# automl/RoBO

Hardware: AMD Instinct MI355X
Metric: EI evals/sec + GP-fit ms at N=4096,D=16; 1/2/4/8 MI355X vs host CPU (higher is better)
Workload: dtype f64

## Files before the change

include/robo_hip.h:

```cpp
#ifndef ROBO_HIP_H
#define ROBO_HIP_H

#include <stdint.h>

#ifdef __cplusplus
extern "C" {
#endif

typedef struct robo_ctx robo_ctx;
typedef struct robo_gp robo_gp;
typedef struct robo_cand robo_cand;

enum robo_status {
    ROBO_OK = 0,
    ROBO_NOT_POSITIVE_DEFINITE = 1,
    ROBO_NOT_FITTED = 2,
    ROBO_BAD_SHAPE = 3,
    ROBO_RUNTIME_ERROR = 4,
    ROBO_BAD_ARGUMENT = 5,
    ROBO_NUMERIC_ERROR = 6
};

enum robo_kernel_kind {
    ROBO_KERNEL_MATERN52_ARD = 0,
    ROBO_KERNEL_RBF_ARD = 1,
    ROBO_KERNEL_FABOLAS = 2
};

enum robo_acq_kind {
    ROBO_ACQ_EI = 0,
    ROBO_ACQ_LOG_EI = 1,
    ROBO_ACQ_PI = 2,
    ROBO_ACQ_LCB = 3
};

#define ROBO_FLAG_ZERO_SIGMA 1u
#define ROBO_FLAG_NEGATIVE_EI 2u
#define ROBO_FLAG_NAN 4u
#define ROBO_FLAG_NOT_FACTORED 8u
#define ROBO_FLAG_FROZEN 16u

int32_t robo_device_count(int32_t* out_n);
int32_t robo_ctx_create(int32_t device, void* hip_stream, robo_ctx** out);
int32_t robo_ctx_destroy(robo_ctx* ctx);
int32_t robo_ctx_live_count(int32_t* out_n);
int32_t robo_ctx_synchronize(robo_ctx* ctx);
int32_t robo_ctx_device_name(robo_ctx* ctx, char* buf, int32_t buf_len);
int32_t robo_ctx_event_record(robo_ctx* ctx, int32_t slot);
int32_t robo_ctx_event_elapsed_ms(robo_ctx* ctx, int32_t slot_begin, int32_t slot_end, float* out_ms);
int32_t robo_ctx_set_phase_events(robo_ctx* ctx, int32_t on);
int32_t robo_ctx_set_tuning(robo_ctx* ctx, const char* key, int64_t value);
const char* robo_last_error_string(void);
const char* robo_version_string(void);

int32_t robo_gp_create(robo_ctx* ctx, int32_t kernel_kind, int32_t n_max, int32_t dim, robo_gp** out);
int32_t robo_gp_destroy(robo_gp* gp);
int32_t robo_gp_set_data(robo_gp* gp, const double* X, const double* y, int32_t n);
int32_t robo_gp_set_output_transform(robo_gp* gp, double y_mean, double y_std);
int32_t robo_gp_set_precision(robo_gp* gp, int32_t fp32_gram);
int32_t robo_theta_size(int32_t kernel_kind, int32_t dim);
int32_t robo_gp_fit(robo_gp* gp, const double* theta, double mean_c, double* out_loglik, int32_t* out_fail_col);
int32_t robo_gp_grad_loglik(robo_gp* gp, const double* theta, double mean_c, double* out_loglik,
                            double* out_grad, int32_t* out_fail_col);

int32_t robo_gp_loglik_batch(robo_gp* gp, const double* thetas, int32_t S, double mean_c, double* out_loglik,
                             int32_t* out_status);

int32_t robo_gp_grad_loglik_batch(robo_gp* gp, const double* thetas, int32_t S, double mean_c, double* out_loglik,
                                  double* out_grad, int32_t* out_status);

int32_t robo_gp_optimize_hypers(robo_gp* gp, double mean_c, int32_t prior_kind, const double* prior_par,
                                const double* lower, const double* upper, const double* starts, int32_t n_starts,
                                int32_t n_iters, int32_t history, double step0, double c1, double gtol,
                                double* out_theta, double* out_value, int32_t* out_best, double* out_final,
                                double* out_values, int32_t* out_status, double* out_trace);

int32_t robo_gp_mcmc_run(robo_gp* gp, double mean_c, int32_t prior_kind, const double* prior_par, int32_t n_walkers,
                         int32_t n_steps, double a, const double* u_stretch, const int32_t* partner,
                         const double* u_accept, int32_t eval_start, double* pos, double* lnp, double* out_chain,
                         double* out_lnprob, int64_t* out_accepted);
int32_t robo_mcmc_draws(uint32_t* mt_key, int32_t* mt_pos, int32_t n_steps, int32_t half, double* u_stretch,
                        int32_t* partner, double* u_accept);
int32_t robo_gp_fit_batch(robo_gp* const* gps, int32_t S, const double* thetas, double mean_c, double* out_loglik,
                          int32_t* out_status);
int32_t robo_gp_get_factor(robo_gp* gp, double* out_L);
int32_t robo_gp_get_gram(robo_gp* gp, const double* theta, double* out_K);
int32_t robo_gp_factor_cond(robo_gp* gp, double* out);
int32_t robo_gp_prefetch_inverse(robo_gp* gp);

int32_t robo_cand_create(robo_ctx* ctx, const double* Xc, int64_t m, int32_t dim, robo_cand** out);
int32_t robo_cand_destroy(robo_cand* cand);
int32_t robo_cand_set_points(robo_cand* cand, const double* Xc, int64_t m);
int32_t robo_cand_create_uniform(robo_ctx* ctx, int64_t m, int32_t dim, uint64_t seed, robo_cand** out);
int32_t robo_cand_create_random(robo_ctx* ctx, int64_t m, int32_t dim, uint64_t seed, int64_t n_uniform,
                                const double* loc, const double* scale, robo_cand** out);
int32_t robo_cand_create_sobol(robo_ctx* ctx, int64_t m, int32_t dim, const uint64_t* sv, const uint64_t* shift,
                               int32_t bits, uint64_t first_index, robo_cand** out);
int32_t robo_cand_get_points(robo_cand* cand, double* out_Xc);
int32_t robo_cand_workspace_chunk(robo_cand* cand, int64_t* out_chunk);
int32_t robo_cand_last_solve_kernel(robo_cand* cand, char* buf, int32_t buf_len);
int32_t robo_cand_get_point(robo_cand* cand, int64_t index, double* out_x);

int32_t robo_gp_predict_cand(robo_gp* gp, robo_cand* cand, double* out_mean, double* out_var);
int32_t robo_gp_predict(robo_gp* gp, const double* Xc, int64_t m, double* out_mean, double* out_var);
int32_t robo_gp_predict_mixture_cand(robo_gp* const* gps, int32_t S, robo_cand* cand, double* out_mean,
                                     double* out_var);
int32_t robo_gp_predict_grad(robo_gp* gp, const double* Xc, int64_t m, double* out_mean, double* out_var,
                             double* out_dmean, double* out_dvar);
int32_t robo_gp_predict_cov(robo_gp* gp, const double* Xc, int64_t m, double* out_mean, double* out_cov);

int32_t robo_acq_eval_cand(robo_gp* gp, int32_t acq_kind, double par, double eta, robo_cand* cand, double* out_acq,
                           double* out_max, int64_t* out_argmax, uint32_t* out_flags);
int32_t robo_acq_eval(robo_gp* gp, int32_t acq_kind, double par, double eta, const double* Xc, int64_t m,
                      double* out_acq, double* out_max, int64_t* out_argmax, uint32_t* out_flags);
#define ROBO_SCREEN_NOT_ELIGIBLE 0
#define ROBO_SCREEN_SCREENED 1
#define ROBO_SCREEN_PROBE_USED 2
#define ROBO_SCREEN_FELL_BACK 3
int32_t robo_cand_last_screen(robo_cand* cand, int64_t* out_n_screened, int64_t* out_n_survivors, int32_t* out_outcome);
#define ROBO_SCREEN_FINISH_NONE 0
#define ROBO_SCREEN_FINISH_FULL 1
#define ROBO_SCREEN_FINISH_LEAN 2
int32_t robo_cand_last_screen_finish(robo_cand* cand, int32_t* out_finish, int32_t* out_fused_tail);
int32_t robo_cand_last_screen_first(robo_cand* cand, int32_t* out_stage, int64_t* out_kept);
int32_t robo_acq_screen_bounds(robo_gp* gp, int32_t acq_kind, double par, double eta, robo_cand* cand, double* out_upper,
                               double* out_lower);
int32_t robo_acq_eval_moments(robo_ctx* ctx, int32_t acq_kind, double par, double eta, const double* mean,
                              const double* var, int64_t m, double* out_acq, double* out_max, int64_t* out_argmax,
                              uint32_t* out_flags);
int32_t robo_acq_eval_marginal_cand(robo_gp* const* gps, int32_t S, int32_t acq_kind, double par, const double* etas,
                                    robo_cand* cand, double* out_acq, double* out_max, int64_t* out_argmax,
                                    uint32_t* out_flags);
int32_t robo_acq_eval_sum_cand(robo_gp* const* gps, int32_t S, int32_t acq_kind, double par, const double* etas,
                               robo_cand* cand, double* out_acq_sum, uint32_t* out_flags);

int32_t robo_acq_refine_cand(robo_gp* gp, int32_t acq_kind, double par, double eta, robo_cand* cand, int32_t n_starts,
                             int32_t n_steps, double step0, double* out_x, double* out_value, int64_t* out_start_index,
                             uint32_t* out_flags, int64_t* out_starts, double* out_trace);
int32_t robo_acq_refine_marginal_cand(robo_gp* const* gps, int32_t S, int32_t acq_kind, double par, const double* etas,
                                      robo_cand* cand, int32_t n_starts, int32_t n_steps, double step0, double* out_x,
                                      double* out_value, int64_t* out_start_index, uint32_t* out_flags,
                                      int64_t* out_starts, double* out_trace);

int32_t robo_rep_sample(robo_gp* gp, int32_t acq_kind, double par, double eta, const double* lower, const double* upper,
                        int32_t normalize, int32_t n_walkers, int32_t n_steps, double a, const double* u_stretch,
                        const int32_t* partner, const double* u_accept, double* pos, double* lnp, int32_t eval_start,
                        int64_t* out_accepted, uint32_t* out_flags, double* out_trace);
int32_t robo_rep_sample_batch(robo_gp* const* gps, int32_t S, int32_t acq_kind, double par, const double* etas,
                              const double* lower, const double* upper, int32_t normalize, int32_t n_walkers,
                              int32_t n_steps, double a, const double* u_stretch, const int32_t* partner,
                              const double* u_accept, double* pos, double* lnp, int32_t eval_start, int64_t* out_accepted,
                              uint32_t* out_flags, double* out_trace);

enum robo_fantasy_kind { ROBO_FANTASY_KRIGING_BELIEVER = 0, ROBO_FANTASY_CONSTANT_LIAR = 1 };
int32_t robo_acq_batch_cand(robo_gp* gp, int32_t acq_kind, double par, double eta, robo_cand* cand, int32_t q,
                            int32_t fantasy_kind, double liar, int64_t* out_idx, double* out_values, double* out_fantasy,
                            uint32_t* out_flags, int32_t* out_n_made, double* out_trace);
int32_t robo_acq_batch_marginal_cand(robo_gp* const* gps, int32_t S, int32_t acq_kind, double par, const double* etas,
                                     robo_cand* cand, int32_t q, int32_t fantasy_kind, double liar, int64_t* out_idx,
                                     double* out_values, double* out_fantasy, uint32_t* out_flags, int32_t* out_n_made,
                                     double* out_trace);

#define ROBO_QEI_MAX_Q 64
#define ROBO_QEI_MAX_K 1024
int32_t robo_qei_batch_cand(robo_gp* gp, double par, double eta, robo_cand* cand, int32_t q, const double* z, int32_t K,
                            int64_t* out_idx, double* out_gain, uint32_t* out_flags, int32_t* out_n_made, double* out_acq,
                            double* out_trace, double* out_coef, double* out_d, double* out_best);
int32_t robo_qei_batch_marginal_cand(robo_gp* const* gps, int32_t S, double par, const double* etas, robo_cand* cand,
                                     int32_t q, const double* z, int32_t K, int64_t* out_idx, double* out_gain,
                                     uint32_t* out_flags, int32_t* out_n_made, double* out_acq, double* out_trace,
                                     double* out_coef, double* out_d, double* out_best);

int32_t robo_mes_eval_cand(robo_gp* gp, double eta, robo_cand* cand, const double* u, int32_t K, int32_t clamp,
                           double* out_acq, double* out_max, int64_t* out_argmax, uint32_t* out_flags, double* out_ystar,
                           double* out_gumbel, double* out_trace);
int32_t robo_mes_eval_marginal_cand(robo_gp* const* gps, int32_t S, const double* etas, robo_cand* cand, const double* u,
                                    int32_t K, int32_t clamp, double* out_acq, double* out_max, int64_t* out_argmax,
                                    uint32_t* out_flags, double* out_ystar, double* out_gumbel, double* out_trace);
int32_t robo_mes_sample_min_moments(robo_ctx* ctx, const double* mean, const double* var, int64_t m, const double* u,
                                    int32_t K, int32_t clamp, double eta, double* out_ystar, double* out_gumbel);
int32_t robo_mes_eval_moments(robo_ctx* ctx, const double* mean, const double* var, int64_t m, const double* ystar,
                              int32_t K, double* out_acq, double* out_max, int64_t* out_argmax, uint32_t* out_flags);

int32_t robo_kg_eval_cand(robo_gp* gp, robo_cand* cand, robo_cand* rep, double sn2, int32_t include_self, double* out_kg,
                          double* out_max, int64_t* out_argmax, uint32_t* out_flags, double* out_disc_mean,
                          double* out_trace);
int32_t robo_kg_eval_marginal_cand(robo_gp* const* gps, int32_t S, robo_cand* cand, robo_cand* rep, const double* sn2s,
                                   int32_t include_self, double* out_kg, double* out_max, int64_t* out_argmax,
                                   uint32_t* out_flags, double* out_disc_mean, double* out_trace);
int32_t robo_kg_eval_moments(robo_ctx* ctx, int64_t m, int32_t nb, double sn2, int32_t include_self, const double* s,
                             const double* v, const double* mean, const double* disc_mean, double* out_kg,
                             double* out_max, int64_t* out_argmax, uint32_t* out_flags);

#define ROBO_EHVI_MAX_FRONT 4096
int32_t robo_ehvi_eval_cand(robo_gp* gp1, robo_gp* gp2, robo_cand* cand, const double* front, int32_t P, const double* ref,
                            double* out_ehvi, double* out_max, int64_t* out_argmax, uint32_t* out_flags,
                            double* out_trace);
int32_t robo_ehvi_eval_moments(robo_ctx* ctx, int64_t m, const double* mean1, const double* var1, const double* mean2,
                               const double* var2, const double* front, int32_t P, const double* ref, double* out_ehvi,
                               double* out_max, int64_t* out_argmax, uint32_t* out_flags);

#define ROBO_CEI_MAX_CONSTRAINTS 16
int32_t robo_cei_eval_cand(robo_gp* objective, robo_gp* const* constraints, int32_t C, const double* thresholds,
                           int32_t acq_kind, double par, double eta, int32_t has_eta, robo_cand* cand,
                           double* out_values , double* out_max, int64_t* out_argmax, uint32_t* out_flags,
                           double* out_trace );
int32_t robo_cei_refine_cand(robo_gp* objective, robo_gp* const* constraints, int32_t C, const double* thresholds,
                             int32_t acq_kind, double par, double eta, int32_t has_eta, robo_cand* cand,
                             int32_t n_starts, int32_t n_steps, double step0,
                             double* out_x, double* out_value, int64_t* out_start_index, uint32_t* out_flags,
                             int64_t* out_starts , double* out_trace );
int32_t robo_cei_eval_moments(robo_ctx* ctx, int64_t m, int32_t C, const double* mean0, const double* var0,
                              const double* means, const double* vars, const double* thresholds, int32_t acq_kind,
                              double par, double eta, int32_t has_eta, double* out_values, double* out_max,
                              int64_t* out_argmax, uint32_t* out_flags);

#define ROBO_PATHS_MAX 64
#define ROBO_PATHS_MAX_FEATURES 4096
typedef struct robo_paths robo_paths;
int32_t robo_paths_create(robo_gp* gp, int32_t F, int32_t S, const double* omega, const double* phase,
                          const double* w, const double* eps, robo_paths** out);
int32_t robo_paths_eval_cand(robo_paths* p, robo_cand* cand, double* out_values ,
                             double* out_min , int64_t* out_argmin , uint32_t* out_flags);
int32_t robo_paths_destroy(robo_paths* p);

#define ROBO_PATHS_MAX_STARTS 1024
#define ROBO_PATHS_MAX_DESCENTS 65536
int32_t robo_paths_descend(robo_paths* p, int32_t P, const int32_t* path_of, const double* x0 ,
                           int32_t n_steps, double step0, double* out_x , double* out_value ,
                           double* out_grad , int32_t* out_code ,
                           uint32_t* out_flags, double* out_trace );
int32_t robo_paths_refine_cand(robo_paths* p, robo_cand* cand, int32_t n_starts, int32_t n_steps, double step0,
                               double* out_x , double* out_value ,
                               int64_t* out_start_index , uint32_t* out_flags,
                               int64_t* out_starts , double* out_trace );

int32_t robo_ig_eval_cand(robo_gp* gp, robo_cand* cand, robo_cand* rep, int32_t n_outcomes, double sn2,
                          const double* logP, const double* lmb, const double* W, const double* dlogPdMu,
                          const double* dlogPdSigma, const double* dlogPdMudMu, double* out_dh, double* out_max,
                          int64_t* out_argmax);
int32_t robo_ig_eval_per_cost_cand(robo_gp* gp, robo_cand* cand, robo_cand* rep, int32_t n_outcomes, double sn2,
                                   const double* logP, const double* lmb, const double* W, const double* dlogPdMu,
                                   const double* dlogPdSigma, const double* dlogPdMudMu, robo_gp* cost_gp,
                                   robo_cand* cost_cand, double overhead, double* out_values, double* out_max,
                                   int64_t* out_argmax);
int32_t robo_ig_eval_moments(robo_ctx* ctx, int64_t m, int32_t nb, int32_t n_outcomes, double sn2, const double* s,
                             const double* v, const double* logP, const double* lmb, const double* W,
                             const double* dlogPdMu, const double* dlogPdSigma, const double* dlogPdMudMu,
                             double* out_dh);
int32_t robo_gp_cross_cov(robo_gp* gp, robo_cand* cand, robo_cand* ref, double* out_cov);
int32_t robo_ep_joint_min(robo_ctx* ctx, int32_t S, int32_t nb, const double* mu, const double* sigma,
                          int32_t with_derivatives, double* logP, double* dlogPdMu, double* dlogPdSigma,
                          double* dlogPdMudMu, int32_t* out_sweeps, int32_t* out_status);

int32_t robo_pmin_mc(robo_ctx* ctx, int32_t S, int32_t nb, int32_t nf, const double* mu, const double* sigma,
                     const double* z, double* out_pmin, double* out_jitter, int32_t* out_status);
int32_t robo_igmc_eval_cand(robo_gp* gp, robo_cand* cand, robo_cand* rep, int32_t n_outcomes, int32_t nf, double sn2,
                            const double* Mb, const double* Vb, const double* logP, const double* lmb, const double* W,
                            const double* z, double* out_dh, double* out_max, int64_t* out_argmax, uint32_t* out_flags);
int32_t robo_igmc_eval_moments(robo_ctx* ctx, int64_t m, int32_t nb, int32_t n_outcomes, int32_t nf, double sn2,
                               const double* s, const double* v, const double* Mb, const double* Vb, const double* logP,
                               const double* lmb, const double* W, const double* z, double* out_dh,
                               int32_t* out_counts, double* out_jitter);

typedef struct robo_comm robo_comm;
#define ROBO_COMM_ID_BYTES 128
int32_t robo_comm_create_id(void* out_id);
int32_t robo_comm_init(robo_ctx* ctx, int32_t rank, int32_t world, const void* id, robo_comm** out);
int32_t robo_comm_destroy(robo_comm* comm);
int32_t robo_comm_info(robo_comm* comm, int32_t* out_rank, int32_t* out_world);
int32_t robo_comm_allgather(robo_comm* comm, const double* send, int64_t count, double* recv);
int32_t robo_acq_eval_cand_sharded(robo_comm* comm, robo_gp* gp, int32_t acq_kind, double par, double eta,
                                   robo_cand* cand, int64_t global_offset, double* out_acq, double* out_max,
                                   int64_t* out_argmax, int32_t* out_owner_rank, uint32_t* out_flags);
int32_t robo_ig_eval_per_cost_cand_sharded(robo_comm* comm, robo_gp* gp, robo_cand* cand, robo_cand* rep,
                                           int32_t n_outcomes, double sn2, const double* logP, const double* lmb,
                                           const double* W, const double* dlogPdMu, const double* dlogPdSigma,
                                           const double* dlogPdMudMu, robo_gp* cost_gp, robo_cand* cost_cand,
                                           double overhead, int64_t global_offset, double* out_values, double* out_max,
                                           int64_t* out_argmax, int32_t* out_owner_rank);
int32_t robo_acq_eval_marginal_cand_sharded(robo_comm* comm, robo_gp* const* gps, int32_t S_local, int32_t S_total,
                                            int32_t acq_kind, double par, const double* etas, robo_cand* cand,
                                            double* out_acq, double* out_max, int64_t* out_argmax,
                                            uint32_t* out_flags);

typedef struct robo_multi robo_multi;
int32_t robo_multi_create(robo_ctx* const* ctxs, int32_t n_ctx, robo_multi** out);
int32_t robo_multi_destroy(robo_multi* multi);
int32_t robo_multi_info(robo_multi* multi, int32_t* out_n, int32_t* out_devices, int32_t* out_threads);
int32_t robo_gp_set_data_multi(robo_multi* multi, robo_gp* const* gps, const double* X, const double* y, int32_t n);
int32_t robo_gp_fit_multi(robo_multi* multi, robo_gp* const* gps, const double* theta, double mean_c, double* out_loglik,
                          int32_t* out_fail_col);
int32_t robo_gp_loglik_batch_multi(robo_multi* multi, robo_gp* const* gps, const double* thetas, int32_t S, double mean_c,
                                   double* out_loglik, int32_t* out_status);
int32_t robo_gp_fit_batch_multi(robo_multi* multi, robo_gp* const* gps, const int32_t* S_dev, const double* thetas,
                                double mean_c, double* out_loglik, int32_t* out_status);
int32_t robo_acq_eval_cand_multi(robo_multi* multi, robo_gp* const* gps, int32_t acq_kind, double par, double eta,
                                 robo_cand* const* cands, const int64_t* global_offsets, double* out_acq, double* out_max,
                                 int64_t* out_argmax, int32_t* out_owner, uint32_t* out_flags);
int32_t robo_ig_eval_cand_multi(robo_multi* multi, robo_gp* const* gps, robo_cand* const* cands, robo_cand* const* reps,
                                int32_t n_outcomes, double sn2, const double* logP, const double* lmb, const double* W,
                                const double* dlogPdMu, const double* dlogPdSigma, const double* dlogPdMudMu,
                                const int64_t* global_offsets, double* out_dh, double* out_max, int64_t* out_argmax,
                                int32_t* out_owner);
int32_t robo_ig_eval_per_cost_cand_multi(robo_multi* multi, robo_gp* const* gps, robo_cand* const* cands,
                                         robo_cand* const* reps, int32_t n_outcomes, double sn2, const double* logP,
                                         const double* lmb, const double* W, const double* dlogPdMu,
                                         const double* dlogPdSigma, const double* dlogPdMudMu, robo_gp* const* cost_gps,
                                         robo_cand* const* cost_cands, double overhead, const int64_t* global_offsets,
                                         double* out_values, double* out_max, int64_t* out_argmax, int32_t* out_owner);
int32_t robo_acq_eval_marginal_cand_multi(robo_multi* multi, robo_gp* const* gps, const int32_t* S_dev, int32_t acq_kind,
                                          double par, const double* etas, robo_cand* const* cands, double* out_acq,
                                          double* out_max, int64_t* out_argmax, uint32_t* out_flags);
int32_t robo_gp_predict_mixture_cand_multi(robo_multi* multi, robo_gp* const* gps, const int32_t* S_dev,
                                           robo_cand* const* cands, double* out_mean, double* out_var);

#ifdef __cplusplus
}
#endif
#endif
```

robo_amd/_lib.py:

```python
import atexit
import ctypes as C
import os
import weakref

import numpy as np

_HERE = os.path.dirname(os.path.abspath(__file__))
DEFAULT_LIBRARY = os.path.join(_HERE, "librobo_hip.so")
DEFAULT_DIAG_LIBRARY = os.path.join(_HERE, "librobo_hip_diag.so")

OK, NOT_POSITIVE_DEFINITE, NOT_FITTED, BAD_SHAPE, RUNTIME_ERROR, BAD_ARGUMENT, NUMERIC_ERROR = range(7)
EP_MAX_NB = 64
EP_NAN_MESSAGE = ("an error occurs while running expectation propagation in entropy search. "
                  "Resulting variance contains NaN")
KERNEL_KINDS = {"matern52": 0, "rbf": 1, "fabolas": 2}
ACQ_KINDS = {"ei": 0, "log_ei": 1, "pi": 2, "lcb": 3}
FLAG_ZERO_SIGMA, FLAG_NEGATIVE_EI, FLAG_NAN, FLAG_NOT_FACTORED, FLAG_FROZEN = 1, 2, 4, 8, 16
SCREEN_NOT_ELIGIBLE, SCREEN_SCREENED, SCREEN_PROBE_USED, SCREEN_FELL_BACK = 0, 1, 2, 3
SCREEN_FINISH_NONE, SCREEN_FINISH_FULL, SCREEN_FINISH_LEAN = 0, 1, 2
FANTASY_KINDS = {"kriging_believer": 0, "constant_liar": 1}
MES_MAX_K = 128
KG_MAX_DISC = 64
EHVI_MAX_FRONT = 4096
CEI_MAX_CONSTRAINTS = 16
PATHS_MAX = 64
PATHS_MAX_FEATURES = 4096
PATHS_MAX_STARTS = 1024
PATHS_MAX_DESCENTS = 65536
REFINE_MAX_STARTS = 1024
MC_MAX_NB, MC_MAX_NP, MC_MAX_NF = 64, 512, 65535

SYMBOLS = [
    "robo_device_count", "robo_ctx_create", "robo_ctx_destroy", "robo_ctx_live_count", "robo_ctx_synchronize",
    "robo_ctx_device_name", "robo_ctx_event_record", "robo_ctx_event_elapsed_ms", "robo_ctx_set_phase_events",
    "robo_ctx_set_tuning",
    "robo_last_error_string", "robo_version_string",
    "robo_gp_create", "robo_gp_destroy", "robo_gp_set_data", "robo_gp_set_output_transform",
    "robo_gp_set_precision", "robo_theta_size",
    "robo_gp_fit", "robo_gp_loglik_batch", "robo_gp_mcmc_run", "robo_mcmc_draws", "robo_gp_fit_batch", "robo_gp_grad_loglik", "robo_gp_grad_loglik_batch",
    "robo_gp_optimize_hypers", "robo_gp_get_factor", "robo_gp_get_gram", "robo_gp_factor_cond", "robo_gp_prefetch_inverse",
    "robo_cand_create", "robo_cand_destroy", "robo_cand_set_points", "robo_cand_create_uniform", "robo_cand_get_points",
    "robo_cand_create_random", "robo_cand_create_sobol", "robo_cand_get_point", "robo_cand_workspace_chunk", "robo_cand_last_solve_kernel",
    "robo_gp_predict_cand", "robo_gp_predict", "robo_gp_predict_cov", "robo_gp_predict_grad", "robo_gp_predict_mixture_cand",
    "robo_acq_eval_cand", "robo_acq_eval", "robo_acq_eval_moments", "robo_acq_eval_marginal_cand", "robo_acq_eval_sum_cand",
    "robo_cand_last_screen", "robo_cand_last_screen_finish", "robo_cand_last_screen_first", "robo_acq_screen_bounds",
    "robo_acq_refine_cand", "robo_acq_refine_marginal_cand",
    "robo_rep_sample", "robo_rep_sample_batch",
    "robo_acq_batch_cand", "robo_acq_batch_marginal_cand", "robo_qei_batch_cand", "robo_qei_batch_marginal_cand",
    "robo_mes_eval_cand", "robo_mes_eval_marginal_cand", "robo_mes_sample_min_moments", "robo_mes_eval_moments",
    "robo_kg_eval_cand", "robo_kg_eval_marginal_cand", "robo_kg_eval_moments",
    "robo_ehvi_eval_cand", "robo_ehvi_eval_moments",
    "robo_cei_eval_cand", "robo_cei_eval_moments", "robo_cei_refine_cand",
    "robo_paths_create", "robo_paths_eval_cand", "robo_paths_destroy", "robo_paths_descend", "robo_paths_refine_cand",
    "robo_ig_eval_cand", "robo_ig_eval_per_cost_cand", "robo_ig_eval_moments", "robo_gp_cross_cov",
    "robo_ep_joint_min", "robo_pmin_mc", "robo_igmc_eval_cand", "robo_igmc_eval_moments",
    "robo_comm_create_id", "robo_comm_init", "robo_comm_destroy", "robo_comm_info", "robo_comm_allgather",
    "robo_acq_eval_cand_sharded", "robo_acq_eval_marginal_cand_sharded", "robo_ig_eval_per_cost_cand_sharded",
    "robo_multi_create", "robo_multi_destroy", "robo_multi_info", "robo_gp_set_data_multi", "robo_gp_fit_multi",
    "robo_gp_loglik_batch_multi", "robo_gp_fit_batch_multi", "robo_acq_eval_cand_multi",
    "robo_ig_eval_cand_multi", "robo_ig_eval_per_cost_cand_multi", "robo_acq_eval_marginal_cand_multi",
    "robo_gp_predict_mixture_cand_multi",
]
COMM_ID_BYTES = 128
DIAG_SYMBOLS = [
    "robo_selftest_mfma_layout", "robo_microbench_mfma_f64", "robo_microbench_mfma_f64_detail", "robo_microbench_gemm_f64",
    "robo_selftest_diag_timeline", "robo_diag_clock_sample_begin", "robo_diag_clock_sample_end",
    "robo_selftest_stretch_move", "robo_diag_cross_gram", "robo_diag_cov_rows",
]


class RoboHipUnavailable(RuntimeError):
    pass


class RoboHipError(RuntimeError):
    pass


class RoboBadShape(AssertionError):
    """ROBO_BAD_SHAPE from the library (the reference uses ``assert`` for shapes, base_model.py:68-70,76) -- its own type
    so that callers can tell the library's verdict from a Python-side assert"""


_lib = None
_lib_path = None
_diag = None
_dp = C.POINTER(C.c_double)


def _arr(a):
    return a.ctypes.data_as(_dp)


def _f64(a, shape=None):
    a = np.ascontiguousarray(a, dtype=np.float64)
    if shape is not None and a.shape != shape:
        raise AssertionError("expected shape %r, got %r" % (shape, a.shape))
    return a


def _handles(gps):
    return (C.c_void_p * max(len(gps), 1))(*[g._h for g in gps])


def _etas(eta, S):
    return _f64(np.broadcast_to(np.asarray(eta, dtype=np.float64), (S,)))


def _ensemble_head(gps, eta, marginal, *between):
    if not marginal:
        return (gps[0]._h,) + between + (float(eta),)
    return (_handles(gps), len(gps)) + between + (_arr(_etas(eta, len(gps))),)


class _Best(object):

    def __init__(self):
        self.max, self.argmax, self.flags = C.c_double(0), C.c_int64(0), C.c_uint32(0)
        self.refs = (C.byref(self.max), C.byref(self.argmax), C.byref(self.flags))

    def values(self):
        return self.max.value, self.argmax.value, self.flags.value


def use_library(path):
    global _lib, _lib_path, _default_ctx, _diag, _extra_ctx, _multis
    _close_multis()
    _lib = None
    _diag = None
    _lib_path = path
    _default_ctx = {}
    _extra_ctx = {}
    _multis = {}


def library_path():
    return _lib_path or DEFAULT_LIBRARY


def lib():
    global _lib
    if _lib is not None:
        return _lib
    path = library_path()
    if not os.path.exists(path):
        raise RoboHipUnavailable(
            "%s not found: build it with `python -m robo_amd.build` (hipcc, gfx950). "
            "robo_amd has no CPU fallback." % path)
    try:
        L = C.CDLL(path)
    except OSError as e:
        raise RoboHipUnavailable("cannot load %s: %s" % (path, e))
    vp, i32, i64, dbl = C.c_void_p, C.c_int32, C.c_int64, C.c_double
    pp = C.POINTER(vp)
    sig = {
        "robo_device_count": [C.POINTER(i32)],
        "robo_ctx_create": [i32, vp, pp],
        "robo_ctx_destroy": [vp],
        "robo_ctx_live_count": [C.POINTER(i32)],
        "robo_ctx_synchronize": [vp],
        "robo_ctx_device_name": [vp, C.c_char_p, i32],
        "robo_ctx_event_record": [vp, i32],
        "robo_ctx_event_elapsed_ms": [vp, i32, i32, C.POINTER(C.c_float)],
        "robo_ctx_set_phase_events": [vp, i32],
        "robo_ctx_set_tuning": [vp, C.c_char_p, i64],
        "robo_gp_create": [vp, i32, i32, i32, pp],
        "robo_gp_destroy": [vp],
        "robo_gp_set_data": [vp, _dp, _dp, i32],
        "robo_gp_set_output_transform": [vp, dbl, dbl],
        "robo_gp_set_precision": [vp, i32],
        "robo_theta_size": [i32, i32],
        "robo_gp_fit": [vp, _dp, dbl, _dp, C.POINTER(i32)],
        "robo_gp_loglik_batch": [vp, _dp, i32, dbl, _dp, C.POINTER(i32)],
        "robo_gp_fit_batch": [pp, i32, _dp, dbl, _dp, C.POINTER(i32)],
        "robo_mcmc_draws": [C.POINTER(C.c_uint32), C.POINTER(i32), i32, i32, _dp, C.POINTER(i32), _dp],
        "robo_gp_mcmc_run": [vp, dbl, i32, _dp, i32, i32, dbl, _dp, C.POINTER(i32), _dp, i32, _dp, _dp, _dp, _dp,
                             C.POINTER(i64)],
        "robo_gp_grad_loglik": [vp, _dp, dbl, _dp, _dp, C.POINTER(i32)],
        "robo_gp_grad_loglik_batch": [vp, _dp, i32, dbl, _dp, _dp, C.POINTER(i32)],
        "robo_gp_optimize_hypers": [vp, dbl, i32, _dp, _dp, _dp, _dp, i32, i32, i32, dbl, dbl, dbl, _dp, _dp,
                                    C.POINTER(i32), _dp, _dp, C.POINTER(i32), _dp],
        "robo_gp_get_factor": [vp, _dp],
        "robo_gp_get_gram": [vp, _dp, _dp],
        "robo_gp_factor_cond": [vp, _dp],
        "robo_gp_prefetch_inverse": [vp],
        "robo_cand_create": [vp, _dp, i64, i32, pp],
        "robo_cand_destroy": [vp],
        "robo_cand_set_points": [vp, _dp, i64],
        "robo_cand_create_uniform": [vp, i64, i32, C.c_uint64, pp],
        "robo_cand_get_points": [vp, _dp],
        "robo_cand_create_random": [vp, i64, i32, C.c_uint64, i64, _dp, _dp, pp],
        "robo_cand_create_sobol": [vp, i64, i32, C.POINTER(C.c_uint64), C.POINTER(C.c_uint64), i32, C.c_uint64, pp],
        "robo_cand_get_point": [vp, i64, _dp],
        "robo_cand_workspace_chunk": [vp, C.POINTER(i64)],
        "robo_cand_last_solve_kernel": [vp, C.c_char_p, i32],
        "robo_gp_predict_cand": [vp, vp, _dp, _dp],
        "robo_gp_predict": [vp, _dp, i64, _dp, _dp],
        "robo_gp_predict_cov": [vp, _dp, i64, _dp, _dp],
        "robo_gp_predict_grad": [vp, _dp, i64, _dp, _dp, _dp, _dp],
        "robo_gp_predict_mixture_cand": [pp, i32, vp, _dp, _dp],
        "robo_acq_eval_cand": [vp, i32, dbl, dbl, vp, _dp, _dp, C.POINTER(i64), C.POINTER(C.c_uint32)],
        "robo_acq_eval": [vp, i32, dbl, dbl, _dp, i64, _dp, _dp, C.POINTER(i64), C.POINTER(C.c_uint32)],
        "robo_cand_last_screen": [vp, C.POINTER(i64), C.POINTER(i64), C.POINTER(i32)],
        "robo_cand_last_screen_finish": [vp, C.POINTER(i32), C.POINTER(i32)],
        "robo_cand_last_screen_first": [vp, C.POINTER(i32), C.POINTER(i64)],
        "robo_acq_screen_bounds": [vp, i32, dbl, dbl, vp, _dp, _dp],
        "robo_acq_eval_moments": [vp, i32, dbl, dbl, _dp, _dp, i64, _dp, _dp, C.POINTER(i64), C.POINTER(C.c_uint32)],
        "robo_acq_eval_marginal_cand": [pp, i32, i32, dbl, _dp, vp, _dp, _dp, C.POINTER(i64),
                                        C.POINTER(C.c_uint32)],
        "robo_acq_eval_sum_cand": [pp, i32, i32, dbl, _dp, vp, _dp, C.POINTER(C.c_uint32)],
        "robo_acq_refine_cand": [vp, i32, dbl, dbl, vp, i32, i32, dbl, _dp, _dp, C.POINTER(i64), C.POINTER(C.c_uint32),
                                 C.POINTER(i64), _dp],
        "robo_acq_refine_marginal_cand": [pp, i32, i32, dbl, _dp, vp, i32, i32, dbl, _dp, _dp, C.POINTER(i64),
                                          C.POINTER(C.c_uint32), C.POINTER(i64), _dp],
        "robo_rep_sample": [vp, i32, dbl, dbl, _dp, _dp, i32, i32, i32, dbl, _dp, C.POINTER(i32), _dp, _dp, _dp, i32,
                            C.POINTER(i64), C.POINTER(C.c_uint32), _dp],
        "robo_rep_sample_batch": [pp, i32, i32, dbl, _dp, _dp, _dp, i32, i32, i32, dbl, _dp, C.POINTER(i32), _dp, _dp, _dp,
                                  i32, C.POINTER(i64), C.POINTER(C.c_uint32), _dp],
        "robo_acq_batch_cand": [vp, i32, dbl, dbl, vp, i32, i32, dbl, C.POINTER(i64), _dp, _dp, C.POINTER(C.c_uint32),
                                C.POINTER(i32), _dp],
        "robo_acq_batch_marginal_cand": [pp, i32, i32, dbl, _dp, vp, i32, i32, dbl, C.POINTER(i64), _dp, _dp,
                                         C.POINTER(C.c_uint32), C.POINTER(i32), _dp],
        "robo_qei_batch_cand": [vp, dbl, dbl, vp, i32, _dp, i32, C.POINTER(i64), _dp, C.POINTER(C.c_uint32), C.POINTER(i32),
                                _dp, _dp, _dp, _dp, _dp],
        "robo_qei_batch_marginal_cand": [pp, i32, dbl, _dp, vp, i32, _dp, i32, C.POINTER(i64), _dp, C.POINTER(C.c_uint32),
                                         C.POINTER(i32), _dp, _dp, _dp, _dp, _dp],
        "robo_mes_eval_cand": [vp, dbl, vp, _dp, i32, i32, _dp, _dp, C.POINTER(i64), C.POINTER(C.c_uint32), _dp, _dp, _dp],
        "robo_mes_eval_marginal_cand": [pp, i32, _dp, vp, _dp, i32, i32, _dp, _dp, C.POINTER(i64), C.POINTER(C.c_uint32),
                                        _dp, _dp, _dp],
        "robo_mes_sample_min_moments": [vp, _dp, _dp, i64, _dp, i32, i32, dbl, _dp, _dp],
        "robo_mes_eval_moments": [vp, _dp, _dp, i64, _dp, i32, _dp, _dp, C.POINTER(i64), C.POINTER(C.c_uint32)],
        "robo_kg_eval_cand": [vp, vp, vp, dbl, i32, _dp, _dp, C.POINTER(i64), C.POINTER(C.c_uint32), _dp, _dp],
        "robo_kg_eval_marginal_cand": [pp, i32, vp, vp, _dp, i32, _dp, _dp, C.POINTER(i64), C.POINTER(C.c_uint32), _dp, _dp],
        "robo_kg_eval_moments": [vp, i64, i32, dbl, i32, _dp, _dp, _dp, _dp, _dp, _dp, C.POINTER(i64),
                                 C.POINTER(C.c_uint32)],
        "robo_ehvi_eval_cand": [vp, vp, vp, _dp, i32, _dp, _dp, _dp, C.POINTER(i64), C.POINTER(C.c_uint32), _dp],
        "robo_ehvi_eval_moments": [vp, i64, _dp, _dp, _dp, _dp, _dp, i32, _dp, _dp, _dp, C.POINTER(i64),
                                   C.POINTER(C.c_uint32)],
        "robo_cei_eval_cand": [vp, pp, i32, _dp, i32, dbl, dbl, i32, vp, _dp, _dp, C.POINTER(i64), C.POINTER(C.c_uint32),
                               _dp],
        "robo_cei_eval_moments": [vp, i64, i32, _dp, _dp, _dp, _dp, _dp, i32, dbl, dbl, i32, _dp, _dp, C.POINTER(i64),
                                  C.POINTER(C.c_uint32)],
        "robo_cei_refine_cand": [vp, pp, i32, _dp, i32, dbl, dbl, i32, vp, i32, i32, dbl, _dp, _dp, C.POINTER(i64),
                                 C.POINTER(C.c_uint32), C.POINTER(i64), _dp],
        "robo_paths_create": [vp, i32, i32, _dp, _dp, _dp, _dp, pp],
        "robo_paths_eval_cand": [vp, vp, _dp, _dp, C.POINTER(i64), C.POINTER(C.c_uint32)],
        "robo_paths_destroy": [vp],
        "robo_paths_descend": [vp, i32, C.POINTER(i32), _dp, i32, dbl, _dp, _dp, _dp, C.POINTER(i32), C.POINTER(C.c_uint32),
                               _dp],
        "robo_paths_refine_cand": [vp, vp, i32, i32, dbl, _dp, _dp, C.POINTER(i64), C.POINTER(C.c_uint32), C.POINTER(i64),
                                   _dp],
        "robo_ig_eval_cand": [vp, vp, vp, i32, dbl, _dp, _dp, _dp, _dp, _dp, _dp, _dp, _dp, C.POINTER(i64)],
        "robo_ig_eval_per_cost_cand": [vp, vp, vp, i32, dbl, _dp, _dp, _dp, _dp, _dp, _dp, vp, vp, dbl, _dp, _dp,
                                       C.POINTER(i64)],
        "robo_ig_eval_per_cost_cand_sharded": [vp, vp, vp, vp, i32, dbl, _dp, _dp, _dp, _dp, _dp, _dp, vp, vp, dbl, i64,
                                               _dp, _dp, C.POINTER(i64), C.POINTER(i32)],
        "robo_ig_eval_moments": [vp, i64, i32, i32, dbl, _dp, _dp, _dp, _dp, _dp, _dp, _dp, _dp, _dp],
        "robo_gp_cross_cov": [vp, vp, vp, _dp],
        "robo_ep_joint_min": [vp, i32, i32, _dp, _dp, i32, _dp, _dp, _dp, _dp, C.POINTER(i32), C.POINTER(i32)],
        "robo_pmin_mc": [vp, i32, i32, i32, _dp, _dp, _dp, _dp, _dp, C.POINTER(i32)],
        "robo_igmc_eval_cand": [vp, vp, vp, i32, i32, dbl, _dp, _dp, _dp, _dp, _dp, _dp, _dp, _dp, C.POINTER(i64),
                                C.POINTER(C.c_uint32)],
        "robo_igmc_eval_moments": [vp, i64, i32, i32, i32, dbl, _dp, _dp, _dp, _dp, _dp, _dp, _dp, _dp, _dp,
                                   C.POINTER(i32), _dp],
        "robo_comm_create_id": [C.c_char_p],
        "robo_comm_init": [vp, i32, i32, C.c_char_p, pp],
        "robo_comm_destroy": [vp],
        "robo_comm_info": [vp, C.POINTER(i32), C.POINTER(i32)],
        "robo_comm_allgather": [vp, _dp, i64, _dp],
        "robo_acq_eval_cand_sharded": [vp, vp, i32, dbl, dbl, vp, i64, _dp, _dp, C.POINTER(i64), C.POINTER(i32),
                                       C.POINTER(C.c_uint32)],
        "robo_acq_eval_marginal_cand_sharded": [vp, pp, i32, i32, i32, dbl, _dp, vp, _dp, _dp, C.POINTER(i64),
                                                C.POINTER(C.c_uint32)],
        "robo_multi_create": [pp, i32, pp],
        "robo_multi_destroy": [vp],
        "robo_multi_info": [vp, C.POINTER(i32), C.POINTER(i32), C.POINTER(i32)],
        "robo_gp_set_data_multi": [vp, pp, _dp, _dp, i32],
        "robo_gp_fit_multi": [vp, pp, _dp, dbl, _dp, C.POINTER(i32)],
        "robo_gp_loglik_batch_multi": [vp, pp, _dp, i32, dbl, _dp, C.POINTER(i32)],
        "robo_gp_fit_batch_multi": [vp, pp, C.POINTER(i32), _dp, dbl, _dp, C.POINTER(i32)],
        "robo_acq_eval_cand_multi": [vp, pp, i32, dbl, dbl, pp, C.POINTER(i64), _dp, _dp, C.POINTER(i64), C.POINTER(i32),
                                     C.POINTER(C.c_uint32)],
        "robo_ig_eval_cand_multi": [vp, pp, pp, pp, i32, dbl, _dp, _dp, _dp, _dp, _dp, _dp, C.POINTER(i64), _dp, _dp,
                                    C.POINTER(i64), C.POINTER(i32)],
        "robo_ig_eval_per_cost_cand_multi": [vp, pp, pp, pp, i32, dbl, _dp, _dp, _dp, _dp, _dp, _dp, pp, pp, dbl,
                                             C.POINTER(i64), _dp, _dp, C.POINTER(i64), C.POINTER(i32)],
        "robo_acq_eval_marginal_cand_multi": [vp, pp, C.POINTER(i32), i32, dbl, _dp, pp, _dp, _dp, C.POINTER(i64),
                                              C.POINTER(C.c_uint32)],
        "robo_gp_predict_mixture_cand_multi": [vp, pp, C.POINTER(i32), pp, _dp, _dp],
    }
    for name, args in sig.items():
        if path != DEFAULT_LIBRARY and not hasattr(L, name):
            def missing(*_, _name=name, _path=path):
                raise RoboHipUnavailable("%s does not export %s" % (_path, _name))
            setattr(L, name, missing)
            continue
        fn = getattr(L, name)
        fn.argtypes = args
        fn.restype = i32
    L.robo_last_error_string.restype = C.c_char_p
    L.robo_last_error_string.argtypes = []
    L.robo_version_string.restype = C.c_char_p
    L.robo_version_string.argtypes = []
    n = i32(0)
    L.robo_device_count(C.byref(n))
    if n.value < 1:
        raise RoboHipUnavailable("librobo_hip loaded but no HIP device is visible (robo_amd has no CPU fallback)")
    _lib = L
    return L


def diag():
    global _diag
    if _diag is not None:
        return _diag
    lib()
    path = _lib_path or DEFAULT_DIAG_LIBRARY
    if not os.path.exists(path):
        raise RoboHipUnavailable("%s not found: build it with `python -m robo_amd.build`" % path)
    D = C.CDLL(path)
    vp, i32 = C.c_void_p, C.c_int32
    for name, args in {"robo_selftest_mfma_layout": [vp, _dp], "robo_microbench_mfma_f64": [vp, i32, _dp],
                       "robo_microbench_mfma_f64_detail": [vp, i32, _dp],
                       "robo_microbench_gemm_f64": [vp, i32, i32, i32, i32, _dp],
                       "robo_selftest_diag_timeline": [vp, _dp, _dp],
                       "robo_diag_clock_sample_begin": [vp, i32], "robo_diag_clock_sample_end": [vp, _dp],
                       "robo_selftest_stretch_move": [vp, _dp, _dp, _dp, C.c_double, i32, i32, _dp, _dp, _dp],
                       "robo_diag_cross_gram": [vp, _dp, _dp, i32, _dp],
                       "robo_diag_cov_rows": [vp, i32, i32, C.c_double, C.c_double, C.c_double, _dp, _dp, C.c_int64,
                                              _dp]}.items():
        fn = getattr(D, name)
        fn.argtypes = args
        fn.restype = i32
    _diag = D
    return D


def last_error():
    return lib().robo_last_error_string().decode("utf-8", "replace")


def check(status, msg=None):
    if status == OK:
        return
    msg = last_error() if msg is None else msg
    if status == NOT_POSITIVE_DEFINITE:
        raise np.linalg.LinAlgError(msg or "matrix is not positive definite")
    if status == NOT_FITTED:
        raise Exception('Model has to be trained first!')
    if status == BAD_SHAPE:
        raise RoboBadShape(msg)
    if status == BAD_ARGUMENT:
        raise ValueError(msg)
    if status == NUMERIC_ERROR:
        raise Exception(EP_NAN_MESSAGE)
    raise RoboHipError(msg)


def live_contexts():
    n = C.c_int32(0)
    lib().robo_ctx_live_count(C.byref(n))
    return n.value


def device_count():
    n = C.c_int32(0)
    lib().robo_device_count(C.byref(n))
    return n.value


def mcmc_draws(random_state, n_steps, half):
    name, key, pos, has_gauss, cached = random_state.get_state()
    if name != "MT19937":
        raise ValueError("legacy MT19937 RandomState expected")
    key = np.ascontiguousarray(key, dtype=np.uint32).copy()
    p = C.c_int32(int(pos))
    uz = np.empty((n_steps, 2, half))
    ua = np.empty((n_steps, 2, half))
    pa = np.empty((n_steps, 2, half), dtype=np.int32)
    check(lib().robo_mcmc_draws(key.ctypes.data_as(C.POINTER(C.c_uint32)), C.byref(p), int(n_steps), int(half), _arr(uz),
                                pa.ctypes.data_as(C.POINTER(C.c_int32)), _arr(ua)))
    random_state.set_state((name, key, int(p.value), has_gauss, cached))
    return uz, pa, ua


class Context(object):

    def __init__(self, device=0, stream=None):
        self._h = C.c_void_p()
        self._owner = lib()
        check(self._owner.robo_ctx_create(int(device), C.c_void_p(stream) if stream else None, C.byref(self._h)))
        self.device = int(device)

    def close(self):
        if getattr(self, "_h", None) is not None and self._h:
            self._owner.robo_ctx_destroy(self._h)
            self._h = None

    def __del__(self):
        try:
            self.close()
        except Exception:
            pass

    def synchronize(self):
        check(lib().robo_ctx_synchronize(self._h))

    @property
    def name(self):
        buf = C.create_string_buffer(256)
        check(lib().robo_ctx_device_name(self._h, buf, 256))
        return buf.value.decode()

    def record(self, slot):
        check(lib().robo_ctx_event_record(self._h, int(slot)))

    def elapsed_ms(self, a, b):
        ms = C.c_float(0)
        check(lib().robo_ctx_event_elapsed_ms(self._h, int(a), int(b), C.byref(ms)))
        return float(ms.value)

    def set_phase_events(self, on):
        check(lib().robo_ctx_set_phase_events(self._h, 1 if on else 0))

    def set_tuning(self, key, value=None):
        v = -(2 ** 63) if value is None else int(value)
        check(lib().robo_ctx_set_tuning(self._h, key.encode(), v))

    def selftest_mfma_layout(self):
        e = C.c_double(0)
        check(diag().robo_selftest_mfma_layout(self._h, C.byref(e)))
        return e.value

    def selftest_stretch_move(self, c, s, u, a=2.0, P=18):
        c, s, u = (np.ascontiguousarray(v, dtype=np.float64) for v in (c, s, u))
        assert c.shape == s.shape == u.shape and c.ndim == 1
        z, q, d = np.empty_like(c), np.empty_like(c), np.empty_like(c)
        check(diag().robo_selftest_stretch_move(self._h, _arr(c), _arr(s), _arr(u), float(a), int(P), c.size,
                                                _arr(z), _arr(q), _arr(d)))
        return z, q, d

    def cov_rows(self, kind, xi, xj, amp=1.0, blr_a=0.0, blr_b=0.0):
        xi, xj = _f64(xi), _f64(xj)
        assert xi.ndim == 2 and xi.shape == xj.shape
        out = np.empty(xi.shape[0])
        check(diag().robo_diag_cov_rows(self._h, KERNEL_KINDS[kind], xi.shape[1], float(amp), float(blr_a), float(blr_b),
                                        _arr(xi), _arr(xj), xi.shape[0], _arr(out)))
        return out

    def microbench_mfma_f64_detail(self, iters=2000):
        out = np.zeros(4)
        check(diag().robo_microbench_mfma_f64_detail(self._h, int(iters), _arr(out)))
        return {"tflops": out[0], "cycles_per_mfma_single_wave": out[1], "shader_mhz": out[2],
                "cycles_per_mfma_dependent_chain": out[3]}

    def microbench_gemm_f64(self, variant, wgs=512, k=4096, reps=5):
        out = np.zeros(2)
        check(diag().robo_microbench_gemm_f64(self._h, int(variant), int(wgs), int(k), int(reps), _arr(out)))
        return float(out[0]), float(out[1])

    def clock_sample_begin(self, window_us):
        check(diag().robo_diag_clock_sample_begin(self._h, int(window_us)))

    def clock_sample_end(self):
        out = np.zeros(3)
        check(diag().robo_diag_clock_sample_end(self._h, _arr(out)))
        return {"mean": float(out[0]), "min": float(out[1]), "max": float(out[2])}

    def microbench_mfma_f64(self, iters=2000):
        t = C.c_double(0)
        check(diag().robo_microbench_mfma_f64(self._h, int(iters), C.byref(t)))
        return t.value


_default_ctx = {}


def default_context(device=None):
    if device is None:
        device = int(os.environ.get("ROBO_DEVICE", os.environ.get("LOCAL_RANK", "0")))
        if device >= device_count():
            device = 0
    if device not in _default_ctx:
        _default_ctx[device] = Context(device)
    return _default_ctx[device]


_extra_ctx = {}
_multis = {}
_live_multis = weakref.WeakSet()


def _close_multis():
    for m in list(_live_multis):
        try:
            m.close()
        except Exception:
            pass
    _multis.clear()


atexit.register(_close_multis)


def resolve_devices(devices=None, n_gpus=None):
    if devices is None and n_gpus is not None and int(n_gpus) > 1:
        devices = list(range(int(n_gpus)))
    if devices is None:
        return None
    devices = [int(d) for d in devices]
    n = device_count()
    if any(d < 0 or d >= n for d in devices):
        raise ValueError("devices %r: this process sees %d HIP device(s)" % (devices, n))
    return devices if len(devices) > 1 else None


def contexts_for(devices):
    seen = {}
    out = []
    for d in devices:
        k = seen.get(d, 0)
        seen[d] = k + 1
        if k == 0:
            out.append(default_context(d))
        else:
            if (d, k) not in _extra_ctx:
                _extra_ctx[(d, k)] = Context(d)
            out.append(_extra_ctx[(d, k)])
    return out


def multi_for(devices):
    key = tuple(int(d) for d in devices)
    if key not in _multis:
        _multis[key] = Multi(contexts_for(key))
    return _multis[key]


def shard_range(n_items, slot, n_slots):
    base, rem = divmod(int(n_items), int(n_slots))
    begin = slot * base + min(slot, rem)
    return begin, begin + base + (1 if slot < rem else 0)


class Candidates(object):

    def __init__(self, ctx, Xc=None, m=None, dim=None, seed=None, n_uniform=None, loc=None, scale=None, sobol=None,
                 first=0):
        self.ctx = ctx
        self._h = C.c_void_p()
        self._owner = lib()
        if sobol is not None:
            if hasattr(sobol, "random"):
                if not all(hasattr(sobol, a) for a in ("_sv", "_shift", "bits")):
                    raise RoboHipError("this SciPy's qmc.Sobol does not expose its direction numbers (_sv, _shift, "
                                       "bits; SciPy 1.7-1.15 do): pass a (sv, shift, bits) triple instead")
                sv, shift, bits = sobol._sv, sobol._shift, int(sobol.bits)
            else:
                sv, shift, bits = sobol
            sv = np.ascontiguousarray(sv, dtype=np.uint64)
            shift = np.ascontiguousarray(shift, dtype=np.uint64)
            assert sv.ndim == 2 and sv.shape[1] == bits and shift.shape == (sv.shape[0],)
            self.m, self.dim = int(m), int(sv.shape[0])
            u64p = C.POINTER(C.c_uint64)
            check(lib().robo_cand_create_sobol(ctx._h, self.m, self.dim, sv.ctypes.data_as(u64p),
                                               shift.ctypes.data_as(u64p), bits, int(first), C.byref(self._h)))
        elif loc is not None:
            loc, scale = _f64(loc), _f64(scale)
            self.m, self.dim = int(m), int(loc.shape[0])
            assert scale.shape == loc.shape
            check(lib().robo_cand_create_random(ctx._h, self.m, self.dim, int(seed or 0),
                                                self.m if n_uniform is None else int(n_uniform), _arr(loc),
                                                _arr(scale), C.byref(self._h)))
        elif Xc is not None:
            Xc = _f64(Xc)
            assert Xc.ndim == 2
            self.m, self.dim = Xc.shape
            check(lib().robo_cand_create(ctx._h, _arr(Xc), self.m, self.dim, C.byref(self._h)))
        else:
            self.m, self.dim = int(m), int(dim)
            check(lib().robo_cand_create_uniform(ctx._h, self.m, self.dim, int(seed or 0), C.byref(self._h)))

    def set_points(self, Xc):
        Xc = _f64(Xc, (self.m, self.dim))
        check(lib().robo_cand_set_points(self._h, _arr(Xc), self.m))

    def point(self, index):
        out = np.empty(self.dim)
        check(lib().robo_cand_get_point(self._h, int(index), _arr(out)))
        return out

    def chunk(self):
        n = C.c_int64(0)
        check(lib().robo_cand_workspace_chunk(self._h, C.byref(n)))
        return int(n.value)

    def solve_kernel(self):
        buf = C.create_string_buffer(64)
        check(lib().robo_cand_last_solve_kernel(self._h, buf, 64))
        return buf.value.decode()

    def bounds_kernel(self):
        buf = C.create_string_buffer(128)
        check(lib().robo_cand_last_solve_kernel(self._h, buf, 128))
        return buf.raw.split(b"\0")[1].decode()

    def screen_finish(self):
        f = C.c_int32(0)
        check(lib().robo_cand_last_screen_finish(self._h, C.byref(f), None))
        return int(f.value)

    def screen_tail_fused(self):
        f, t = C.c_int32(0), C.c_int32(0)
        check(lib().robo_cand_last_screen_finish(self._h, C.byref(f), C.byref(t)))
        return bool(t.value)

    def screen_first(self):
        stage, kept = C.c_int32(0), C.c_int64(0)
        check(lib().robo_cand_last_screen_first(self._h, C.byref(stage), C.byref(kept)))
        return int(stage.value), int(kept.value)

    def last_screen(self):
        n, kept, outcome = C.c_int64(0), C.c_int64(0), C.c_int32(0)
        check(lib().robo_cand_last_screen(self._h, C.byref(n), C.byref(kept), C.byref(outcome)))
        return int(n.value), int(kept.value), int(outcome.value)

    def points(self):
        out = np.empty((self.m, self.dim))
        check(lib().robo_cand_get_points(self._h, _arr(out)))
        return out

    def close(self):
        if getattr(self, "_h", None) is not None and self._h:
            self._owner.robo_cand_destroy(self._h)
            self._h = None

    def __del__(self):
        try:
            self.close()
        except Exception:
            pass


def _full_theta(gp, theta):
    head = gp.fixed_head
    if not head:
        return theta
    theta = np.asarray(theta, dtype=np.float64)
    if theta.ndim == 1:
        return np.concatenate([head, theta])
    return np.hstack([np.tile(np.asarray(head, dtype=np.float64), (theta.shape[0], 1)), theta])


class DeviceGP(object):

    def __init__(self, ctx, kind, n_max, dim, fixed_head=()):
        self.ctx, self.kind, self.n_max, self.dim = ctx, kind, int(n_max), int(dim)
        self._h = C.c_void_p()
        self._owner = lib()
        check(self._owner.robo_gp_create(ctx._h, KERNEL_KINDS[kind], self.n_max, self.dim, C.byref(self._h)))
        self.n = 0
        self.n_theta = lib().robo_theta_size(KERNEL_KINDS[kind], self.dim)
        self.fixed_head = tuple(float(v) for v in fixed_head)

    def set_precision(self, fp32_gram):
        check(lib().robo_gp_set_precision(self._h, 1 if fp32_gram else 0))

    def close(self):
        if getattr(self, "_h", None) is not None and self._h:
            self._owner.robo_gp_destroy(self._h)
            self._h = None

    def __del__(self):
        try:
            self.close()
        except Exception:
            pass

    def set_data(self, X, y):
        X, y = _f64(X), _f64(y)
        assert X.ndim == 2 and y.ndim == 1 and X.shape[0] == y.shape[0] and X.shape[1] == self.dim
        check(lib().robo_gp_set_data(self._h, _arr(X), _arr(y), X.shape[0]))
        self.n = X.shape[0]

    def set_output_transform(self, y_mean, y_std):
        check(lib().robo_gp_set_output_transform(self._h, float(y_mean), float(y_std)))

    def fit(self, theta, mean_c):
        theta = _f64(_full_theta(self, theta), (self.n_theta,))
        ll, col = C.c_double(0), C.c_int32(0)
        check(lib().robo_gp_fit(self._h, _arr(theta), float(mean_c), C.byref(ll), C.byref(col)))
        return ll.value

    def grad_loglik(self, theta, mean_c):
        theta = _f64(_full_theta(self, theta), (self.n_theta,))
        ll = C.c_double()
        col = C.c_int32()
        grad = np.empty(self.n_theta)
        check(lib().robo_gp_grad_loglik(self._h, _arr(theta), float(mean_c), C.byref(ll), _arr(grad), C.byref(col)))
        return ll.value, grad[len(self.fixed_head):]

    def loglik_batch(self, thetas, mean_c):
        thetas = _f64(_full_theta(self, np.atleast_2d(thetas)))
        assert thetas.ndim == 2 and thetas.shape[1] == self.n_theta
        S = thetas.shape[0]
        ll = np.empty(S)
        st = np.empty(S, dtype=np.int32)
        check(lib().robo_gp_loglik_batch(self._h, _arr(thetas), S, float(mean_c), _arr(ll),
                                         st.ctypes.data_as(C.POINTER(C.c_int32))))
        return ll, st

    def grad_loglik_batch(self, thetas, mean_c):
        thetas = _f64(_full_theta(self, np.atleast_2d(thetas)))
        assert thetas.ndim == 2 and thetas.shape[1] == self.n_theta
        S = thetas.shape[0]
        ll = np.empty(S)
        grad = np.empty((S, self.n_theta))
        st = np.empty(S, dtype=np.int32)
        check(lib().robo_gp_grad_loglik_batch(self._h, _arr(thetas), S, float(mean_c), _arr(ll), _arr(grad),
                                              st.ctypes.data_as(C.POINTER(C.c_int32))))
        return ll, grad[:, len(self.fixed_head):], st

    def optimize_hypers(self, mean_c, prior, lower, upper, starts, n_iters=60, history=8, step0=0.5, c1=1e-4, gtol=1e-5,
                        diagnostics=False):
        assert not self.fixed_head, "the device optimiser moves every library hyper-parameter: use the host optimiser"
        P = self.n_theta
        starts = _f64(np.atleast_2d(starts))
        K = starts.shape[0]
        assert starts.shape == (K, P)
        lower, upper = _f64(np.broadcast_to(lower, (P,))), _f64(np.broadcast_to(upper, (P,)))
        if prior is None:
            kind, par = 0, np.zeros(9)
        else:
            kind = int(prior[0])
            par = np.zeros(9)
            given = _f64(prior[1]).reshape(-1)
            assert given.size == (9 if kind == 2 else 5)
            par[:given.size] = given
        n_iters = int(n_iters)
        theta, value, best = np.empty(P), C.c_double(), C.c_int32()
        final, values, status = np.empty((K, P)), np.empty(K), np.empty(K, dtype=np.int32)
        trace = np.empty((max(n_iters, 0) + 1, K, 2 * P + 3)) if diagnostics else None
        check(lib().robo_gp_optimize_hypers(self._h, float(mean_c), kind, _arr(par), _arr(lower), _arr(upper), _arr(starts),
                                            K, n_iters, int(history), float(step0), float(c1), float(gtol), _arr(theta),
                                            C.byref(value), C.byref(best), _arr(final), _arr(values),
                                            status.ctypes.data_as(C.POINTER(C.c_int32)),
                                            _arr(trace) if diagnostics else None))
        return HyperOptResult(theta, value.value, best.value, final, values, status, trace)

    def mcmc_run(self, mean_c, prior, pos, lnp, n_steps, u_stretch, partner, u_accept, a=2.0):
        pos = np.array(pos, dtype=np.float64, order="C")
        k = pos.shape[0]
        assert not self.fixed_head, "the device chain moves every library hyper-parameter: use the host sampler"
        assert pos.shape == (k, self.n_theta)
        eval_start = lnp is None
        lnp = np.zeros(k) if eval_start else np.array(lnp, dtype=np.float64)
        n_steps = int(n_steps)
        uz = np.ascontiguousarray(u_stretch, dtype=np.float64).reshape(-1)
        ua = np.ascontiguousarray(u_accept, dtype=np.float64).reshape(-1)
        pa = np.ascontiguousarray(partner, dtype=np.int32).reshape(-1)
        assert uz.size == ua.size == pa.size == n_steps * k
        chain = np.empty((k, n_steps, self.n_theta))
        lnps = np.empty((k, n_steps))
        acc = np.zeros(k, dtype=np.int64)
        if prior is None:
            kind, par = 0, np.zeros(9)
        else:
            kind = int(prior[0])
            par = np.zeros(9)
            given = _f64(prior[1]).reshape(-1)
            assert given.size == (9 if kind == 2 else 5)
            par[:given.size] = given
        check(lib().robo_gp_mcmc_run(self._h, float(mean_c), kind, _arr(par), k, n_steps, float(a), _arr(uz),
                                     pa.ctypes.data_as(C.POINTER(C.c_int32)), _arr(ua), int(eval_start), _arr(pos),
                                     _arr(lnp), _arr(chain), _arr(lnps), acc.ctypes.data_as(C.POINTER(C.c_int64))))
        return pos, lnp, chain, lnps, acc

    def factor(self):
        out = np.empty((self.n, self.n))
        check(lib().robo_gp_get_factor(self._h, _arr(out)))
        return out

    def prefetch_inverse(self):
        check(lib().robo_gp_prefetch_inverse(self._h))

    def factor_cond(self):
        out = np.zeros(3)
        check(lib().robo_gp_factor_cond(self._h, _arr(out)))
        return float(out[0]), float(out[1]), float(out[2])

    def gram(self, theta):
        theta = _f64(_full_theta(self, theta), (self.n_theta,))
        out = np.empty((self.n, self.n))
        check(lib().robo_gp_get_gram(self._h, _arr(theta), _arr(out)))
        return out

    def cross_gram(self, theta, Xc):
        theta = _f64(_full_theta(self, theta), (self.n_theta,))
        Xc = _f64(Xc)
        assert Xc.ndim == 2 and Xc.shape[1] == self.dim
        out = np.empty((Xc.shape[0], self.n))
        check(diag().robo_diag_cross_gram(self._h, _arr(theta), _arr(Xc), Xc.shape[0], _arr(out)))
        return out

    def diag_timeline(self, theta):
        theta = _f64(theta, (self.n_theta,))
        out = np.zeros(38)
        check(diag().robo_selftest_diag_timeline(self._h, _arr(theta), _arr(out)))
        return out

    def predict(self, Xc):
        if isinstance(Xc, Candidates):
            mean, var = np.empty(Xc.m), np.empty(Xc.m)
            check(lib().robo_gp_predict_cand(self._h, Xc._h, _arr(mean), _arr(var)))
            return mean, var
        Xc = _f64(Xc)
        assert Xc.ndim == 2 and Xc.shape[1] == self.dim
        mean, var = np.empty(Xc.shape[0]), np.empty(Xc.shape[0])
        check(lib().robo_gp_predict(self._h, _arr(Xc), Xc.shape[0], _arr(mean), _arr(var)))
        return mean, var

    def predict_cov(self, Xc):
        Xc = _f64(Xc)
        assert Xc.ndim == 2 and Xc.shape[1] == self.dim
        m = Xc.shape[0]
        mean, cov = np.empty(m), np.empty((m, m))
        check(lib().robo_gp_predict_cov(self._h, _arr(Xc), m, _arr(mean), _arr(cov)))
        return mean, cov

    def predict_grad(self, Xc):
        Xc = _f64(Xc)
        assert Xc.ndim == 2 and Xc.shape[1] == self.dim
        m = Xc.shape[0]
        mean, var, dm, dv = np.empty(m), np.empty(m), np.empty((m, self.dim)), np.empty((m, self.dim))
        check(lib().robo_gp_predict_grad(self._h, _arr(Xc), m, _arr(mean), _arr(var), _arr(dm), _arr(dv)))
        return mean, var, dm, dv

    def acq(self, kind, par, eta, Xc, want_values=True):
        best = _Best()
        if isinstance(Xc, Candidates):
            m = Xc.m
            out = np.empty(m) if want_values else None
            check(lib().robo_acq_eval_cand(self._h, ACQ_KINDS[kind], float(par), float(eta), Xc._h,
                                           _arr(out) if want_values else None, *best.refs))
        else:
            Xc = _f64(Xc)
            assert Xc.ndim == 2 and Xc.shape[1] == self.dim
            m = Xc.shape[0]
            out = np.empty(m) if want_values else None
            check(lib().robo_acq_eval(self._h, ACQ_KINDS[kind], float(par), float(eta), _arr(Xc), m,
                                      _arr(out) if want_values else None, *best.refs))
        return (out,) + best.values()

    def screen_bounds(self, kind, par, eta, cand):
        up, lo = np.empty(cand.m), np.empty(cand.m)
        check(lib().robo_acq_screen_bounds(self._h, ACQ_KINDS[kind], float(par), float(eta), cand._h, _arr(up), _arr(lo)))
        return up, lo

    def refine(self, kind, par, eta, cand, n_starts=256, n_steps=50, step0=0.05, diagnostics=False):
        return acq_refine([self], kind, par, eta, cand, n_starts, n_steps, step0, diagnostics, marginal=False)


    def select_batch(self, kind, par, eta, cand, q, fantasy="kriging_believer", liar=0.0, diagnostics=False):
        return acq_batch([self], kind, par, eta, cand, q, fantasy, liar, diagnostics, marginal=False)

    def select_batch_joint(self, par, eta, cand, q, z, diagnostics=False):
        return qei_batch([self], par, eta, cand, q, z, diagnostics, marginal=False)


    def mes(self, eta, cand, u, clamp=True, want_values=True, diagnostics=False):
        return mes_marginal([self], eta, cand, u, clamp, want_values, diagnostics, marginal=False)


    def kg(self, cand, rep, sn2, include_self=True, want_values=True, diagnostics=False):
        return kg_marginal([self], cand, rep, sn2, include_self, want_values, diagnostics, marginal=False)


    def ehvi(self, other, cand, front, ref, want_values=True, diagnostics=False):
        front, ref = _ehvi_front(front, ref)
        P = front.shape[0]
        out = np.empty(cand.m) if want_values else None
        trace = np.empty((cand.m, 4)) if (diagnostics and P <= EHVI_MAX_FRONT) else None
        best = _Best()
        check(lib().robo_ehvi_eval_cand(self._h, other._h, cand._h, _arr(front), P, _arr(ref),
                                        _arr(out) if want_values else None, *best.refs,
                                        _arr(trace) if trace is not None else None))
        return EHVIResult(out, *best.values(), trace)

    def cei(self, constraint_gps, cand, thresholds, kind, par, eta, want_values=True, diagnostics=False):
        head = self._cei_head(constraint_gps, thresholds, kind, par, eta)
        Cn = head[2]
        out = np.empty(cand.m) if want_values else None
        trace = np.empty((cand.m, 2 * (Cn + 1) + 2)) if (diagnostics and Cn <= CEI_MAX_CONSTRAINTS) else None
        best = _Best()
        check(lib().robo_cei_eval_cand(*head, cand._h, _arr(out) if want_values else None, *best.refs,
                                       _arr(trace) if trace is not None else None))
        return CEIResult(out, *best.values(), trace)

    def _cei_head(self, constraint_gps, thresholds, kind, par, eta):
        constraint_gps = list(constraint_gps)
        Cn = len(constraint_gps)
        return (self._h, _handles(constraint_gps), Cn, _arr(_cei_thresholds(thresholds, Cn)), _cei_kind(kind), float(par),
                0.0 if eta is None else float(eta), int(eta is not None))

    def cei_refine(self, constraint_gps, cand, thresholds, kind, par, eta, n_starts=256, n_steps=50, step0=0.05,
                   diagnostics=False):
        return _refine_call(lib().robo_cei_refine_cand, self._cei_head(constraint_gps, thresholds, kind, par, eta), cand,
                            n_starts, n_steps, step0, diagnostics)

    def sample_paths(self, omega, phase, w, eps):
        return PosteriorPaths(self, omega, phase, w, eps)


class HyperOptResult(object):

    def __init__(self, theta, value, best, final, values, status, trace=None):
        self.theta, self.value, self.best = theta, value, best
        self.final, self.values, self.status, self.trace = final, values, status, trace


class MESResult(object):

    def __init__(self, values, max, argmax, flags, ystar, gumbel=None, trace=None):
        self.values, self.max, self.argmax, self.flags = values, float(max), int(argmax), int(flags)
# ... 741 lines not shown
```

robo_amd/csrc/api_ctx.hip:

```cpp
#include <atomic>
#include <cctype>
#include <cstdarg>
#include <cstdlib>
#include <mutex>

#include "api_internal.h"

namespace robo {

static thread_local char g_err[1024] = "";

void set_error(const char* fmt, ...) {
    va_list ap;
    va_start(ap, fmt);
    vsnprintf(g_err, sizeof(g_err), fmt, ap);
    va_end(ap);
}

struct TuneKey {
    const char* name;
    long long Tuning::*ll;
    int Tuning::*i;
    long long dflt;
};
static const TuneKey TUNE_KEYS[] = {
    {"ws_bytes", &Tuning::ws_bytes, nullptr, (long long)6 << 30},
    {"trsm_small_max", &Tuning::trsm_small_max, nullptr, 16384},
    {"trsm_small_narrow", nullptr, &Tuning::trsm_small_narrow, -1},
    {"trsm_small_deep", nullptr, &Tuning::trsm_small_deep, -1},
    {"trsm_rows", nullptr, &Tuning::trsm_rows, 1},
    {"trsm_pair", nullptr, &Tuning::trsm_pair, 0},
    {"predict_stepwise", nullptr, &Tuning::predict_stepwise, 0},
    {"winv_max", &Tuning::winv_max, nullptr, 32768},
    {"winv_min_blocks", nullptr, &Tuning::winv_min_blocks, 6},
    {"winv_cond_max", &Tuning::winv_cond_max, nullptr, 100000},
    {"winv_rows", nullptr, &Tuning::winv_rows, -1},
    {"winv_kc_shift", nullptr, &Tuning::winv_kc_shift, -1},
    {"winv_gemv", nullptr, &Tuning::winv_gemv, -1},
    {"potrf_fused", nullptr, &Tuning::potrf_fused, 1},
    {"potrf_fused_panels", nullptr, &Tuning::potrf_fused_panels, -1},
    {"potrf_tm4_min", nullptr, &Tuning::potrf_tm4_min, 96},
    {"potrf_max_wg", nullptr, &Tuning::potrf_max_wg, 0},
    {"potrf_group", nullptr, &Tuning::potrf_group, 0},
    {"potrf_tail_split", nullptr, &Tuning::potrf_tail_split, 1},
    {"potrf_follow", nullptr, &Tuning::potrf_follow, 1},
    {"potrf_follow_from", nullptr, &Tuning::potrf_follow_from, -2},
    {"potrf_pub_early", nullptr, &Tuning::potrf_pub_early, 6},
    {"potrf_follow_rows", nullptr, &Tuning::potrf_follow_rows, -1},
    {"potrf_poll_sleep", nullptr, &Tuning::potrf_poll_sleep, 1},
    {"potrf_batch_roll", nullptr, &Tuning::potrf_batch_roll, 0},
    {"potrf_batch_follow", nullptr, &Tuning::potrf_batch_follow, -1},
    {"potrf_batch_tm4_min", nullptr, &Tuning::potrf_batch_tm4_min, 96},
    {"potrf_thin_last", nullptr, &Tuning::potrf_thin_last, 1},
    {"potrf_split", nullptr, &Tuning::potrf_split, 3},
    {"potrf_gram_split", nullptr, &Tuning::potrf_gram_split, 0},
    {"potrf_split_min", nullptr, &Tuning::potrf_split_min, 12},
    {"potrf_lead", nullptr, &Tuning::potrf_lead, -1},
    {"mcmc_block_step", nullptr, &Tuning::mcmc_block_step, 2},
    {"mcmc_fused_tail", nullptr, &Tuning::mcmc_fused_tail, 1},
    {"acq_screen", nullptr, &Tuning::acq_screen, 1},
    {"acq_screen_min", &Tuning::acq_screen_min, nullptr, -1},
    {"acq_screen_keep_max", nullptr, &Tuning::acq_screen_keep_max, 25},
    {"acq_screen_dot", nullptr, &Tuning::acq_screen_dot, -1},
    {"acq_screen_lean", nullptr, &Tuning::acq_screen_lean, -1},
    {"acq_screen_single", nullptr, &Tuning::acq_screen_single, -1},
    {"acq_screen_fused_tail", nullptr, &Tuning::acq_screen_fused_tail, 1},
    {"trsm_chain", nullptr, &Tuning::trsm_chain, -1},
    {"trsm_chain_max_wg", nullptr, &Tuning::trsm_chain_max_wg, 4},
    {"trsm_chain_spin_limit", &Tuning::trsm_chain_spin_limit, nullptr, -1},
};

static void tune_set(Tuning* t, const TuneKey& k, long long v) {
    if (k.ll) t->*(k.ll) = v;
    else t->*(k.i) = (int)v;
}

void tuning_from_env(Tuning* t) {
    for (const TuneKey& k : TUNE_KEYS) {
        char env[64] = "ROBO_";
        size_t o = strlen(env);
        for (const char* p = k.name; *p && o + 1 < sizeof(env); ++p) env[o++] = (char)toupper((unsigned char)*p);
        env[o] = 0;
        const char* e = getenv(env);
        tune_set(t, k, (e && *e) ? (long long)atof(e) : k.dflt);
    }
    if (t->ws_bytes < 1) t->ws_bytes = (long long)6 << 30;
}

static std::mutex g_ctx_life;
static std::atomic<int> g_ctx_live{0};

static void ctx_free(robo_ctx* c) {
    hipSetDevice(c->device);
    hipStreamSynchronize(c->stream);
    for (int i = 0; i < ROBO_EVENT_SLOTS; ++i) hipEventDestroy(c->events[i]);
    if (c->aux_ready) {
        hipEventDestroy(c->ev_fork);
        for (int i = 0; i < ROBO_AUX_STREAMS; ++i) {
            hipStreamSynchronize(c->aux[i]);
            hipStreamDestroy(c->aux[i]);
            hipEventDestroy(c->ev_join[i]);
        }
    }
    hipFree(c->d_scalars);
    hipFree(c->d_fail);
    hipFree(c->d_prog);
    hipHostFree(c->h_pinned);
    if (c->h_chain) hipHostFree(c->h_chain);
    ep_release(c);
    mc_release(c);
    if (c->own_stream) hipStreamDestroy(c->stream);
    delete c;
    --g_ctx_live;
}

void ctx_retain(robo_ctx* c) {
    std::lock_guard<std::mutex> lock(g_ctx_life);
    ++c->users;
}

void ctx_release(robo_ctx* c) {
    bool last;
    {
        std::lock_guard<std::mutex> lock(g_ctx_life);
        last = --c->users == 0 && c->closing;
    }
    if (last) ctx_free(c);
}

int ctx_aux_streams(robo_ctx* c) {
    if (c->aux_ready) return ROBO_OK;
    ROBO_HIP_CHECK(hipSetDevice(c->device));
    ROBO_HIP_CHECK(hipEventCreateWithFlags(&c->ev_fork, hipEventDisableTiming));
    for (int i = 0; i < ROBO_AUX_STREAMS; ++i) {
        ROBO_HIP_CHECK(hipStreamCreateWithFlags(&c->aux[i], hipStreamNonBlocking));
        ROBO_HIP_CHECK(hipEventCreateWithFlags(&c->ev_join[i], hipEventDisableTiming));
    }
    c->aux_ready = true;
    return ROBO_OK;
}

}

using namespace robo;

extern "C" {

const char* robo_last_error_string(void) { return g_err; }
const char* robo_version_string(void) { return "robo_hip 0.1 (gfx950, fp64 MFMA)"; }

int32_t robo_device_count(int32_t* out_n) {
    int n = 0;
    if (hipGetDeviceCount(&n) != hipSuccess) n = 0;
    *out_n = n;
    return ROBO_OK;
}

int32_t robo_ctx_create(int32_t device, void* hip_stream, robo_ctx** out) {
    if (!out) return ROBO_BAD_ARGUMENT;
    ROBO_HIP_CHECK(hipSetDevice(device));
    robo_ctx* c = new robo_ctx();
    memset(c, 0, sizeof(*c));
    c->device = device;
    if (hip_stream) {
        c->stream = (hipStream_t)hip_stream;
        c->own_stream = false;
    } else {
        ROBO_HIP_CHECK(hipStreamCreateWithFlags(&c->stream, hipStreamNonBlocking));
        c->own_stream = true;
    }
    for (int i = 0; i < ROBO_EVENT_SLOTS; ++i) ROBO_HIP_CHECK(hipEventCreate(&c->events[i]));
    {
        const char* e = getenv("ROBO_PHASE_EVENTS");
        c->phase_events = e && atoi(e) != 0;
    }
    tuning_from_env(&c->tune);
    hipDeviceProp_t prop;
    ROBO_HIP_CHECK(hipGetDeviceProperties(&prop, device));
    snprintf(c->name, sizeof(c->name), "%s (%s)", prop.name, prop.gcnArchName);
    c->num_cu = prop.multiProcessorCount;
    ROBO_TRY(dev_alloc(&c->d_scalars, 8));
    ROBO_TRY(dev_alloc(&c->d_fail, 4));
    ROBO_TRY(dev_alloc(&c->d_prog, 2 * PROG_STRIDE));
    ROBO_HIP_CHECK(hipHostMalloc((void**)&c->h_pinned, (MAX_DIM + 64) * sizeof(double), 0));
    ++g_ctx_live;
    *out = c;
    return ROBO_OK;
}

int32_t robo_ctx_destroy(robo_ctx* c) {
    if (!c) return ROBO_OK;
    bool now;
    {
        std::lock_guard<std::mutex> lock(g_ctx_life);
        c->closing = true;
        now = c->users == 0;
    }
    if (now) ctx_free(c);
    return ROBO_OK;
}

int32_t robo_ctx_live_count(int32_t* out_n) {
    if (!out_n) return ROBO_BAD_ARGUMENT;
    *out_n = g_ctx_live.load();
    return ROBO_OK;
}

int32_t robo_ctx_synchronize(robo_ctx* c) {
    if (!c) return ROBO_BAD_ARGUMENT;
    ROBO_HIP_CHECK(hipSetDevice(c->device));
    ROBO_HIP_CHECK(hipStreamSynchronize(c->stream));
    return ROBO_OK;
}

int32_t robo_ctx_device_name(robo_ctx* c, char* buf, int32_t len) {
    if (!buf || len <= 0) return ROBO_BAD_ARGUMENT;
    snprintf(buf, (size_t)len, "%s", c->name);
    return ROBO_OK;
}

int32_t robo_ctx_event_record(robo_ctx* c, int32_t slot) {
    if (slot < 0 || slot >= ROBO_EVENT_SLOTS) return ROBO_BAD_ARGUMENT;
    ROBO_HIP_CHECK(hipSetDevice(c->device));
    ROBO_HIP_CHECK(hipEventRecord(c->events[slot], c->stream));
    return ROBO_OK;
}

int32_t robo_ctx_set_phase_events(robo_ctx* c, int32_t on) {
    if (!c) return ROBO_BAD_ARGUMENT;
    c->phase_events = on != 0;
    return ROBO_OK;
}

int32_t robo_ctx_set_tuning(robo_ctx* c, const char* key, int64_t value) {
    if (!c || !key) return ROBO_BAD_ARGUMENT;
    if (strcmp(key, "env") == 0) {
        tuning_from_env(&c->tune);
        return ROBO_OK;
    }
    for (const TuneKey& k : TUNE_KEYS)
        if (strcmp(key, k.name) == 0) {
            tune_set(&c->tune, k, value == INT64_MIN ? k.dflt : (long long)value);
            if (c->tune.ws_bytes < 1) c->tune.ws_bytes = (long long)6 << 30;
            if (strcmp(key, "trsm_chain") == 0) c->chain_off = false;
            return ROBO_OK;
        }
    set_error("robo_ctx_set_tuning: unknown key '%s'", key);
    return ROBO_BAD_ARGUMENT;
}

int32_t robo_ctx_event_elapsed_ms(robo_ctx* c, int32_t a, int32_t b, float* out_ms) {
    if (a < 0 || a >= ROBO_EVENT_SLOTS || b < 0 || b >= ROBO_EVENT_SLOTS || !out_ms) return ROBO_BAD_ARGUMENT;
    ROBO_HIP_CHECK(hipEventSynchronize(c->events[b]));
    ROBO_HIP_CHECK(hipEventElapsedTime(out_ms, c->events[a], c->events[b]));
    return ROBO_OK;
}

}
```

robo_amd/csrc/common.h:

```cpp
#pragma once
#include <hip/hip_runtime.h>

#include <cstdint>
#include <cstdio>
#include <cstring>

#include "../../include/robo_hip.h"

namespace robo {

constexpr int NB = 128;
constexpr int WG = 256;
constexpr double JITTER = 1.25e-12;
constexpr int MAX_DIM = 256;
constexpr int PROG_STRIDE = 512;

typedef double v4d __attribute__((vector_size(32)));

__device__ __forceinline__ v4d mfma_f64(double a, double b, v4d c) {
    return __builtin_amdgcn_mfma_f64_16x16x4f64(a, b, c, 0, 0, 0);
}

__device__ __forceinline__ double rn_add(double a, double b) {
#pragma clang fp contract(off)
    return a + b;
}
__device__ __forceinline__ double rn_sub(double a, double b) {
#pragma clang fp contract(off)
    return a - b;
}
__device__ __forceinline__ double rn_mul(double a, double b) {
#pragma clang fp contract(off)
    return a * b;
}
__device__ __forceinline__ double rn_div(double a, double b) {
#pragma clang fp contract(off)
    return a / b;
}

__device__ __forceinline__ void st_agent(double* p, double v) { __hip_atomic_store(p, v, __ATOMIC_RELAXED, __HIP_MEMORY_SCOPE_AGENT); }
__device__ __forceinline__ double ld_agent(const double* p) {
    return __hip_atomic_load(const_cast<double*>(p), __ATOMIC_RELAXED, __HIP_MEMORY_SCOPE_AGENT);
}
__device__ __forceinline__ void st_agent_u32(unsigned* p, unsigned v) { __hip_atomic_store(p, v, __ATOMIC_RELAXED, __HIP_MEMORY_SCOPE_AGENT); }
__device__ __forceinline__ unsigned ld_agent_u32(const unsigned* p) {
    return __hip_atomic_load(const_cast<unsigned*>(p), __ATOMIC_RELAXED, __HIP_MEMORY_SCOPE_AGENT);
}
__device__ __forceinline__ void add_agent_u32(unsigned* p, unsigned v) {
    __hip_atomic_fetch_add(p, v, __ATOMIC_RELAXED, __HIP_MEMORY_SCOPE_AGENT);
}
__device__ __forceinline__ void st_agent2(double* p, double2 v) {
#ifdef __AMDGCN__
    typedef double v2d __attribute__((ext_vector_type(2)));
    const v2d x = {v.x, v.y};
    asm volatile("global_store_dwordx4 %0, %1, off sc1\n\ts_nop 1" : : "v"(p), "v"(x) : "memory");
#else
    p[0] = v.x;
    p[1] = v.y;
#endif
}
__device__ __forceinline__ void ld_agent2x4(const double* p, double2& a, double2& b, double2& c, double2& d) {
#ifdef __AMDGCN__
    typedef double v2d __attribute__((ext_vector_type(2)));
    v2d x0, x1, x2, x3;
    asm volatile(
        "global_load_dwordx4 %0, %4, off sc1\n\t"
        "global_load_dwordx4 %1, %4, off offset:16 sc1\n\t"
        "global_load_dwordx4 %2, %4, off offset:32 sc1\n\t"
        "global_load_dwordx4 %3, %4, off offset:48 sc1\n\t"
        "s_waitcnt vmcnt(0)"
        : "=&v"(x0), "=&v"(x1), "=&v"(x2), "=&v"(x3)
        : "v"(p)
        : "memory");
    a = make_double2(x0.x, x0.y);
    b = make_double2(x1.x, x1.y);
    c = make_double2(x2.x, x2.y);
    d = make_double2(x3.x, x3.y);
#else
    a = make_double2(p[0], p[1]);
    b = make_double2(p[2], p[3]);
    c = make_double2(p[4], p[5]);
    d = make_double2(p[6], p[7]);
#endif
}
__device__ __forceinline__ void drain_vmem() { __builtin_amdgcn_s_waitcnt(0x0F70); }
constexpr long long FOLLOW_SENTINEL = 0x7FF8DEAD00C0FFEELL;
constexpr unsigned PROG_SPIN_LIMIT = 1u << 24;

struct CovParams {
    int kind;
    int dim;
    double amp, blr_a, blr_b;
};

struct FitSample {
    CovParams cov;
    double noise;
    double mean_c;
    int direct;
};

constexpr double GRAM_DIRECT_BOUND = 1e-12;
__host__ __device__ inline int gram_needs_direct(int kind, const double* ism, const double* x2max, int D) {
#pragma clang fp contract(off)
    if (kind == ROBO_KERNEL_FABOLAS) return 0;
    double s = 0.0;
    for (int d = 0; d < D; ++d) {
        const double m2 = ism[d] * ism[d];
        const double t = m2 * x2max[d];
        s = s + t;
    }
    const double c = (double)(D + 3) * 4.44089209850062616e-16;
    const double b = c * s;
    return b > GRAM_DIRECT_BOUND ? 1 : 0;
}

struct ThetaArgs {
    FitSample sp;
    double ism[MAX_DIM];
};

void set_error(const char* fmt, ...);

#define ROBO_HIP_CHECK(expr)                                                                       \
    do {                                                                                           \
        hipError_t _e = (expr);                                                                    \
        if (_e != hipSuccess) {                                                                    \
            robo::set_error("%s failed: %s (%s:%d)", #expr, hipGetErrorString(_e), __FILE__, __LINE__); \
            return ROBO_RUNTIME_ERROR;                                                             \
        }                                                                                          \
    } while (0)

#define ROBO_LAUNCH_CHECK()                                                                        \
    do {                                                                                           \
        hipError_t _e = hipGetLastError();                                                         \
        if (_e != hipSuccess) {                                                                    \
            robo::set_error("kernel launch failed: %s (%s:%d)", hipGetErrorString(_e), __FILE__, __LINE__); \
            return ROBO_RUNTIME_ERROR;                                                             \
        }                                                                                          \
    } while (0)

#define ROBO_TRY(expr)                \
    do {                              \
        int _s = (expr);              \
        if (_s != ROBO_OK) return _s; \
    } while (0)

static inline int round_up(int x, int m) { return (x + m - 1) / m * m; }
static inline int64_t round_up64(int64_t x, int64_t m) { return (x + m - 1) / m * m; }

}

namespace robo {
struct Tuning {
    long long ws_bytes;
    long long trsm_small_max;
    int trsm_small_narrow;
    int trsm_small_deep;
    int trsm_rows;
    int trsm_pair;
    int predict_stepwise;
    long long winv_max;
    int winv_min_blocks;
    int winv_gemv;
    int winv_kc_shift;
    int winv_rows;
    long long winv_cond_max;
    int potrf_fused;
    int potrf_fused_panels;
    int potrf_tm4_min, potrf_max_wg, potrf_group;
    int potrf_batch_tm4_min;
    int potrf_thin_last;
    int potrf_split;
    int potrf_gram_split;
    int potrf_split_min;
    int potrf_lead;
    int potrf_tail_split;
    int potrf_follow;
    int potrf_follow_from;
    int potrf_pub_early;
    int potrf_follow_rows;
    int potrf_poll_sleep;
    int potrf_batch_roll;
    int potrf_batch_follow;
    int mcmc_fused_tail;
    int mcmc_block_step;
    int acq_screen;
    long long acq_screen_min;
    int acq_screen_keep_max;
    int acq_screen_dot;
    int acq_screen_lean;
    int acq_screen_single;
    int acq_screen_fused_tail;
    int trsm_chain;
    int trsm_chain_max_wg;
    long long trsm_chain_spin_limit;
};
void tuning_from_env(Tuning* t);
}
struct robo_ctx;
namespace robo {
struct EpWork;
void ep_release(robo_ctx* ctx);
struct McWork;
void mc_release(robo_ctx* ctx);
int ctx_aux_streams(robo_ctx* ctx);
void ctx_retain(robo_ctx* ctx);
void ctx_release(robo_ctx* ctx);
}

struct robo_cand;
namespace robo {
struct RefineSel {
    unsigned long long hi;
    unsigned lo;
    unsigned remaining;
    unsigned keff;
    unsigned count;
};
struct RefineState {
    int K, D;
    double *x, *f, *g, *alpha;
    double *aused;
    double *y, *ys;
    double *fy, *gy;
    int *frozen, *bad;
    long long* start;
    double* sel_val;
    long long* sel_idx;
    unsigned* hist;
    unsigned* flags;
    RefineSel* sel;
    double* out;
    double* trace;
};
struct RefineWork {
    int K, D;
    ::robo_cand* ws;
    char* d_block;
    double* d_trace;
    size_t trace_cap;
    RefineState st;
};
int refine_alloc(robo_ctx* ctx, int K, int D, RefineWork** out);
void refine_free(RefineWork* w);

constexpr int BATCH_MAX_Q = 1024;
struct BatchState {
    int S, q, qcap;
    long long m, m_pad;
    double *mu_lat, *var_lat;
    double* mean_t;
    double *w, *v, *beta;
    double* chist;
    double* dhist;
    double* scal;
    double* eta;
    double *val, *fant;
    long long* idx;
    unsigned* flg;
    int *n_made, *stop;
    double* trace;
};
struct BatchWork {
    int64_t m;
    int S, n_pad, q;
    char* d_block;
    double* d_trace;
    size_t trace_cap;
    char* h_report;
    size_t rep_off, rep_bytes, off_fant, off_idx, off_flg, off_int;
    BatchState st;
};
int batch_alloc(robo_ctx* ctx, int64_t m, int64_t m_pad, int S, int n_pad, int q, BatchWork** out);
void batch_free(BatchWork* w);

constexpr int QEI_MAX_Q = 64, QEI_MAX_K = 1024;
struct QeiState {
    int K;
    double* z;
    double* b;
    double* acq;
    double* coef;
    double* best;
};
struct QeiWork {
    int64_t m;
    int S, n_pad, q, K;
    BatchWork* base;
    char* d_block;
    double* d_diag;
    size_t diag_cap;
    QeiState qs;
};

struct MesState {
    long long m;
    int K, nblk;
    double *ystar, *gumbel;
    double* status;
    double* u;
    double* brk;
    double *bpart, *fpart;
    int* done;
};
struct MesWork {
    int64_t m;
    int S, K;
    double* d_block;
    double* d_trace;
    size_t trace_cap;
    double* h_stage;
    size_t rep_doubles;
    MesState st;
};
int mes_alloc(int64_t m, int S, int K, MesWork** out);
void mes_free(MesWork* w);

struct RepChain {
    const double* ism;
    double* Xcs;
    const double *mean, *var;
    double eta;
};
struct RepState {
    int S, k, D, T, normalize;
    long long m_pad;
    double a;
    double *pos, *lnp;
    double *q, *z;
    int* outside;
    long long* nacc;
    unsigned* flags;
    const double *uz, *ua;
    const int* partner;
    const double *lower, *upper;
    const RepChain* chain;
    double* trace;
};
struct RepWork {
    size_t bytes;
    char* d_block;
    double* d_trace;
    size_t trace_cap;
};
void rep_free(RepWork* w);

constexpr int HYPER_MAX_STARTS = 64, HYPER_MAX_HISTORY = 16;
struct HyperState {
    int K, P, D, kind, n, hist, n_iters, prior_kind;
    double mean_c, step0, c1, gtol;
    double prior_par[9];
    const double *lower, *upper;
    double *x, *f, *g, *alpha;
    double *z, *aused;
    double *sh, *yh;
    int *npairs, *state, *pending;
    int* err;
    double* out;
    double* trace;
    FitSample* d_sp;
    double* d_ism;
    const double* d_x2max;
    const double *d_out, *d_grad;
    const int* d_fail;
};
struct HyperWork {
    int g_cap, g_npad, g_P;
    double *d_V, *d_A, *d_alpha, *d_part, *d_out;
    int K, P, hist;
    char* d_block;
    double* d_trace;
    size_t trace_cap;
};
void hyper_free(HyperWork* w);
int launch_rep_propose(robo_ctx* ctx, const RepState& st, int start, int h, int it);
int launch_rep_accept(robo_ctx* ctx, const RepState& st, int acq_kind, double par, int start, int h, int it);
}

constexpr int ROBO_AUX_STREAMS = 3;
enum RoboEventSlot {
    EV_GRAM_KERNEL = 19,
    EV_FIT_BEGIN = 20,
    EV_FIT_GRAM_END = 21,
    EV_FIT_POTRF_END = 22,
    EV_FIT_END = 23,
    EV_PREDICT_BEGIN = 24,
    EV_PREDICT_GRAM_END = 25,
    EV_PREDICT_SOLVE_END = 26,
    EV_PREDICT_END = 27,
    EV_GRAD_BEGIN = 28,
    EV_GRAD_END = 29,
    EV_FOLD_BEGIN = 30,
    EV_FOLD_END = 31,
    EV_CEI_BEGIN = 32,
    EV_CEI_END = 33,
    EV_LAST = EV_CEI_END
};
constexpr int ROBO_EVENT_SLOTS = EV_LAST + 1;
constexpr int ROBO_CHAIN_SLOTS = 16;
struct robo_ctx {
    int device;
    hipStream_t stream;
    bool own_stream;
    hipStream_t aux[ROBO_AUX_STREAMS];
    hipEvent_t ev_fork, ev_join[ROBO_AUX_STREAMS];
    bool aux_ready;
    int users;
    bool closing;
    hipEvent_t events[ROBO_EVENT_SLOTS];
    bool phase_events;
    char name[256];
    int num_cu;
    robo::Tuning tune;
    double* d_scalars;
    int* d_fail;
    unsigned* d_prog;
    double* h_pinned;
    robo::EpWork* ep;
    robo::McWork* mc;
    unsigned* h_chain;
    int chain_pending;
    bool chain_off;
};

namespace robo {
constexpr int WP_FRAGS = 144;
constexpr int WP_BLOCK = WP_FRAGS * 64;
__host__ __device__ constexpr int wp_offset(int cb) { return 4 * (36 - (cb + 1) * (cb + 2) / 2); }
}

struct robo_gp {
    robo_ctx* ctx;
    int kind, dim, n_max;
    int n;
    int n_pad;
    int n_pad_max;
    bool has_data, fitted;
    unsigned long long fit_gen;
    struct robo_cand* host_cand;
    bool fp32_gram;
    robo::CovParams cov;
    double amp, noise, mean_c;
    double y_mean, y_std;
    double loglik;
    double* d_X;
    double* d_Xs;
    double* d_y;
    double* d_K;
    double* d_Linv;
    double* d_LinvP;
    double* d_theta;
    robo::FitSample* d_sp;
    double x2max[robo::MAX_DIM];
    double* d_x2max;
    int b_cap, b_npad;
    double *d_bK, *d_bLinv, *d_bXs, *d_bism, *d_bout, *h_bstage;
    robo::FitSample* d_bsp;
    int* d_bfail;
    unsigned* d_bprog;
    double *d_llpart, *d_bllpart;
    char* d_bkeep;
    double *d_gV, *d_gA, *d_galpha, *d_gpart, *d_gout;
    char* d_mcmc;
    size_t mcmc_bytes;
    double* d_Winv;
    unsigned long long winv_gen;
    int* d_wunits[3];
    int* d_wprefix[3];
    int winv_units[3], winv_kc[3];
    int winv_nbk;
    double diag_min, diag_max;
    double winv_cond;
    double* d_wnorm;
    double* h_wnorm;
    unsigned long long winv_launched;
    robo::RefineWork* refine;
    robo::BatchWork* batch;
    robo::QeiWork* qei;
    robo::MesWork* mes;
    robo::RepWork* rep;
    robo::HyperWork* hyper;
    double* d_alpha;
    double dot_extent;
    double dot_alpha_sum;
    unsigned long long alpha_gen;
    unsigned long long screen_gen;
    int screen_skip, screen_backoff;
    int single_skip, single_backoff;
};

struct robo_cand {
    robo_ctx* ctx;
    int dim;
    int64_t m;
    int64_t m_pad;
    double* d_Xc;
    double* d_Xcs;
    double* d_V;
    int64_t chunk;
    const char* solve_kernel;
    int ldv;
    size_t v_bytes;
    const robo_gp* solved_gp;
    unsigned long long solved_gen;
    double* d_q;
    double* d_mu;
    double* d_mean;
    double* d_var;
    double* d_acq;
    double* d_acq_sum;
    double *d_S, *d_F, *d_Q, *d_G, *d_igc;
    size_t f_cap, q_cap, g_cap;
    double* d_kg;
    size_t kg_cap;
    double* h_igkey;
    size_t igkey_len;
    double* d_mu_all;
    double* d_var_all;
    int s_cap;
    double *d_Ks, *d_P, *d_qpart;
    size_t ks_bytes, p_bytes, qpart_bytes;
    double* d_part_val;
    long long* d_part_idx;
    unsigned* d_flags;
    int n_part;
    double *d_scr_up, *d_scr_lo;
    int* d_scr_cnt;
    long long* d_scr_map;
    struct robo_cand* scr_sub;
    robo::RefineWork* scr_probe;
    int64_t scr_cap;
    int64_t scr_n, scr_kept;
    int scr_outcome;
    const char* scr_bounds_kernel;
    int scr_finish;
    int scr_first_stage;
    int64_t scr_first_kept;
    bool scr_tail_fused;
    char* d_chain;
    size_t chain_bytes;
    bool defer_post;
    bool best_reported;
    size_t chain_cleared;
};

namespace robo {
inline bool phase_events_on(const robo_ctx* c, const robo_cand* k) { return c->phase_events || (k && k->m_pad > 16384); }
inline int record_phase(robo_ctx* c, int slot) {
    ROBO_HIP_CHECK(hipEventRecord(c->events[slot], c->stream));
    return ROBO_OK;
}
}

namespace robo {
int launch_scale_inputs(robo_ctx* ctx, const double* d_in, double* d_out, const double* d_inv_sqrt_metric,
                        int64_t rows_real, int64_t rows_pad, int dim, int S = 1, size_t out_stride = 0,
                        size_t ism_stride = 0, unsigned long long* d_word = nullptr, unsigned long long word_value = 0);
struct FitBuffers {
    double* K; size_t k_stride;
    double* Linv; size_t linv_stride;
    const double* Xs; size_t xs_stride;
    const FitSample* sp;
    int* fail;
    unsigned* prog;
    double* out;
    double* ll_part;
    double* LinvP;
    double* host_out;
    bool want_inverse;
    bool skip_tail;
    bool gram_mixed = true;
    int S;
};
int launch_scale_inputs_theta(robo_ctx* ctx, const double* d_in, double* d_out, const ThetaArgs& ta, int64_t rows_real,
                              int64_t rows_pad, int dim, double* d_ism_out, FitSample* d_sp_out);
struct KeepDst {
    double *K, *Linv, *LinvP, *Xs, *theta;
    double *X, *y;
    FitSample* sp;
    int ok;
};
int launch_batch_keep(robo_gp* g0, const KeepDst* d_dst, int ns);
int launch_gram(robo_gp* gp, const FitBuffers& fb, hipStream_t stream = nullptr, int s0 = 0, int ns = -1);
struct McmcState {
    int k, P, D, kind, n, n_steps, ns_eval, prior_kind;
    double a, mean_c;
    double prior_par[9];
    double *d_pos, *d_lnp, *d_q, *d_z, *d_prior;
    long long* d_nacc;
    int *d_it, *d_err;
    const double *d_uz, *d_ua;
    const int* d_partner;
    double *d_chain, *d_lnprob;
    FitSample* d_sp;
    double* d_ism;
    const double* d_x2max;
    const double* d_out;
    const int* d_fail;
};
int launch_mcmc_propose_scale(robo_ctx* ctx, const McmcState& st, int start, int first, int h, int it, const double* d_X,
                              double* d_Xs, int64_t rows_real, int64_t rows_pad, size_t xs_stride);
int launch_mcmc_accept(robo_ctx* ctx, const McmcState& st, int start, int first, int h, int it);
int launch_mcmc_tail(robo_ctx* ctx, const McmcState& st, int start, int first, int h, int it, const double* d_K, size_t k_stride,
                     int ld, int nbf, const int* d_fail);
int launch_mcmc_block_step(robo_gp* gp, const McmcState& st, int start, int first, int h, int it);
int launch_potrf(robo_gp* gp, const FitBuffers& fb, bool with_gram = false);
int launch_diag_timeline(robo_gp* gp, long long* d_stamps);
int launch_cross_gram(robo_gp* gp, robo_cand* cand, int64_t c0, int64_t cn, double* d_out = nullptr);
int winv_ensure(robo_gp* gp);
int winv_launch(robo_gp* gp);
int launch_per_cost(robo_ctx* ctx, double* d_dh, const double* d_log_cost, double overhead, int64_t m);
int launch_predict_winv(robo_gp* gp, robo_cand* cand, int64_t c0, int64_t cn, bool store_v);
int winv_rows_buffer(robo_gp* gp, robo_cand* cand, int64_t rows, double** out);
int launch_winv_rows(robo_gp* gp, robo_cand* cand, int64_t rows);
int launch_trsm(robo_gp* gp, robo_cand* cand, int64_t c0, int64_t cn);
int launch_predict_fused(robo_gp* gp, robo_cand* cand, int64_t c0, int64_t cn);
bool chain_wanted(const robo_gp* gp, int64_t cn);
int launch_predict_chain(robo_gp* gp, robo_cand* cand, int64_t c0, int64_t cn);
int chain_state_ensure(const robo_gp* gp, robo_cand* cand, int64_t cn, size_t* state_bytes_out);
bool chain_timed_out(robo_ctx* ctx);
int launch_pack_linv(robo_gp* gp);
int launch_grad_loglik(robo_gp* gp, double* d_V, double* d_A, double* d_alpha, double* d_part, double* d_out,
                       double* h_out);
int launch_triinv(robo_gp* gp, double* d_W, double* d_V);
struct GradBatch {
    const double* K; size_t k_stride;
    const double* Linv; size_t linv_stride;
    const double* Xs; size_t xs_stride;
    const FitSample* sp;
    double *V, *A;
    double *alpha, *part, *out;
    int S;
};
int launch_grad_loglik_batch(robo_gp* gp, const GradBatch& gb);
int launch_hyper_propose(robo_ctx* ctx, const HyperState& st, int t, const double* d_X, double* d_Xs, int64_t rows_real,
                         int64_t rows_pad, size_t xs_stride);
int launch_hyper_accept(robo_ctx* ctx, const HyperState& st, int t);
int launch_hyper_result(robo_ctx* ctx, const HyperState& st);
int launch_post(robo_gp* gp, robo_cand* cand, int64_t c0, int64_t cn);
int launch_cross_grad(robo_gp* gp, const double* d_Xcs, double* d_V, int64_t c_first, int64_t c_count, int64_t rows_pad);
int launch_predgrad_post(robo_gp* gp, const double* d_V, const double* d_q, const double* d_mu, const double* d_Xcs,
                         int64_t c_first, int64_t c_count, double* d_mean, double* d_var, double* d_dmean,
                         double* d_dvar);
int launch_refine_select(robo_ctx* ctx, const RefineState& st, const double* d_vals, int64_t m, const double* d_Xc,
                         double step0);
int launch_refine_eval(robo_gp* gp, const RefineState& st, const robo_cand* ws, int acq_kind, double par, double eta, int s,
                       int S, int t, int T);
int launch_refine_result(robo_ctx* ctx, const RefineState& st, unsigned* d_cand_flags, bool sweep_only);
int refine_ensure(robo_gp* g, int K, int D, RefineWork** out);
struct CeiRefineStep {
    bool objective, first, last;
    double thr;
    int C, kind, has_eta;
    double par, eta;
};
int launch_cei_refine_eval(robo_gp* gp, const RefineState& st, const robo_cand* ws, const CeiRefineStep& step, int t, int T);
int launch_batch_reset(robo_ctx* ctx, const BatchState& st);
int launch_batch_init(robo_gp* gp, const BatchState& st, const robo_cand* cand, int s, double eta);
int launch_batch_record(robo_ctx* ctx, const BatchState& st, const robo_cand* cand, int j, bool take_flags);
int launch_batch_condition(robo_gp* gp, const BatchState& st, const robo_cand* cand, int s, int j, int acq_kind, double par,
                           int fantasy_kind, double liar);
int launch_acq(robo_ctx* ctx, robo_cand* cand, int acq_kind, double par, double eta, bool accumulate, bool first);
int launch_argmax(robo_cand* cand, const double* d_vals, double scale);
int launch_report_best(robo_cand* cand, double* h_pinned);
int launch_acq_tail(robo_gp* gp, robo_cand* s, int acq_kind, double par, double eta, const long long* d_map, robo_cand* k,
                    double* h_report);
int launch_fwd_rows(robo_gp* gp, double* d_w, double* d_v, const int* d_stop);
int launch_bwd_rows(robo_gp* gp, double* d_v, double* d_beta, const int* d_stop = nullptr);
int launch_cov(robo_gp* gp, robo_cand* cand, double* d_cov);
int launch_mixture(robo_cand* cand, int S);
int launch_cross_cov(robo_gp* gp, robo_cand* cand, robo_cand* rep, int64_t c0, int64_t cn, double* d_S, bool clip = true);
int launch_kg(robo_ctx* ctx, const double* d_S, const double* d_var, const double* d_mean, const double* d_disc, int64_t m,
              int nb, double sn2, int include_self, bool first, double* d_acq_sum, unsigned* d_flags, double* d_trace);
int launch_ehvi(robo_ctx* ctx, const double* d_mean1, const double* d_var1, const double* d_mean2, const double* d_var2,
                const double* d_front, int P, double r1, double r2, int64_t m, double* d_out, unsigned* d_flags,
                double* d_trace);
struct CeiThresholds {
    double t[ROBO_CEI_MAX_CONSTRAINTS];
};
int launch_cei(robo_ctx* ctx, const double* d_mean0, const double* d_var0, const double* d_means, const double* d_vars,
               int64_t stride, int C, const CeiThresholds& th, int kind, double par, double eta, int has_eta, int64_t m,
               double* d_out, unsigned* d_flags, double* d_trace);
int launch_ig_dh(robo_ctx* ctx, const double* d_S, const double* d_var, double* d_F, double* d_Q, const double* d_G,
                 const double* d_consts, int64_t c0, int64_t cn, int64_t m, int nb, int npts, int kf, double sn2,
                 double H, double* d_out);
int mc_eval_gains(robo_ctx* c, int64_t m, int nb, int np, int nf, double sn2, const double* d_s, int lds,
                  const double* d_v, const double* Mb, const double* Vb, const double* logP, const double* lmb,
                  const double* W, const double* z, double* d_gain, int* d_counts, double* d_jit, unsigned* d_flags);
int launch_random_candidates(robo_ctx* ctx, double* d_out, int64_t m_pad, int dim, uint64_t seed, int64_t n_uniform,
                             const double* d_loc, const double* d_scale);
int launch_uniform(robo_ctx* ctx, double* d_out, int64_t m, int64_t m_pad, int dim, uint64_t seed);
int launch_sobol(robo_ctx* ctx, double* d_out, int64_t m, int64_t m_pad, int dim, const unsigned long long* d_sv,
                 const unsigned long long* d_shift, int bits, uint64_t first);
int launch_mfma_selftest(robo_ctx* ctx, double* out_err);
int launch_cov_rows_probe(robo_ctx* ctx, const CovParams& cp, const double* h_xi, const double* h_xj, long long n,
                          double* h_out);
int launch_stretch_probe(robo_ctx* ctx, const double* h_c, const double* h_s, const double* h_u, double a, int P, int n,
                         double* h_z, double* h_q, double* h_d);
int launch_gemm_microbench(robo_ctx* ctx, int variant, int wgs, int K, int reps, double* out_tflops);
int launch_clock_sampler(robo_ctx* ctx, int window_us);
int collect_clock_sampler(double* out3);
int launch_mfma_microbench(robo_ctx* ctx, int iters, double* out_tflops, double* out_cycles_per_mfma,
                           double* out_shader_mhz, double* out_chain);
}
```

robo_amd/csrc/diag/selftest.hip:

```cpp
#include "../common.h"
#include "../kern_math.h"
#include "../mcmc_dev.h"

namespace robo {

__global__ __launch_bounds__(64) void mfma_layout_kernel(const double* __restrict__ A, const double* __restrict__ B,
                                                         double* __restrict__ C) {
    const int l = threadIdx.x;
    v4d acc = {0.0, 0.0, 0.0, 0.0};
    acc = mfma_f64(A[(l & 15) * 4 + (l >> 4)], B[(l >> 4) * 16 + (l & 15)], acc);
#pragma unroll
    for (int r = 0; r < 4; ++r) C[((l >> 4) + 4 * r) * 16 + (l & 15)] = acc[r];
}

__global__ __launch_bounds__(256) void mfma_bench_kernel(double* __restrict__ sink, int iters, double seed,
                                                         long long* __restrict__ clocks) {
    const int l = threadIdx.x & 63;
    const long long t0 = clock64(), w0 = wall_clock64();
    const double a = seed + 1e-3 * l, b = seed - 1e-3 * l;
    v4d c0 = {0, 0, 0, 0}, c1 = {1, 1, 1, 1}, c2 = {2, 2, 2, 2}, c3 = {3, 3, 3, 3};
    v4d c4 = {0, 0, 0, 0}, c5 = {1, 1, 1, 1}, c6 = {2, 2, 2, 2}, c7 = {3, 3, 3, 3};
    for (int i = 0; i < iters; ++i) {
        c0 = mfma_f64(a, b, c0);
        c1 = mfma_f64(a, b, c1);
        c2 = mfma_f64(a, b, c2);
        c3 = mfma_f64(a, b, c3);
        c4 = mfma_f64(a, b, c4);
        c5 = mfma_f64(a, b, c5);
        c6 = mfma_f64(a, b, c6);
        c7 = mfma_f64(a, b, c7);
    }
    const v4d s = c0 + c1 + c2 + c3 + c4 + c5 + c6 + c7;
    if (s[0] + s[1] + s[2] + s[3] == 12345.678) sink[threadIdx.x] = s[0];
    const long long t1 = clock64(), w1 = wall_clock64();
    if (clocks && blockIdx.x == 0 && threadIdx.x == 0) {
        clocks[0] = t1 - t0;
        clocks[1] = w1 - w0;
    }
}

__global__ __launch_bounds__(64) void mfma_chain_kernel(double* __restrict__ sink, int iters, double seed,
                                                        long long* __restrict__ clocks) {
    const int l = threadIdx.x & 63;
    const double a = seed + 1e-3 * l, b = seed - 1e-3 * l;
    v4d c0 = {0, 0, 0, 0};
    const long long t0 = clock64();
    for (int i = 0; i < iters; ++i) {
        c0 = mfma_f64(a, b, c0);
        c0 = mfma_f64(a, b, c0);
        c0 = mfma_f64(a, b, c0);
        c0 = mfma_f64(a, b, c0);
    }
    if (c0[0] + c0[1] == 12345.678) sink[threadIdx.x] = c0[0];
    const long long t1 = clock64();
    if (threadIdx.x == 0) clocks[0] = t1 - t0;
}

__global__ __launch_bounds__(256) void stretch_q_probe_kernel(const double* __restrict__ c, const double* __restrict__ s,
                                                              const double* __restrict__ z, double* __restrict__ q, int n) {
    const int i = blockIdx.x * 256 + threadIdx.x;
    if (i < n) q[i] = mcmc_stretch_q(c[i], s[i], z[i]);
}
__global__ __launch_bounds__(256) void stretch_z_probe_kernel(const double* __restrict__ u, double a, double* __restrict__ z,
                                                              int n) {
    const int i = blockIdx.x * 256 + threadIdx.x;
    if (i < n) z[i] = mcmc_stretch_z(a, u[i]);
}
__global__ __launch_bounds__(256) void lnpdiff_probe_kernel(const double* __restrict__ lz, const double* __restrict__ lpn,
                                                            const double* __restrict__ lpo, int P, double* __restrict__ out,
                                                            int n) {
    const int i = blockIdx.x * 256 + threadIdx.x;
    if (i < n) out[i] = mcmc_lnpdiff(P, lz[i], lpn[i], lpo[i]);
}

int launch_stretch_probe(robo_ctx* ctx, const double* h_c, const double* h_s, const double* h_u, double a, int P, int n,
                         double* h_z, double* h_q, double* h_d) {
    double* d = nullptr;
    const size_t bytes = (size_t)n * sizeof(double);
    ROBO_HIP_CHECK(hipMalloc(&d, 6 * bytes));
    double *dc = d, *ds = d + n, *du = d + 2 * (size_t)n, *dz = d + 3 * (size_t)n, *dq = d + 4 * (size_t)n, *dd = d + 5 * (size_t)n;
    ROBO_HIP_CHECK(hipMemcpyAsync(dc, h_c, bytes, hipMemcpyHostToDevice, ctx->stream));
    ROBO_HIP_CHECK(hipMemcpyAsync(ds, h_s, bytes, hipMemcpyHostToDevice, ctx->stream));
    ROBO_HIP_CHECK(hipMemcpyAsync(du, h_u, bytes, hipMemcpyHostToDevice, ctx->stream));
    const int blocks = (n + 255) / 256;
    hipLaunchKernelGGL(stretch_z_probe_kernel, dim3(blocks), dim3(256), 0, ctx->stream, (const double*)du, a, dz, n);
    hipLaunchKernelGGL(stretch_q_probe_kernel, dim3(blocks), dim3(256), 0, ctx->stream, (const double*)dc, (const double*)ds,
                       (const double*)dz, dq, n);
    hipLaunchKernelGGL(lnpdiff_probe_kernel, dim3(blocks), dim3(256), 0, ctx->stream, (const double*)du, (const double*)dc,
                       (const double*)ds, P, dd, n);
    ROBO_LAUNCH_CHECK();
    ROBO_HIP_CHECK(hipMemcpyAsync(h_z, dz, bytes, hipMemcpyDeviceToHost, ctx->stream));
    ROBO_HIP_CHECK(hipMemcpyAsync(h_q, dq, bytes, hipMemcpyDeviceToHost, ctx->stream));
    ROBO_HIP_CHECK(hipMemcpyAsync(h_d, dd, bytes, hipMemcpyDeviceToHost, ctx->stream));
    ROBO_HIP_CHECK(hipStreamSynchronize(ctx->stream));
    ROBO_HIP_CHECK(hipFree(d));
    return ROBO_OK;
}

__global__ __launch_bounds__(256) void cov_rows_probe_kernel(CovParams cp, const double* __restrict__ xi,
                                                             const double* __restrict__ xj, double* __restrict__ out,
                                                             long long n) {
    const long long p = (long long)blockIdx.x * blockDim.x + threadIdx.x;
    if (p < n) out[p] = cov_rows(cp, xi + p * cp.dim, xj + p * cp.dim);
}

int launch_cov_rows_probe(robo_ctx* ctx, const CovParams& cp, const double* h_xi, const double* h_xj, long long n,
                          double* h_out) {
    const size_t rows = (size_t)n * cp.dim * sizeof(double), bytes = 2 * rows + (size_t)n * sizeof(double);
    double* d = nullptr;
    ROBO_HIP_CHECK(hipMalloc((void**)&d, bytes));
    double *dxi = d, *dxj = d + (size_t)n * cp.dim, *dout = dxj + (size_t)n * cp.dim;
    const int st = [&]() -> int {
        ROBO_HIP_CHECK(hipMemcpyAsync(dxi, h_xi, rows, hipMemcpyHostToDevice, ctx->stream));
        ROBO_HIP_CHECK(hipMemcpyAsync(dxj, h_xj, rows, hipMemcpyHostToDevice, ctx->stream));
        hipLaunchKernelGGL(cov_rows_probe_kernel, dim3((unsigned)((n + 255) / 256)), dim3(256), 0, ctx->stream, cp,
                           (const double*)dxi, (const double*)dxj, dout, n);
        ROBO_LAUNCH_CHECK();
        ROBO_HIP_CHECK(hipMemcpyAsync(h_out, dout, (size_t)n * sizeof(double), hipMemcpyDeviceToHost, ctx->stream));
        ROBO_HIP_CHECK(hipStreamSynchronize(ctx->stream));
        return ROBO_OK;
    }();
    hipFree(d);
    return st;
}

int launch_mfma_selftest(robo_ctx* ctx, double* out_err) {
    double hA[64], hB[64], hC[256];
    for (int i = 0; i < 64; ++i) {
        hA[i] = 0.25 * i + 1.0 + 0.01 * (i % 7);
        hB[i] = 3.0 - 0.125 * i + 0.02 * (i % 5);
    }
    double* d = nullptr;
    ROBO_HIP_CHECK(hipMalloc(&d, (64 + 64 + 256) * sizeof(double)));
    ROBO_HIP_CHECK(hipMemcpyAsync(d, hA, sizeof(hA), hipMemcpyHostToDevice, ctx->stream));
    ROBO_HIP_CHECK(hipMemcpyAsync(d + 64, hB, sizeof(hB), hipMemcpyHostToDevice, ctx->stream));
    hipLaunchKernelGGL(mfma_layout_kernel, dim3(1), dim3(64), 0, ctx->stream, (const double*)d,
                       (const double*)(d + 64), d + 128);
    ROBO_HIP_CHECK(hipMemcpyAsync(hC, d + 128, sizeof(hC), hipMemcpyDeviceToHost, ctx->stream));
    ROBO_HIP_CHECK(hipStreamSynchronize(ctx->stream));
    ROBO_HIP_CHECK(hipFree(d));
    double err = 0.0;
    for (int i = 0; i < 16; ++i)
        for (int j = 0; j < 16; ++j) {
            double s = 0.0;
            for (int k = 0; k < 4; ++k) s += hA[i * 4 + k] * hB[k * 16 + j];
            const double e = s - hC[i * 16 + j];
            if ((e < 0 ? -e : e) > err) err = e < 0 ? -e : e;
        }
    *out_err = err;
    return ROBO_OK;
}

int launch_mfma_microbench(robo_ctx* ctx, int iters, double* out_tflops, double* out_cycles_per_mfma,
                           double* out_shader_mhz, double* out_chain) {
    const int blocks = 4096;
    double* sink = nullptr;
    ROBO_HIP_CHECK(hipMalloc(&sink, (256 + 4) * sizeof(double)));
    long long* clocks = reinterpret_cast<long long*>(sink + 256);
    hipEvent_t e0, e1;
    ROBO_HIP_CHECK(hipEventCreate(&e0));
    ROBO_HIP_CHECK(hipEventCreate(&e1));
    hipLaunchKernelGGL(mfma_bench_kernel, dim3(blocks), dim3(256), 0, ctx->stream, sink, iters / 4 + 1, 0.5,
                       (long long*)nullptr);
    ROBO_HIP_CHECK(hipEventRecord(e0, ctx->stream));
    hipLaunchKernelGGL(mfma_bench_kernel, dim3(blocks), dim3(256), 0, ctx->stream, sink, iters, 0.5, clocks);
    ROBO_HIP_CHECK(hipEventRecord(e1, ctx->stream));
    ROBO_HIP_CHECK(hipEventSynchronize(e1));
    float ms = 0.f;
    ROBO_HIP_CHECK(hipEventElapsedTime(&ms, e0, e1));
    ROBO_HIP_CHECK(hipEventDestroy(e0));
    ROBO_HIP_CHECK(hipEventDestroy(e1));
    long long hclk[2] = {0, 0};
    ROBO_HIP_CHECK(hipMemcpy(hclk, clocks, sizeof(hclk), hipMemcpyDeviceToHost));
    if (out_shader_mhz) *out_shader_mhz = hclk[1] > 0 ? (double)hclk[0] / ((double)hclk[1] / 100.0) : 0.0;
    hipLaunchKernelGGL(mfma_bench_kernel, dim3(1), dim3(64), 0, ctx->stream, sink, iters, 0.5, clocks);
    ROBO_HIP_CHECK(hipStreamSynchronize(ctx->stream));
    ROBO_HIP_CHECK(hipMemcpy(hclk, clocks, sizeof(hclk), hipMemcpyDeviceToHost));
    if (out_cycles_per_mfma) *out_cycles_per_mfma = (double)hclk[0] / ((double)iters * 8.0);
    hipLaunchKernelGGL(mfma_chain_kernel, dim3(1), dim3(64), 0, ctx->stream, sink, iters, 0.5, clocks);
    ROBO_HIP_CHECK(hipStreamSynchronize(ctx->stream));
    ROBO_HIP_CHECK(hipMemcpy(hclk, clocks, sizeof(hclk), hipMemcpyDeviceToHost));
    ROBO_HIP_CHECK(hipFree(sink));
    if (out_chain) *out_chain = (double)hclk[0] / ((double)iters * 4.0);
    const double flops = (double)blocks * 4.0 * (double)iters * 8.0 * 2048.0;
    *out_tflops = flops / ((double)ms * 1e-3) / 1e12;
    return ROBO_OK;
}

}
```

robo_amd/csrc/screen.hip:

```cpp
#include <cmath>

#include "api_internal.h"
#include "kern_math.h"

namespace robo {

constexpr double SCREEN_DELTA_REL = 1e-11;
constexpr double SCREEN_RHO = 1e-5;
constexpr double SCREEN_DIAG_RATIO_MAX = 1e4;
constexpr int SCREEN_PROBE = NB;
constexpr int SCREEN_DOT_MAX_D = 32;
constexpr double SCREEN_DOT_SAFETY = 4.0;
constexpr double SCREEN_DOT_BOUND = GRAM_DIRECT_BOUND;

constexpr int SC_CAND = 64;
constexpr int SC_ROWS = 32;
constexpr int SC_LD = NB + 2;

__global__ __launch_bounds__(256) void screen_alpha_norm_kernel(const double* __restrict__ alpha, const double* __restrict__ Xs,
                                                                CovParams cp, int n, double* __restrict__ out) {
    __shared__ double sh[256];
    double a = 0.0;
    for (int j = threadIdx.x; j < n; j += 256)
        a += fabs(alpha[j]) * sqrt(fabs(cov_self(cp, Xs[(size_t)j * cp.dim + cp.dim - 1])));
    sh[threadIdx.x] = a;
    __syncthreads();
    for (int o = 128; o > 0; o >>= 1) {
        if ((int)threadIdx.x < o) sh[threadIdx.x] += sh[threadIdx.x + o];
        __syncthreads();
    }
    if (threadIdx.x == 0) out[0] = sh[0];
}

__device__ __forceinline__ double screen_widen(double x, double sign, double abs_term) {
    return isfinite(x) ? x + sign * SCREEN_RHO * (fabs(x) + abs_term) : x;
}

__device__ __forceinline__ void screen_bounds(int kind, double par, double eta, double m, double delta, double v_prior,
                                              double& up, double& lo) {
    const double eps = 2.220446049250313e-16;
    double v_hi = v_prior < eps ? eps : v_prior;
    v_hi = v_hi * (1.0 + SCREEN_RHO);
    const double v_lo = eps;
    const double m_lo = m - delta, m_hi = m + delta;
    if (kind == ROBO_ACQ_EI) {
        up = acq_ei(m_lo, v_hi, eta, par);
        lo = acq_ei(m_hi, v_lo, eta, par);
        if (up < 0.0 && up > -2.2250738585072014e-308) up = 0.0;
        if (lo < 0.0 && lo > -2.2250738585072014e-308) lo = 0.0;
        up = screen_widen(up, 1.0, 0.0);
        lo = screen_widen(lo, -1.0, 0.0);
    } else if (kind == ROBO_ACQ_LOG_EI) {
        up = screen_widen(acq_log_ei(m_lo, v_hi, eta, par), 1.0, 1.0);
        lo = screen_widen(acq_log_ei(m_hi, v_lo, eta, par), -1.0, 1.0);
    } else if (kind == ROBO_ACQ_PI) {
        up = (eta - m_lo - par >= 0.0) ? 1.0 : screen_widen(acq_pi(m_lo, v_hi, eta, par), 1.0, 0.0);
        lo = screen_widen(acq_pi(m_hi, (eta - m_hi - par >= 0.0) ? v_hi : v_lo, eta, par), -1.0, 0.0);
    } else {
        up = acq_lcb(m_lo, v_hi, par);
        lo = acq_lcb(m_hi, v_lo, par);
    }
}

__device__ __forceinline__ unsigned long long screen_key(double x) {
    const unsigned long long u = (unsigned long long)__double_as_longlong(x);
    return (u >> 63) ? ~u : (u | 0x8000000000000000ull);
}
__device__ __forceinline__ double screen_unkey(unsigned long long k) {
    return __longlong_as_double((long long)((k >> 63) ? (k & 0x7FFFFFFFFFFFFFFFull) : ~k));
}
constexpr unsigned long long SCREEN_KEY_NONE = 0x000FFFFFFFFFFFFFull;

__device__ __forceinline__ double screen_block_max(double x, double* sh) {
    for (int o = 32; o > 0; o >>= 1) {
        const double y = __shfl_xor(x, o);
        x = y > x ? y : x;
    }
    if ((threadIdx.x & 63) == 0) sh[threadIdx.x >> 6] = x;
    __syncthreads();
    double r = sh[0];
    for (int w = 1; w < 4; ++w) r = sh[w] > r ? sh[w] : r;
    return r;
}

template <int KIND, bool SMALLD>
__global__ __launch_bounds__(256) void screen_bounds_kernel(const double* __restrict__ Xcs, const double* __restrict__ Xs,
                                                            const double* __restrict__ alpha,
                                                            const double* __restrict__ alpha_norm, CovParams cp, int n,
                                                            long long m, double mean_c, double y_mean, double y_std,
                                                            int acq_kind, double par, double eta, double* __restrict__ up,
                                                            double* __restrict__ lo, unsigned long long* __restrict__ bkey) {
    __shared__ double sX[16 * SC_LD];
    __shared__ double sA[NB];
    __shared__ double sP[4][SC_CAND];
    const int tid = threadIdx.x, lane = tid & 63, wave = tid >> 6, D = cp.dim;
    const long long i = (long long)blockIdx.x * SC_CAND + lane;
    const bool live = i < m;
    const long long ii = live ? i : 0;
    double xc[16];
    if (SMALLD) {
#pragma unroll
        for (int d = 0; d < 16; ++d) xc[d] = d < D ? Xcs[ii * D + d] : 0.0;
    }
    const int nbk = (n + NB - 1) / NB;
    double dot = 0.0;
    for (int tile = 0; tile < nbk; ++tile) {
        double acc[SC_ROWS], uu[SC_ROWS];
#pragma unroll
        for (int r = 0; r < SC_ROWS; ++r) cov_init<double, KIND>(cp, acc[r], uu[r]);
        for (int d0 = 0; d0 < D; d0 += 16) {
            __syncthreads();
#pragma unroll
            for (int e = 0; e < 8; ++e) {
                const int idx = tid + e * 256, row = idx >> 4, d = idx & 15;
                const int rg = tile * NB + row;
                sX[d * SC_LD + row] = (d0 + d < D && rg < n) ? Xs[(size_t)rg * D + d0 + d] : 0.0;
            }
            if (d0 == 0 && tid < NB) sA[tid] = tile * NB + tid < n ? alpha[tile * NB + tid] : 0.0;
            __syncthreads();
            const int dn = D - d0 < 16 ? D - d0 : 16;
            const double* sx = sX + wave * SC_ROWS;
            if (SMALLD) {
#pragma unroll
                for (int d = 0; d < 16; ++d) {
                    if (d < dn) {
#pragma unroll
                        for (int r = 0; r < SC_ROWS; ++r)
                            cov_step<double, KIND>(cp, d, xc[d], sx[d * SC_LD + r], acc[r], uu[r]);
                    }
                }
            } else {
                for (int d = 0; d < dn; ++d) {
                    const double xi = Xcs[ii * D + d0 + d];
#pragma unroll
                    for (int r = 0; r < SC_ROWS; ++r)
                        cov_step<double, KIND>(cp, d0 + d, xi, sx[d * SC_LD + r], acc[r], uu[r]);
                }
            }
        }
#pragma unroll
        for (int r = 0; r < SC_ROWS; ++r) {
            const double kv = cov_finish<double, KIND>(cp, acc[r], uu[r]);
            if (tile * NB + wave * SC_ROWS + r < n) dot = fma(kv, sA[wave * SC_ROWS + r], dot);
        }
    }
    sP[wave][lane] = dot;
    __syncthreads();
    if (wave != 0) return;
    double lmax = -__builtin_huge_val();
    if (live) {
        const double mu = (sP[0][lane] + sP[1][lane]) + (sP[2][lane] + sP[3][lane]);
        const double kself = cov_self(cp, Xcs[i * D + D - 1]);
        double mt = mu + mean_c;
        mt = mt * y_std + y_mean;
        const double v_prior = kself * (y_std * y_std);
        const double delta = SCREEN_DELTA_REL * (fabs(y_mean) + fabs(y_std) * (fabs(mean_c) + sqrt(fabs(kself)) * alpha_norm[0]));
        double u, l;
        screen_bounds(acq_kind, par, eta, mt, delta, v_prior, u, l);
        up[i] = u;
        lo[i] = l;
        if (!isnan(l)) lmax = l;
    }
    for (int o = 32; o > 0; o >>= 1) {
        const double y = __shfl_xor(lmax, o);
        lmax = y > lmax ? y : lmax;
    }
    if (lane == 0) atomicMax(bkey, screen_key(lmax));
}

template <int N>
__device__ __forceinline__ double screen_block_reduce(double x, double* sh, int op) {
    __syncthreads();
    sh[threadIdx.x] = x;
    __syncthreads();
    for (int o = N / 2; o > 0; o >>= 1) {
        if ((int)threadIdx.x < o) {
            const double y = sh[threadIdx.x + o];
            sh[threadIdx.x] = op == 0 ? sh[threadIdx.x] + y : (y > sh[threadIdx.x] ? y : sh[threadIdx.x]);
        }
        __syncthreads();
    }
    return sh[0];
}

constexpr int SD_CTR = 4;
__global__ __launch_bounds__(256) void screen_dot_prep_kernel(const double* __restrict__ alpha, const double* __restrict__ Xs,
                                                              int D, int n, double* __restrict__ st) {
    __shared__ double sh[256];
    __shared__ double sc[SCREEN_DOT_MAX_D];
    const double inf = __builtin_huge_val();
    double ext = 0.0;
    for (int d = 0; d < D; ++d) {
        double hi = -inf, nlo = -inf;
        for (int j = threadIdx.x; j < n; j += 256) {
            const double x = Xs[(size_t)j * D + d];
            hi = x > hi ? x : hi;
            nlo = -x > nlo ? -x : nlo;
        }
        hi = screen_block_reduce<256>(hi, sh, 1);
        nlo = screen_block_reduce<256>(nlo, sh, 1);
        const double c = 0.5 * (hi - nlo), h = hi - c, l = c + nlo;
        ext += fmax(h * h, l * l);
        if (threadIdx.x == 0) sc[d] = c;
    }
    __syncthreads();
    double a = 0.0, r = 0.0;
    for (int j = threadIdx.x; j < n; j += 256) {
        a += fabs(alpha[j]);
        double s = 0.0;
        for (int d = 0; d < D; ++d) {
            const double b = Xs[(size_t)j * D + d] - sc[d];
            s = fma(b, b, s);
        }
        r = s > r ? s : r;
    }
    a = screen_block_reduce<256>(a, sh, 0);
    r = screen_block_reduce<256>(r, sh, 1);
    if (threadIdx.x == 0) {
        st[1] = a;
        st[2] = r;
        st[3] = ext;
    }
    if ((int)threadIdx.x < D) st[SD_CTR + threadIdx.x] = sc[threadIdx.x];
}

__global__ __launch_bounds__(256) void screen_dot_pack_kernel(const double* __restrict__ alpha, const double* __restrict__ Xs,
                                                              const double* __restrict__ st, double amp, int D, int ks, int n,
                                                              double* __restrict__ rows, double* __restrict__ apack) {
    const int tile = blockIdx.x * 4 + (threadIdx.x >> 6), l = threadIdx.x & 63, g = l >> 4;
    const int row = tile * 16 + (l & 15);
    const bool real = row < n;
    double nb = 0.0;
    if (real)
        for (int d = 0; d < D; ++d) {
            const double b = Xs[(size_t)row * D + d] - st[SD_CTR + d];
            nb = fma(b, b, nb);
        }
    for (int kk = 0; kk < ks; ++kk) {
        const int k = 4 * kk + g;
        double v = 0.0;
        if (real && k < D) v = -2.0 * (Xs[(size_t)row * D + k] - st[SD_CTR + k]);
        rows[((size_t)tile * ks + kk) * 64 + l] = v;
    }
    if (l < 16) {
        const int slot = (tile >> 3) * 2 * NB + (tile & 7) * 16 + (l & 3) * 4 + (l >> 2);
        apack[slot] = real ? amp * alpha[row] : 0.0;
        apack[slot + NB] = nb;
    }
}

constexpr double SD_R2_MIN = 1e-290;
template <int KIND>
__device__ __forceinline__ void screen_dot_finish(const v4d acc, double nc, const double* __restrict__ al, double (&dot)[4]) {
    double x[4], q[4];
#pragma unroll
    for (int r = 0; r < 4; ++r) {
        if (KIND == ROBO_KERNEL_MATERN52_ARD) {
            const double t = fmax(fma(5.0, acc[r], nc), 5.0 * SD_R2_MIN);
            double y = __builtin_amdgcn_rsq(t);
            const double e = fma(-t * y, y, 1.0);
            y = fma(y * e, fma(e, 0.375, 0.5), y);
            const double s0 = t * y;
            const double s = fma(fma(-s0, s0, t), 0.5 * y, s0);
            x[r] = -s;
            q[r] = fma(t, 1.0 / 3.0, 1.0 + s);
        } else {
            x[r] = fmin(fma(-0.5, acc[r], nc), -0.5 * SD_R2_MIN);
            q[r] = 1.0;
        }
    }
    double nn[4], rr[4], p[4];
#pragma unroll
    for (int r = 0; r < 4; ++r) {
        nn[r] = rint(x[r] * 1.4426950408889634074);
        rr[r] = fma(nn[r], -6.93147180369123816490e-01, x[r]);
        rr[r] = fma(nn[r], -1.90821492927058770002e-10, rr[r]);
        p[r] = 2.08767569878680989792e-09;
    }
#define ROBO_SD_HORNER(C)                                     \
    _Pragma("unroll") for (int r = 0; r < 4; ++r) p[r] = fma(p[r], rr[r], C)
    ROBO_SD_HORNER(2.50521083854417187751e-08);
    ROBO_SD_HORNER(2.75573192239858906526e-07);
    ROBO_SD_HORNER(2.75573192239858906526e-06);
    ROBO_SD_HORNER(2.48015873015873015873e-05);
    ROBO_SD_HORNER(1.98412698412698412698e-04);
    ROBO_SD_HORNER(1.38888888888888888889e-03);
    ROBO_SD_HORNER(8.33333333333333333333e-03);
    ROBO_SD_HORNER(4.16666666666666666667e-02);
    ROBO_SD_HORNER(1.66666666666666666667e-01);
    ROBO_SD_HORNER(0.5);
    ROBO_SD_HORNER(1.0);
    ROBO_SD_HORNER(1.0);
#undef ROBO_SD_HORNER
#pragma unroll
    for (int r = 0; r < 4; ++r) {
        double kv = ldexp(p[r], (int)nn[r]);
        if (KIND == ROBO_KERNEL_MATERN52_ARD) kv *= q[r];
        dot[r] = fma(kv, al[r], dot[r]);
    }
}

constexpr double SD_LEAN_EPS = 8e-13;
constexpr double SCREEN_LEAN_SAFETY = 1e4;
constexpr double SCREEN_LEAN_MAX = 1e-2;
template <int KIND>
__device__ __forceinline__ void screen_dot_finish_lean(const v4d acc, double nc, const double* __restrict__ al, double (&dot)[4]) {
    double x[4], q[4];
#pragma unroll
    for (int r = 0; r < 4; ++r) {
        if (KIND == ROBO_KERNEL_MATERN52_ARD) {
            const double t = fmax(fma(5.0, acc[r], nc), 5.0 * SD_R2_MIN);
            double y = __builtin_amdgcn_rsq(t);
            const double e = fma(-t * y, y, 1.0);
            y = fma(y * e, fma(e, 0.375, 0.5), y);
            const double s = t * y;
            x[r] = -s;
            q[r] = fma(t, 1.0 / 3.0, 1.0 + s);
        } else {
            x[r] = fmin(fma(-0.5, acc[r], nc), -0.5 * SD_R2_MIN);
            q[r] = 1.0;
        }
    }
    double nn[4], rr[4], p[4];
#pragma unroll
    for (int r = 0; r < 4; ++r) {
        nn[r] = rint(x[r] * 1.4426950408889634074);
        rr[r] = fma(nn[r], -6.93147180559945286e-01, x[r]);
        p[r] = 2.47270673012491639e-05;
    }
#define ROBO_SD_HORNER(C)                                     \
    _Pragma("unroll") for (int r = 0; r < 4; ++r) p[r] = fma(p[r], rr[r], C)
    ROBO_SD_HORNER(1.99155698002864343e-04);
    ROBO_SD_HORNER(1.38891798039418699e-03);
    ROBO_SD_HORNER(8.33326676781509339e-03);
    ROBO_SD_HORNER(4.16666642053601585e-02);
    ROBO_SD_HORNER(1.66666668867537560e-01);
    ROBO_SD_HORNER(5.00000000062317818e-01);
    ROBO_SD_HORNER(9.99999999980468957e-01);
    ROBO_SD_HORNER(9.99999999999759970e-01);
#undef ROBO_SD_HORNER
#pragma unroll
    for (int r = 0; r < 4; ++r) {
        double kv = ldexp(p[r], (int)nn[r]);
        if (KIND == ROBO_KERNEL_MATERN52_ARD) kv *= q[r];
        dot[r] = fma(kv, al[r], dot[r]);
    }
}

constexpr double SD_SINGLE_EPS = 6.3e-7;
constexpr double SCREEN_SINGLE_SAFETY = 1.5;
constexpr double SCREEN_SINGLE_MAX = 0.5;
template <int KIND>
__device__ __forceinline__ void screen_dot_finish_single(const v4d acc, double nc, const double* __restrict__ al, double (&dot)[4]) {
#pragma unroll
    for (int r = 0; r < 4; ++r) {
        float kv;
        if (KIND == ROBO_KERNEL_MATERN52_ARD) {
            const float t = (float)fmax(fma(5.0, acc[r], nc), 5.0 * SD_R2_MIN);
            const float s = hw_sqrt_f32(t);
            const float q = fmaf(t, 0.333333333f, 1.0f + s);
            kv = q * hw_exp2_f32(s * -1.44269504f);
        } else {
            const float x = (float)fmin(fma(-0.5, acc[r], nc), -0.5 * SD_R2_MIN);
            kv = hw_exp2_f32(x * 1.44269504f);
        }
        dot[r] = fma((double)kv, al[r], dot[r]);
    }
}

enum ScreenFinish { SD_FULL = 0, SD_LEAN = 1, SD_SINGLE = 2 };

constexpr int SD_CAND = 64;
constexpr int SD_STAGE = NB;

template <int KIND, int KS, ScreenFinish FINISH>
__global__ __launch_bounds__(256) void screen_bounds_dot_kernel(const double* __restrict__ Xcs, const double* __restrict__ Xs,
                                                                const double* __restrict__ alpha,
                                                                const double* __restrict__ alpha_norm, CovParams cp, int n,
                                                                long long m, double mean_c, double y_mean, double y_std,
                                                                int acq_kind, double par, double eta, double* __restrict__ up,
                                                                double* __restrict__ lo, unsigned long long* __restrict__ bkey) {
    __shared__ double sMx[4];
    constexpr int TILES = SD_STAGE / 16, STAGE_DOUBLES = TILES * KS * 64, PER = STAGE_DOUBLES / 256;
    __shared__ double sA[STAGE_DOUBLES];
    __shared__ __attribute__((aligned(32))) double sAN[2 * SD_STAGE];
    const double *sAl = sAN, *sNj = sAN + SD_STAGE;
    const int tid = threadIdx.x, lane = tid & 63, wave = tid >> 6, g = lane >> 4, D = cp.dim;
    const long long i = (long long)blockIdx.x * SD_CAND + wave * 16 + (lane & 15);
    const bool live = i < m;
    const long long ii = live ? i : 0;
    double b[KS], nc = 0.0;
#pragma unroll
    for (int kk = 0; kk < KS; ++kk) {
        const int k = 4 * kk + g;
        b[kk] = k < D ? Xcs[ii * D + k] - alpha_norm[SD_CTR + k] : 0.0;
        nc = fma(b[kk], b[kk], nc);
    }
    nc += __shfl_xor(nc, 16);
    nc += __shfl_xor(nc, 32);
    const double ncf = KIND == ROBO_KERNEL_MATERN52_ARD ? 5.0 * nc : -0.5 * nc;
    const int nst = (n + SD_STAGE - 1) / SD_STAGE;
    double pa[PER];
#pragma unroll
    for (int e = 0; e < PER; ++e) pa[e] = Xs[e * 256 + tid];
    double pan = alpha[tid];
    double dot[4] = {0.0, 0.0, 0.0, 0.0};
    for (int s = 0; s < nst; ++s) {
        __syncthreads();
#pragma unroll
        for (int e = 0; e < PER; ++e) sA[e * 256 + tid] = pa[e];
        sAN[tid] = pan;
        __syncthreads();
        if (s + 1 < nst) {
            const double* nx = Xs + (size_t)(s + 1) * STAGE_DOUBLES;
#pragma unroll
            for (int e = 0; e < PER; ++e) pa[e] = nx[e * 256 + tid];
            pan = alpha[(s + 1) * 2 * SD_STAGE + tid];
        }
        const double* nj = sNj + g * 4;
        v4d acc = v4d{nj[0], nj[1], nj[2], nj[3]};
#pragma unroll
        for (int kk = 0; kk < KS; ++kk) acc = mfma_f64(sA[kk * 64 + lane], b[kk], acc);
#pragma unroll
        for (int t = 0; t < TILES; ++t) {
            v4d nxt = acc;
            if (t + 1 < TILES) {
                nj += 16;
                nxt = v4d{nj[0], nj[1], nj[2], nj[3]};
#pragma unroll
                for (int kk = 0; kk < KS; ++kk) nxt = mfma_f64(sA[((t + 1) * KS + kk) * 64 + lane], b[kk], nxt);
            }
            if (FINISH == SD_SINGLE) screen_dot_finish_single<KIND>(acc, ncf, sAl + t * 16 + g * 4, dot);
            else if (FINISH == SD_LEAN) screen_dot_finish_lean<KIND>(acc, ncf, sAl + t * 16 + g * 4, dot);
            else screen_dot_finish<KIND>(acc, ncf, sAl + t * 16 + g * 4, dot);
            acc = nxt;
        }
    }
    double mu = (dot[0] + dot[1]) + (dot[2] + dot[3]);
    mu += __shfl_xor(mu, 16);
    mu += __shfl_xor(mu, 32);
    double lmax = -__builtin_huge_val();
    if (g == 0 && live) {
        const double kself = cp.amp;
        double mt = mu + mean_c;
        mt = mt * y_std + y_mean;
        const double v_prior = kself * (y_std * y_std);
        const double ck = KIND == ROBO_KERNEL_MATERN52_ARD ? 5.0 / 6.0 : 0.5;
        const double r2_err = (double)(4 * KS + 6) * 4.44089209850062616e-16 * (nc + alpha_norm[2]);
        double delta = SCREEN_DELTA_REL * (fabs(y_mean) + fabs(y_std) * (fabs(mean_c) + sqrt(fabs(kself)) * alpha_norm[0])) +
                       SCREEN_DOT_SAFETY * fabs(y_std) * fabs(cp.amp) * ck * r2_err * alpha_norm[1];
        if (FINISH != SD_FULL) delta += SCREEN_LEAN_SAFETY * SD_LEAN_EPS * fabs(y_std) * fabs(cp.amp) * alpha_norm[1];
        if (FINISH == SD_SINGLE) delta += SCREEN_SINGLE_SAFETY * SD_SINGLE_EPS * fabs(y_std) * fabs(cp.amp) * alpha_norm[1];
        double u, l;
        screen_bounds(acq_kind, par, eta, mt, delta, v_prior, u, l);
        up[i] = u;
        lo[i] = l;
        if (!isnan(l)) lmax = l;
    }
    lmax = screen_block_max(lmax, sMx);
    if (tid == 0) atomicMax(bkey, screen_key(lmax));
}

__device__ __forceinline__ bool screen_survives(const double* __restrict__ up, long long c, long long m, double b) {
    return c < m && !(up[c] < b);
}

__device__ __forceinline__ void screen_scan(int* cnt, int n_part, double b, double* __restrict__ host) {
    __shared__ int s[256];
    __shared__ int carry;
    const int t = threadIdx.x;
    if (t == 0) carry = 0;
    __syncthreads();
    for (int base = 0; base < n_part; base += 256) {
        const int x = base + t < n_part ? cnt[base + t] : 0;
        s[t] = x;
        __syncthreads();
        for (int o = 1; o < 256; o <<= 1) {
            const int y = t >= o ? s[t - o] : 0;
            __syncthreads();
            s[t] += y;
            __syncthreads();
        }
        const int c0 = carry;
        if (base + t < n_part) cnt[base + t] = c0 + s[t] - x;
        __syncthreads();
        if (t == 255) carry = c0 + s[255];
        __syncthreads();
    }
    if (t == 0) {
        cnt[n_part] = carry;
        host[0] = (double)carry;
        host[1] = b;
    }
}

__global__ __launch_bounds__(256) void screen_count_scan_kernel(const double* __restrict__ up, long long m,
                                                                const unsigned long long* __restrict__ bkey, int* cnt,
                                                                int n_part, double* __restrict__ host) {
    __shared__ int sw[4];
    __shared__ int last;
    const double b = screen_unkey(*bkey);
    const long long c = (long long)blockIdx.x * 256 + threadIdx.x;
    const unsigned long long mask = __ballot(screen_survives(up, c, m, b) ? 1 : 0);
    if ((threadIdx.x & 63) == 0) sw[threadIdx.x >> 6] = __builtin_popcountll(mask);
    __syncthreads();
    if (threadIdx.x == 0) {
        cnt[blockIdx.x] = (sw[0] + sw[1]) + (sw[2] + sw[3]);
        __threadfence();
        last = atomicAdd(cnt + n_part + 1, 1) == n_part - 1;
    }
    __syncthreads();
    if (!last) return;
    __threadfence();
    screen_scan(cnt, n_part, b, host);
    if (threadIdx.x == 0) cnt[n_part + 1] = 0;
}

__global__ __launch_bounds__(256) void screen_gather_kernel(const double* __restrict__ up, long long m,
                                                            const unsigned long long* __restrict__ bkey,
                                                            const int* __restrict__ cnt, const double* __restrict__ Xcs, int dim,
                                                            long long rows, long long cap, double* __restrict__ sub_Xcs,
                                                            long long* __restrict__ map, unsigned* __restrict__ clear,
                                                            long long clear_words) {
    __shared__ int sw[4];
    __shared__ long long first;
    for (long long e = (long long)blockIdx.x * 256 + threadIdx.x; e < clear_words; e += (long long)gridDim.x * 256) clear[e] = 0u;
    const int lane = threadIdx.x & 63, wave = threadIdx.x >> 6;
    const long long c = (long long)blockIdx.x * 256 + threadIdx.x;
    const bool keep = screen_survives(up, c, m, screen_unkey(*bkey));
    const unsigned long long mask = __ballot(keep ? 1 : 0);
    if (lane == 0) sw[wave] = __builtin_popcountll(mask);
    if (threadIdx.x == 0) first = -1;
    __syncthreads();
    if (keep) {
        int before = __builtin_popcountll(mask & ((1ull << lane) - 1ull));
        for (int w = 0; w < wave; ++w) before += sw[w];
        const long long dst = (long long)cnt[blockIdx.x] + before;
        if (dst < cap) {
            map[dst] = c;
            for (int d = 0; d < dim; ++d) sub_Xcs[dst * dim + d] = Xcs[c * dim + d];
            if (dst == 0) first = c;
        }
    }
    __syncthreads();
    const long long c0 = first;
    if (c0 < 0) return;
    const long long total = (cap - rows) * dim;
    for (long long e = threadIdx.x; e < total; e += 256) sub_Xcs[rows * dim + e] = Xcs[c0 * dim + e % dim];
}

__global__ void screen_map_best_kernel(const double* __restrict__ sub_val, const long long* __restrict__ sub_idx,
                                       unsigned* __restrict__ sub_flags, const long long* __restrict__ map,
                                       double* __restrict__ best_val, long long* __restrict__ best_idx,
                                       unsigned* __restrict__ flags) {
    if (threadIdx.x != 0 || blockIdx.x != 0) return;
    *best_val = *sub_val;
    *best_idx = *sub_idx < 0 ? *sub_idx : map[*sub_idx];
    *flags |= *sub_flags;
    *sub_flags = 0u;
}

__global__ void screen_probe_bound_kernel(const double* __restrict__ vals, const RefineSel* __restrict__ sel, int kind,
                                          unsigned long long* __restrict__ bkey, unsigned* __restrict__ probe_flags) {
    if (threadIdx.x != 0 || blockIdx.x != 0) return;
    double best = -__builtin_huge_val();
    const int keff = (int)sel->keff;
    for (int i = 0; i < keff; ++i)
        if (vals[i] > best) best = vals[i];
    if (kind != ROBO_ACQ_LCB) best = screen_widen(best, -1.0, kind == ROBO_ACQ_LOG_EI ? 1.0 : 0.0);
    if (best > screen_unkey(*bkey)) *bkey = screen_key(best);
    *probe_flags = 0u;
}

static bool screen_kind_ok(int kind, double par, double eta) {
    if (!std::isfinite(par)) return false;
    if (kind == ROBO_ACQ_LCB) return par >= 0.0;
    return (kind == ROBO_ACQ_EI || kind == ROBO_ACQ_LOG_EI || kind == ROBO_ACQ_PI) && std::isfinite(eta);
}

static int screen_dot_ks(const robo_gp* g) {
    if ((g->kind != ROBO_KERNEL_MATERN52_ARD && g->kind != ROBO_KERNEL_RBF_ARD) || g->dim > SCREEN_DOT_MAX_D) return 0;
    return g->dim <= 4 ? 1 : g->dim <= 8 ? 2 : g->dim <= 16 ? 4 : 8;
}

static int alpha_ensure(robo_gp* g) {
    const size_t np = (size_t)g->n_pad_max;
    const int ks = screen_dot_ks(g);
    const size_t dot_doubles = ks ? SD_CTR + SCREEN_DOT_MAX_D + 2 * np + np * 4 * (size_t)ks : 0;
    if (!g->d_alpha) ROBO_TRY(dev_alloc(&g->d_alpha, 2 * np + 8 + dot_doubles));
    if (g->alpha_gen == g->fit_gen) return ROBO_OK;
    robo_ctx* c = g->ctx;
    hipStream_t st = c->stream;
    double* v = g->d_alpha;
    double* a = g->d_alpha + np;
    ROBO_HIP_CHECK(hipMemcpyAsync(v, g->d_K + (size_t)g->n * g->n_pad, (size_t)g->n * sizeof(double), hipMemcpyDeviceToDevice, st));
    ROBO_TRY(launch_bwd_rows(g, v, a));
    double* stats = g->d_alpha + 2 * np;
    hipLaunchKernelGGL(screen_alpha_norm_kernel, dim3(1), dim3(256), 0, st, (const double*)a, (const double*)g->d_Xs, g->cov,
                       g->n, stats);
    g->dot_extent = g->dot_alpha_sum = 0.0;
    if (ks) {
        double* apack = stats + SD_CTR + SCREEN_DOT_MAX_D;
        const int nst = (g->n + SD_STAGE - 1) / SD_STAGE;
        hipLaunchKernelGGL(screen_dot_prep_kernel, dim3(1), dim3(256), 0, st, (const double*)a, (const double*)g->d_Xs, g->dim,
                           g->n, stats);
        hipLaunchKernelGGL(screen_dot_pack_kernel, dim3((unsigned)(nst * SD_STAGE / 64)), dim3(256), 0, st, (const double*)a,
                           (const double*)g->d_Xs, (const double*)stats, g->cov.amp, g->dim, ks, g->n, apack + 2 * np, apack);
        ROBO_LAUNCH_CHECK();
        double* hp = c->h_pinned + MAX_DIM + 16;
        ROBO_HIP_CHECK(hipMemcpyAsync(hp, stats + 1, 3 * sizeof(double), hipMemcpyDeviceToHost, st));
        ROBO_HIP_CHECK(hipStreamSynchronize(st));
        g->dot_alpha_sum = hp[0];
        g->dot_extent = hp[2];
    }
    ROBO_LAUNCH_CHECK();
    g->alpha_gen = g->fit_gen;
    return ROBO_OK;
}

static bool screen_dot_wanted(const robo_gp* g) {
    const int t = g->ctx->tune.acq_screen_dot;
    if (t == 0 || !screen_dot_ks(g)) return false;
    if (t > 0) return true;
    const double worst = (double)(g->dim + 3) * 4.44089209850062616e-16 * g->dot_extent;
    return worst <= SCREEN_DOT_BOUND;
}

static bool screen_lean_wanted(const robo_gp* g) {
    const int t = g->ctx->tune.acq_screen_lean;
    if (t == 0) return false;
    if (t > 0) return true;
    const double term = SCREEN_LEAN_SAFETY * SD_LEAN_EPS * std::sqrt(std::fabs(g->cov.amp)) * g->dot_alpha_sum;
    return term <= SCREEN_LEAN_MAX;
}

static bool screen_single_wanted(const robo_gp* g) {
    const int t = g->ctx->tune.acq_screen_single;
    if (t == 0 || !screen_dot_wanted(g) || !screen_lean_wanted(g)) return false;
    if (t > 0) return true;
    const double term = SCREEN_SINGLE_SAFETY * SD_SINGLE_EPS * std::sqrt(std::fabs(g->cov.amp)) * g->dot_alpha_sum;
    return term <= SCREEN_SINGLE_MAX;
}

static int screen_buffers(robo_cand* k) {
    const size_t mp = (size_t)k->m_pad;
    if (!k->d_scr_up) ROBO_TRY(dev_alloc(&k->d_scr_up, mp));
    if (!k->d_scr_lo) ROBO_TRY(dev_alloc(&k->d_scr_lo, mp + 2));
    if (!k->d_scr_cnt) {
        ROBO_TRY(dev_alloc(&k->d_scr_cnt, (size_t)k->n_part + 2));
        ROBO_HIP_CHECK(hipMemsetAsync(k->d_scr_cnt, 0, ((size_t)k->n_part + 2) * sizeof(int), k->ctx->stream));
    }
    return ROBO_OK;
}

static int launch_screen_bounds(robo_gp* g, robo_cand* k, int kind, double par, double eta, bool single = false) {
    robo_ctx* c = g->ctx;
    ROBO_TRY(alpha_ensure(g));
    ROBO_TRY(screen_buffers(k));
    unsigned long long* bkey = reinterpret_cast<unsigned long long*>(k->d_scr_lo + k->m_pad);
    ROBO_TRY(launch_scale_inputs(c, k->d_Xc, k->d_Xcs, g->d_theta, k->m, k->m_pad, g->dim, 1, 0, 0, bkey, SCREEN_KEY_NONE));
    const dim3 grid((unsigned)((k->m + SC_CAND - 1) / SC_CAND));
    const double* alpha = g->d_alpha + (size_t)g->n_pad_max;
    const double* anorm = g->d_alpha + 2 * (size_t)g->n_pad_max;
    if (screen_dot_wanted(g)) {
        const double* apack = anorm + SD_CTR + SCREEN_DOT_MAX_D;
        const double* rows = apack + 2 * (size_t)g->n_pad_max;
        const dim3 dgrid((unsigned)((k->m + SD_CAND - 1) / SD_CAND));
#define ROBO_SCREEN_DOT_CALL(KIND, KS, LEAN)                                                                                  \
    hipLaunchKernelGGL((screen_bounds_dot_kernel<KIND, KS, LEAN>), dgrid, dim3(256), 0, c->stream, (const double*)k->d_Xcs, rows,  \
                       apack, anorm, g->cov, g->n, (long long)k->m, g->mean_c, g->y_mean, g->y_std, kind, par, eta,          \
                       k->d_scr_up, k->d_scr_lo, bkey)
#define ROBO_SCREEN_DOT_KS(KIND, LEAN)                            \
    switch (screen_dot_ks(g)) {                                   \
        case 1: ROBO_SCREEN_DOT_CALL(KIND, 1, LEAN); break;       \
        case 2: ROBO_SCREEN_DOT_CALL(KIND, 2, LEAN); break;       \
        case 4: ROBO_SCREEN_DOT_CALL(KIND, 4, LEAN); break;       \
        default: ROBO_SCREEN_DOT_CALL(KIND, 8, LEAN); break;      \
    }
        const bool lean = screen_lean_wanted(g);
        if (g->kind == ROBO_KERNEL_MATERN52_ARD) {
            if (single) ROBO_SCREEN_DOT_KS(ROBO_KERNEL_MATERN52_ARD, SD_SINGLE)
            else if (lean) ROBO_SCREEN_DOT_KS(ROBO_KERNEL_MATERN52_ARD, SD_LEAN)
            else ROBO_SCREEN_DOT_KS(ROBO_KERNEL_MATERN52_ARD, SD_FULL)
        } else {
            if (single) ROBO_SCREEN_DOT_KS(ROBO_KERNEL_RBF_ARD, SD_SINGLE)
            else if (lean) ROBO_SCREEN_DOT_KS(ROBO_KERNEL_RBF_ARD, SD_LEAN)
            else ROBO_SCREEN_DOT_KS(ROBO_KERNEL_RBF_ARD, SD_FULL)
        }
#undef ROBO_SCREEN_DOT_KS
#undef ROBO_SCREEN_DOT_CALL
        ROBO_LAUNCH_CHECK();
        k->scr_bounds_kernel = "screen_bounds_dot_kernel";
        k->scr_finish = lean ? ROBO_SCREEN_FINISH_LEAN : ROBO_SCREEN_FINISH_FULL;
        return ROBO_OK;
    }
    k->scr_bounds_kernel = "screen_bounds_kernel";
    k->scr_finish = ROBO_SCREEN_FINISH_NONE;
#define ROBO_SCREEN_CALL(KIND)                                                                                           \
    do {                                                                                                                  \
        if (g->dim <= 16)                                                                                                 \
            hipLaunchKernelGGL((screen_bounds_kernel<KIND, true>), grid, dim3(256), 0, c->stream, (const double*)k->d_Xcs, \
                               (const double*)g->d_Xs, alpha, anorm, g->cov, g->n, (long long)k->m, g->mean_c, g->y_mean, \
                               g->y_std, kind, par, eta, k->d_scr_up, k->d_scr_lo, bkey);                                     \
        else                                                                                                              \
            hipLaunchKernelGGL((screen_bounds_kernel<KIND, false>), grid, dim3(256), 0, c->stream, (const double*)k->d_Xcs, \
                               (const double*)g->d_Xs, alpha, anorm, g->cov, g->n, (long long)k->m, g->mean_c, g->y_mean, \
                               g->y_std, kind, par, eta, k->d_scr_up, k->d_scr_lo, bkey);                                     \
    } while (0)
    if (g->kind == ROBO_KERNEL_MATERN52_ARD) ROBO_SCREEN_CALL(ROBO_KERNEL_MATERN52_ARD);
    else if (g->kind == ROBO_KERNEL_RBF_ARD) ROBO_SCREEN_CALL(ROBO_KERNEL_RBF_ARD);
    else ROBO_SCREEN_CALL(ROBO_KERNEL_FABOLAS);
#undef ROBO_SCREEN_CALL
    ROBO_LAUNCH_CHECK();
    return ROBO_OK;
}

static bool screen_eligible(const robo_gp* g, const robo_cand* k, int kind, double par, double eta) {
    if (!g || !k || !g->fitted || k->dim != g->dim || k->ctx != g->ctx) return false;
    const Tuning& t = g->ctx->tune;
    if (t.acq_screen == 0 || !screen_kind_ok(kind, par, eta)) return false;
    if (k->m <= (t.acq_screen_min >= 0 ? t.acq_screen_min : t.winv_max)) return false;
    if (g->fp32_gram || t.predict_stepwise || winv_candidate(g, k)) return false;
    return g->diag_min > 0.0 && g->diag_max <= SCREEN_DIAG_RATIO_MAX * g->diag_min;
}

static int screen_sub(robo_cand* k, int64_t cap) {
    if (cap < SCREEN_PROBE) cap = SCREEN_PROBE;
    if (k->scr_sub && k->scr_cap >= cap) return ROBO_OK;
    robo_cand_destroy(k->scr_sub);
    hipFree(k->d_scr_map);
    k->scr_sub = nullptr;
    k->d_scr_map = nullptr;
    k->scr_cap = 0;
    ROBO_TRY(cand_alloc(k->ctx, cap, k->dim, &k->scr_sub));
    ROBO_TRY(dev_alloc(&k->d_scr_map, (size_t)k->scr_sub->m_pad));
    k->scr_cap = cap;
    return ROBO_OK;
}

int acq_sweep_best(robo_gp* g, int32_t kind, double par, double eta, robo_cand* k, bool want_values, bool allow_chain,
                   double* h_report) {
    if (k) {
        k->best_reported = false;
        k->scr_outcome = ROBO_SCREEN_NOT_ELIGIBLE;
        k->scr_n = k->scr_kept = 0;
        k->scr_tail_fused = false;
        k->scr_first_stage = 0;
        k->scr_first_kept = 0;
    }
    if (want_values || !screen_eligible(g, k, kind, par, eta)) return acq_sweep(&g, 1, false, kind, par, &eta, k, allow_chain);
    if (g->screen_gen != g->fit_gen) {
        g->screen_gen = g->fit_gen;
        g->screen_skip = 0;
        g->screen_backoff = 1;
        g->single_skip = 0;
        g->single_backoff = 1;
    }
    if (g->screen_skip > 0) {
        --g->screen_skip;
        return acq_sweep(&g, 1, false, kind, par, &eta, k, allow_chain);
    }
    robo_ctx* c = g->ctx;
    hipStream_t st = c->stream;
    ROBO_HIP_CHECK(hipSetDevice(c->device));
    k->solved_gen = 0;
    ROBO_TRY(alpha_ensure(g));
    bool first = screen_single_wanted(g);
    if (first && g->single_skip > 0) {
        --g->single_skip;
        first = false;
    }
    ROBO_TRY(launch_screen_bounds(g, k, kind, par, eta, first));
    unsigned long long* b = reinterpret_cast<unsigned long long*>(k->d_scr_lo + k->m_pad);
    double* hp = c->h_pinned + 8;
    const dim3 blocks((unsigned)k->n_part);
    int64_t kept = 0;
    auto count_survivors = [&]() -> int {
        hipLaunchKernelGGL(screen_count_scan_kernel, blocks, dim3(256), 0, st, (const double*)k->d_scr_up, (long long)k->m,
                           (const unsigned long long*)b, k->d_scr_cnt, k->n_part, hp);
        ROBO_LAUNCH_CHECK();
        ROBO_HIP_CHECK(hipStreamSynchronize(st));
        kept = (int64_t)hp[0];
        return ROBO_OK;
    };
    ROBO_TRY(count_survivors());
    int64_t cap = k->m / 100 * c->tune.acq_screen_keep_max + k->m % 100 * c->tune.acq_screen_keep_max / 100;
    if (cap > k->m) cap = k->m;
    if (cap < 1) cap = 1;
    if (first) {
        k->scr_first_kept = kept;
        if (kept >= 1 && kept <= (cap < NB ? cap : (int64_t)NB)) {
            k->scr_first_stage = 1;
            g->single_backoff = 1;
        } else {
            k->scr_first_stage = 2;
            g->single_skip = g->single_backoff;
            if (g->single_backoff < (1 << 20)) g->single_backoff *= 2;
            ROBO_TRY(launch_screen_bounds(g, k, kind, par, eta));
            ROBO_TRY(count_survivors());
        }
    }
    k->scr_n = k->m;
    k->scr_kept = kept;
    bool probed = false;
    if (kept > cap) {
        ROBO_TRY(screen_sub(k, cap));
        if (!k->scr_probe) ROBO_TRY(refine_alloc(c, SCREEN_PROBE, k->dim, &k->scr_probe));
        const RefineState& ps = k->scr_probe->st;
        robo_cand* s = k->scr_sub;
        ROBO_TRY(launch_refine_select(c, ps, k->d_scr_up, k->m, k->d_Xcs, 0.0));
        s->m = s->m_pad = SCREEN_PROBE;
        s->n_part = 1;
        s->solved_gen = 0;
        ROBO_HIP_CHECK(hipMemcpyAsync(s->d_Xcs, ps.x, (size_t)SCREEN_PROBE * k->dim * sizeof(double), hipMemcpyDeviceToDevice, st));
        ROBO_TRY(cand_ensure_workspace(s, g->n_pad, false));
        ROBO_TRY(predict_scaled(g, s, false, nullptr, false, false, allow_chain));
        ROBO_TRY(clear_flags_on_error(s, launch_acq(c, s, kind, par, eta, false, false)));
        hipLaunchKernelGGL(screen_probe_bound_kernel, dim3(1), dim3(64), 0, st, (const double*)s->d_acq,
                           (const RefineSel*)ps.sel, kind, b, s->d_flags);
        ROBO_LAUNCH_CHECK();
        ROBO_TRY(count_survivors());
        if (allow_chain && chain_timed_out(c)) return clear_flags_on_error(s, ROBO_CHAIN_RETRY);
        k->scr_kept = kept;
        probed = true;
    }
    if (kept < 1 || kept > cap) {
        k->scr_outcome = ROBO_SCREEN_FELL_BACK;
        g->screen_skip = g->screen_backoff;
        if (g->screen_backoff < (1 << 20)) g->screen_backoff *= 2;
        return acq_sweep(&g, 1, false, kind, par, &eta, k, allow_chain);
    }
    g->screen_backoff = 1;
    k->scr_outcome = probed ? ROBO_SCREEN_PROBE_USED : ROBO_SCREEN_SCREENED;
    ROBO_TRY(screen_sub(k, cap));
    robo_cand* s = k->scr_sub;
    s->m = kept;
    s->m_pad = round_up64(kept, NB);
    s->n_part = (int)((kept + 255) / 256);
    s->solved_gen = 0;
    ROBO_TRY(cand_ensure_workspace(s, g->n_pad, false));
    unsigned* clear = nullptr;
    size_t clear_bytes = 0;
    s->chain_cleared = 0;
    if (allow_chain && s->chunk >= s->m_pad && !g->fp32_gram && !c->tune.predict_stepwise && chain_wanted(g, s->m_pad)) {
        ROBO_TRY(chain_state_ensure(g, s, s->m_pad, &clear_bytes));
        clear = reinterpret_cast<unsigned*>(s->d_chain);
    }
    hipLaunchKernelGGL(screen_gather_kernel, blocks, dim3(256), 0, st, (const double*)k->d_scr_up, (long long)k->m,
                       (const unsigned long long*)b, (const int*)k->d_scr_cnt, (const double*)k->d_Xcs, k->dim, (long long)kept,
                       (long long)s->m_pad, s->d_Xcs, k->d_scr_map, clear, (long long)(clear_bytes / sizeof(unsigned)));
    ROBO_LAUNCH_CHECK();
    s->chain_cleared = clear_bytes;
    const bool fused = c->tune.acq_screen_fused_tail != 0 && s->n_part == 1 && s->m_pad <= 256;
    s->defer_post = fused;
    const int solved = predict_scaled(g, s, false, nullptr, false, phase_events_on(g->ctx, k), allow_chain);
    s->chain_cleared = 0;
    s->defer_post = false;
    ROBO_TRY(solved);
    int status = fused ? launch_acq_tail(g, s, kind, par, eta, k->d_scr_map, k, h_report) : launch_acq(c, s, kind, par, eta, false, false);
    if (fused) {
        k->scr_tail_fused = true;
        if (status == ROBO_OK) k->best_reported = h_report != nullptr;
    } else if (status == ROBO_OK) {
        hipLaunchKernelGGL(screen_map_best_kernel, dim3(1), dim3(64), 0, st, (const double*)(s->d_part_val + s->n_part),
                           (const long long*)(s->d_part_idx + s->n_part), s->d_flags, (const long long*)k->d_scr_map,
                           k->d_part_val + k->n_part, k->d_part_idx + k->n_part, k->d_flags);
        if (hipGetLastError() != hipSuccess) status = ROBO_RUNTIME_ERROR;
    }
    if (status != ROBO_OK) clear_flags_on_error(s, status);
    k->solve_kernel = s->solve_kernel;
    return clear_flags_on_error(k, status);
}

}

using namespace robo;

extern "C" {

int32_t robo_cand_last_screen(robo_cand* k, int64_t* out_n_screened, int64_t* out_n_survivors, int32_t* out_outcome) {
    if (!k) return ROBO_BAD_ARGUMENT;
    if (out_n_screened) *out_n_screened = k->scr_n;
    if (out_n_survivors) *out_n_survivors = k->scr_kept;
    if (out_outcome) *out_outcome = k->scr_outcome;
    return ROBO_OK;
}

int32_t robo_cand_last_screen_finish(robo_cand* k, int32_t* out_finish, int32_t* out_fused_tail) {
    if (!k || !out_finish) return ROBO_BAD_ARGUMENT;
    *out_finish = k->scr_finish;
    if (out_fused_tail) *out_fused_tail = k->scr_tail_fused ? 1 : 0;
    return ROBO_OK;
}

int32_t robo_cand_last_screen_first(robo_cand* k, int32_t* out_stage, int64_t* out_kept) {
    if (!k) return ROBO_BAD_ARGUMENT;
    if (out_stage) *out_stage = k->scr_first_stage;
    if (out_kept) *out_kept = k->scr_first_kept;
    return ROBO_OK;
}

int32_t robo_acq_screen_bounds(robo_gp* g, int32_t acq_kind, double par, double eta, robo_cand* k, double* out_upper,
                               double* out_lower) {
    if (!g || !k) return ROBO_BAD_ARGUMENT;
    ROBO_TRY(check_acq_kind(acq_kind));
    if (!g->fitted) {
        set_error("Model has to be trained first!");
        return ROBO_NOT_FITTED;
    }
    if (k->dim != g->dim || k->ctx != g->ctx) {
        set_error("candidate batch (dim %d) does not match the GP (dim %d) or lives on another context", k->dim, g->dim);
        return ROBO_BAD_SHAPE;
    }
    if (g->fp32_gram || !screen_kind_ok(acq_kind, par, eta)) {
        set_error("robo_acq_screen_bounds: no bound for this call (LCB needs kappa >= 0; finite eta / par; fp64 covariance "
                  "entries)");
        return ROBO_BAD_ARGUMENT;
    }
    hipStream_t st = g->ctx->stream;
    ROBO_HIP_CHECK(hipSetDevice(g->ctx->device));
    k->solved_gen = 0;
    ROBO_TRY(alpha_ensure(g));
    ROBO_TRY(launch_screen_bounds(g, k, acq_kind, par, eta, g->ctx->tune.acq_screen_single == 2 && screen_single_wanted(g)));
    if (out_upper)
        ROBO_HIP_CHECK(hipMemcpyAsync(out_upper, k->d_scr_up, (size_t)k->m * sizeof(double), hipMemcpyDeviceToHost, st));
    if (out_lower)
        ROBO_HIP_CHECK(hipMemcpyAsync(out_lower, k->d_scr_lo, (size_t)k->m * sizeof(double), hipMemcpyDeviceToHost, st));
    ROBO_HIP_CHECK(hipStreamSynchronize(st));
    return ROBO_OK;
}

}
```

Before: 127.1 million.

## Add int8 MFMA screening path for single-precision screen bounds

Result: faster. 147.2 million, median of 6 (+15.9%).

```diff
diff --git a/include/robo_hip.h b/include/robo_hip.h
--- a/include/robo_hip.h
+++ b/include/robo_hip.h
@@ -123,6 +123,9 @@
 #define ROBO_SCREEN_FINISH_LEAN 2
 int32_t robo_cand_last_screen_finish(robo_cand* cand, int32_t* out_finish, int32_t* out_fused_tail);
 int32_t robo_cand_last_screen_first(robo_cand* cand, int32_t* out_stage, int64_t* out_kept);
+#define ROBO_SCREEN_FORM_FP64 0
+#define ROBO_SCREEN_FORM_INT8 1
+int32_t robo_cand_last_screen_form(robo_cand* cand, int32_t* out_form, double* out_step);
 int32_t robo_acq_screen_bounds(robo_gp* gp, int32_t acq_kind, double par, double eta, robo_cand* cand, double* out_upper,
                                double* out_lower);
 int32_t robo_acq_eval_moments(robo_ctx* ctx, int32_t acq_kind, double par, double eta, const double* mean,
diff --git a/robo_amd/_lib.py b/robo_amd/_lib.py
--- a/robo_amd/_lib.py
+++ b/robo_amd/_lib.py
@@ -43,7 +43,8 @@
     "robo_cand_create_random", "robo_cand_create_sobol", "robo_cand_get_point", "robo_cand_workspace_chunk", "robo_cand_last_solve_kernel",
     "robo_gp_predict_cand", "robo_gp_predict", "robo_gp_predict_cov", "robo_gp_predict_grad", "robo_gp_predict_mixture_cand",
     "robo_acq_eval_cand", "robo_acq_eval", "robo_acq_eval_moments", "robo_acq_eval_marginal_cand", "robo_acq_eval_sum_cand",
-    "robo_cand_last_screen", "robo_cand_last_screen_finish", "robo_cand_last_screen_first", "robo_acq_screen_bounds",
+    "robo_cand_last_screen", "robo_cand_last_screen_finish", "robo_cand_last_screen_first", "robo_cand_last_screen_form",
+    "robo_acq_screen_bounds",
     "robo_acq_refine_cand", "robo_acq_refine_marginal_cand",
     "robo_rep_sample", "robo_rep_sample_batch",
     "robo_acq_batch_cand", "robo_acq_batch_marginal_cand", "robo_qei_batch_cand", "robo_qei_batch_marginal_cand",
@@ -204,6 +205,7 @@
         "robo_cand_last_screen": [vp, C.POINTER(i64), C.POINTER(i64), C.POINTER(i32)],
         "robo_cand_last_screen_finish": [vp, C.POINTER(i32), C.POINTER(i32)],
         "robo_cand_last_screen_first": [vp, C.POINTER(i32), C.POINTER(i64)],
+        "robo_cand_last_screen_form": [vp, C.POINTER(i32), C.POINTER(C.c_double)],
         "robo_acq_screen_bounds": [vp, i32, dbl, dbl, vp, _dp, _dp],
         "robo_acq_eval_moments": [vp, i32, dbl, dbl, _dp, _dp, i64, _dp, _dp, C.POINTER(i64), C.POINTER(C.c_uint32)],
         "robo_acq_eval_marginal_cand": [pp, i32, i32, dbl, _dp, vp, _dp, _dp, C.POINTER(i64),
@@ -620,6 +622,11 @@
         check(lib().robo_cand_last_screen_first(self._h, C.byref(stage), C.byref(kept)))
         return int(stage.value), int(kept.value)
 
+    def screen_form(self):
+        form, step = C.c_int32(0), C.c_double(0.0)
+        check(lib().robo_cand_last_screen_form(self._h, C.byref(form), C.byref(step)))
+        return int(form.value), float(step.value)
+
     def last_screen(self):
         n, kept, outcome = C.c_int64(0), C.c_int64(0), C.c_int32(0)
         check(lib().robo_cand_last_screen(self._h, C.byref(n), C.byref(kept), C.byref(outcome)))
diff --git a/robo_amd/csrc/api_ctx.hip b/robo_amd/csrc/api_ctx.hip
--- a/robo_amd/csrc/api_ctx.hip
+++ b/robo_amd/csrc/api_ctx.hip
@@ -64,6 +64,7 @@
     {"acq_screen_dot", nullptr, &Tuning::acq_screen_dot, -1},
     {"acq_screen_lean", nullptr, &Tuning::acq_screen_lean, -1},
     {"acq_screen_single", nullptr, &Tuning::acq_screen_single, -1},
+    {"acq_screen_int", nullptr, &Tuning::acq_screen_int, -1},
     {"acq_screen_fused_tail", nullptr, &Tuning::acq_screen_fused_tail, 1},
     {"trsm_chain", nullptr, &Tuning::trsm_chain, -1},
     {"trsm_chain_max_wg", nullptr, &Tuning::trsm_chain_max_wg, 4},
diff --git a/robo_amd/csrc/common.h b/robo_amd/csrc/common.h
--- a/robo_amd/csrc/common.h
+++ b/robo_amd/csrc/common.h
@@ -19,6 +19,36 @@
 
 __device__ __forceinline__ v4d mfma_f64(double a, double b, v4d c) {
     return __builtin_amdgcn_mfma_f64_16x16x4f64(a, b, c, 0, 0, 0);
+}
+
+typedef int v4i __attribute__((vector_size(16)));
+
+__device__ __forceinline__ int dot_i8x8(long long x, long long y) {
+    int s = 0;
+    for (int j = 0; j < 8; ++j) s += (int)(signed char)(x >> (8 * j)) * (int)(signed char)(y >> (8 * j));
+    return s;
+}
+
+__device__ __forceinline__ v4i mfma_i8(v4i a, v4i b, v4i c) {
+#ifdef __AMDGCN__
+    return __builtin_amdgcn_mfma_i32_16x16x64_i8(a, b, c, 0, 0, 0);
+#else
+    const int l = threadIdx.x & 63;
+    const long long a0 = (long long)(((unsigned long long)(unsigned)a[1] << 32) | (unsigned)a[0]);
+    const long long a1 = (long long)(((unsigned long long)(unsigned)a[3] << 32) | (unsigned)a[2]);
+    const long long b0 = (long long)(((unsigned long long)(unsigned)b[1] << 32) | (unsigned)b[0]);
+    const long long b1 = (long long)(((unsigned long long)(unsigned)b[3] << 32) | (unsigned)b[2]);
+    v4i d = c;
+    for (int gk = 0; gk < 4; ++gk) {
+        const long long y0 = __shfl(b0, (l & 15) + 16 * gk), y1 = __shfl(b1, (l & 15) + 16 * gk);
+        for (int r = 0; r < 4; ++r) {
+            const int src = 4 * (l >> 4) + r + 16 * gk;
+            const long long x0 = __shfl(a0, src), x1 = __shfl(a1, src);
+            d[r] += dot_i8x8(x0, y0) + dot_i8x8(x1, y1);
+        }
+    }
+    return d;
+#endif
 }
 
 __device__ __forceinline__ double rn_add(double a, double b) {
@@ -191,6 +221,7 @@
     int acq_screen_dot;
     int acq_screen_lean;
     int acq_screen_single;
+    int acq_screen_int;
     int acq_screen_fused_tail;
     int trsm_chain;
     int trsm_chain_max_wg;
@@ -484,6 +515,7 @@
     double* d_alpha;
     double dot_extent;
     double dot_alpha_sum;
+    double int_step, int_eps;
     unsigned long long alpha_gen;
     unsigned long long screen_gen;
     int screen_skip, screen_backoff;
@@ -537,6 +569,8 @@
     int scr_finish;
     int scr_first_stage;
     int64_t scr_first_kept;
+    int scr_int;
+    double scr_int_step;
     bool scr_tail_fused;
     char* d_chain;
     size_t chain_bytes;
diff --git a/robo_amd/csrc/diag/selftest.hip b/robo_amd/csrc/diag/selftest.hip
--- a/robo_amd/csrc/diag/selftest.hip
+++ b/robo_amd/csrc/diag/selftest.hip
@@ -11,6 +11,22 @@
     acc = mfma_f64(A[(l & 15) * 4 + (l >> 4)], B[(l >> 4) * 16 + (l & 15)], acc);
 #pragma unroll
     for (int r = 0; r < 4; ++r) C[((l >> 4) + 4 * r) * 16 + (l & 15)] = acc[r];
+}
+
+__global__ __launch_bounds__(64) void mfma_i8_layout_kernel(const signed char* __restrict__ A, const signed char* __restrict__ B,
+                                                            int* __restrict__ C) {
+    const int l = threadIdx.x;
+    v4i a = {0, 0, 0, 0}, b = {0, 0, 0, 0}, c;
+    for (int j = 0; j < 16; ++j) {
+        const int k = 16 * (l >> 4) + j;
+        a[j >> 2] |= ((int)A[(l & 15) * 64 + k] & 255) << (8 * (j & 3));
+        b[j >> 2] |= ((int)B[k * 16 + (l & 15)] & 255) << (8 * (j & 3));
+    }
+#pragma unroll
+    for (int r = 0; r < 4; ++r) c[r] = C[(4 * (l >> 4) + r) * 16 + (l & 15)];
+    c = mfma_i8(a, b, c);
+#pragma unroll
+    for (int r = 0; r < 4; ++r) C[(4 * (l >> 4) + r) * 16 + (l & 15)] = c[r];
 }
 
 __global__ __launch_bounds__(256) void mfma_bench_kernel(double* __restrict__ sink, int iters, double seed,
@@ -145,6 +161,30 @@
             double s = 0.0;
             for (int k = 0; k < 4; ++k) s += hA[i * 4 + k] * hB[k * 16 + j];
             const double e = s - hC[i * 16 + j];
+            if ((e < 0 ? -e : e) > err) err = e < 0 ? -e : e;
+        }
+    signed char iA[16 * 64], iB[64 * 16];
+    int iC[256], iD[256];
+    for (int i = 0; i < 16 * 64; ++i) {
+        iA[i] = (signed char)((i * 37 + (i >> 6) * 11 + 5) % 256 - 128);
+        iB[i] = (signed char)((i * 91 + (i & 15) * 7 + 200) % 256 - 128);
+    }
+    for (int i = 0; i < 256; ++i) iC[i] = 1000 * (i >> 4) - 7 * (i & 15) - 3;
+    char* di = nullptr;
+    ROBO_HIP_CHECK(hipMalloc(&di, sizeof(iA) + sizeof(iB) + sizeof(iC)));
+    ROBO_HIP_CHECK(hipMemcpyAsync(di, iA, sizeof(iA), hipMemcpyHostToDevice, ctx->stream));
+    ROBO_HIP_CHECK(hipMemcpyAsync(di + sizeof(iA), iB, sizeof(iB), hipMemcpyHostToDevice, ctx->stream));
+    ROBO_HIP_CHECK(hipMemcpyAsync(di + sizeof(iA) + sizeof(iB), iC, sizeof(iC), hipMemcpyHostToDevice, ctx->stream));
+    hipLaunchKernelGGL(mfma_i8_layout_kernel, dim3(1), dim3(64), 0, ctx->stream, (const signed char*)di,
+                       (const signed char*)(di + sizeof(iA)), reinterpret_cast<int*>(di + sizeof(iA) + sizeof(iB)));
+    ROBO_HIP_CHECK(hipMemcpyAsync(iD, di + sizeof(iA) + sizeof(iB), sizeof(iD), hipMemcpyDeviceToHost, ctx->stream));
+    ROBO_HIP_CHECK(hipStreamSynchronize(ctx->stream));
+    ROBO_HIP_CHECK(hipFree(di));
+    for (int i = 0; i < 16; ++i)
+        for (int j = 0; j < 16; ++j) {
+            int s = iC[i * 16 + j];
+            for (int k = 0; k < 64; ++k) s += (int)iA[i * 64 + k] * (int)iB[k * 16 + j];
+            const double e = (double)s - (double)iD[i * 16 + j];
             if ((e < 0 ? -e : e) > err) err = e < 0 ? -e : e;
         }
     *out_err = err;
diff --git a/robo_amd/csrc/screen.hip b/robo_amd/csrc/screen.hip
--- a/robo_amd/csrc/screen.hip
+++ b/robo_amd/csrc/screen.hip
@@ -184,12 +184,19 @@
 }
 
 constexpr int SD_CTR = 4;
+constexpr int SD_INT = SD_CTR + SCREEN_DOT_MAX_D;
+constexpr int SD_STATS = SD_INT + 4;
+constexpr int SD_INT_MAX_D = 16;
+constexpr double SD_INT_AMAX = 8355711.0;
+constexpr double SD_INT_GRID = 8355000.0;
+constexpr double SD_INT_OFF = 1048576.0 / 2;
+constexpr double SD_INT_H0 = 0.5;
 __global__ __launch_bounds__(256) void screen_dot_prep_kernel(const double* __restrict__ alpha, const double* __restrict__ Xs,
-                                                              int D, int n, double* __restrict__ st) {
+                                                              int D, int n, int matern, double* __restrict__ st) {
     __shared__ double sh[256];
     __shared__ double sc[SCREEN_DOT_MAX_D];
     const double inf = __builtin_huge_val();
-    double ext = 0.0;
+    double ext = 0.0, H = 0.0;
     for (int d = 0; d < D; ++d) {
         double hi = -inf, nlo = -inf;
         for (int j = threadIdx.x; j < n; j += 256) {
@@ -201,6 +208,7 @@
         nlo = screen_block_reduce<256>(nlo, sh, 1);
         const double c = 0.5 * (hi - nlo), h = hi - c, l = c + nlo;
         ext += fmax(h * h, l * l);
+        H = fmax(H, fmax(h, l));
         if (threadIdx.x == 0) sc[d] = c;
     }
     __syncthreads();
@@ -220,6 +228,12 @@
         st[1] = a;
         st[2] = r;
         st[3] = ext;
+        const bool extent = H > 0.0 && H < inf;
+        const double hs = 2.0 * (extent ? H : SD_INT_H0) / SD_INT_GRID;
+        st[SD_INT] = hs;
+        st[SD_INT + 1] = 1.0 / hs;
+        st[SD_INT + 2] = (matern ? 0.63 : 0.61) * sqrt((double)D) * hs + (matern ? 5.0 / 6.0 : 0.5) * 2.0 * SD_INT_OFF * hs * hs;
+        st[SD_INT + 3] = extent ? H : 0.0;
     }
     if ((int)threadIdx.x < D) st[SD_CTR + threadIdx.x] = sc[threadIdx.x];
 }
@@ -246,6 +260,38 @@
         const int slot = (tile >> 3) * 2 * NB + (tile & 7) * 16 + (l & 3) * 4 + (l >> 2);
         apack[slot] = real ? amp * alpha[row] : 0.0;
         apack[slot + NB] = nb;
+    }
+}
+
+__device__ __forceinline__ void screen_int_digits(int A, int& d0, int& d1, int& d2) {
+    d2 = (int)(signed char)A;
+    A = (A - d2) >> 8;
+    d1 = (int)(signed char)A;
+    d0 = (A - d1) >> 8;
+}
+__device__ __forceinline__ void screen_int_put(v4i& v, int d, int digit) { v[d >> 2] |= (digit & 255) << (8 * (d & 3)); }
+
+__global__ __launch_bounds__(256) void screen_int_pack_kernel(const double* __restrict__ alpha, const double* __restrict__ Xs,
+                                                              const double* __restrict__ st, double amp, int D, int n,
+                                                              v4i* __restrict__ rows, double* __restrict__ apack) {
+    const int tile = blockIdx.x * 4 + (threadIdx.x >> 6), l = threadIdx.x & 63, g = l >> 4;
+    const int row = tile * 16 + (l & 15);
+    const bool real = row < n;
+    v4i v = {0, 0, 0, 0};
+    double na = 0.0;
+    if (real)
+        for (int d = 0; d < D; ++d) {
+            const double q = fmax(fmin(rint((Xs[(size_t)row * D + d] - st[SD_CTR + d]) * st[SD_INT + 1]), SD_INT_AMAX), -SD_INT_AMAX);
+            int dg[3];
+            screen_int_digits((int)q, dg[0], dg[1], dg[2]);
+            if (g < 3) screen_int_put(v, d, dg[g]);
+            na = fma(q, q, na);
+        }
+    rows[(size_t)tile * 64 + l] = v;
+    if (g == 0) {
+        const int slot = (tile >> 3) * 2 * NB + (tile & 7) * 16 + l;
+        apack[slot] = real ? amp * alpha[row] : 0.0;
+        apack[slot + NB] = na;
     }
 }
 
@@ -351,20 +397,22 @@
 constexpr double SCREEN_SINGLE_SAFETY = 1.5;
 constexpr double SCREEN_SINGLE_MAX = 0.5;
 template <int KIND>
+__device__ __forceinline__ float screen_single_cov(float tx) {
+    if (KIND == ROBO_KERNEL_MATERN52_ARD) {
+        const float s = hw_sqrt_f32(tx);
+        const float q = fmaf(tx, 0.333333333f, 1.0f + s);
+        return q * hw_exp2_f32(s * -1.44269504f);
+    }
+    return hw_exp2_f32(tx * 1.44269504f);
+}
+
+template <int KIND>
 __device__ __forceinline__ void screen_dot_finish_single(const v4d acc, double nc, const double* __restrict__ al, double (&dot)[4]) {
 #pragma unroll
     for (int r = 0; r < 4; ++r) {
-        float kv;
-        if (KIND == ROBO_KERNEL_MATERN52_ARD) {
-            const float t = (float)fmax(fma(5.0, acc[r], nc), 5.0 * SD_R2_MIN);
-            const float s = hw_sqrt_f32(t);
-            const float q = fmaf(t, 0.333333333f, 1.0f + s);
-            kv = q * hw_exp2_f32(s * -1.44269504f);
-        } else {
-            const float x = (float)fmin(fma(-0.5, acc[r], nc), -0.5 * SD_R2_MIN);
-            kv = hw_exp2_f32(x * 1.44269504f);
-        }
-        dot[r] = fma((double)kv, al[r], dot[r]);
+        const float tx = KIND == ROBO_KERNEL_MATERN52_ARD ? (float)fmax(fma(5.0, acc[r], nc), 5.0 * SD_R2_MIN)
+                                                          : (float)fmin(fma(-0.5, acc[r], nc), -0.5 * SD_R2_MIN);
+        dot[r] = fma((double)screen_single_cov<KIND>(tx), al[r], dot[r]);
     }
 }
 
@@ -451,6 +499,117 @@
                        SCREEN_DOT_SAFETY * fabs(y_std) * fabs(cp.amp) * ck * r2_err * alpha_norm[1];
         if (FINISH != SD_FULL) delta += SCREEN_LEAN_SAFETY * SD_LEAN_EPS * fabs(y_std) * fabs(cp.amp) * alpha_norm[1];
         if (FINISH == SD_SINGLE) delta += SCREEN_SINGLE_SAFETY * SD_SINGLE_EPS * fabs(y_std) * fabs(cp.amp) * alpha_norm[1];
+        double u, l;
+        screen_bounds(acq_kind, par, eta, mt, delta, v_prior, u, l);
+        up[i] = u;
+        lo[i] = l;
+        if (!isnan(l)) lmax = l;
+    }
+    lmax = screen_block_max(lmax, sMx);
+    if (tid == 0) atomicMax(bkey, screen_key(lmax));
+}
+
+template <int KIND>
+__global__ __launch_bounds__(256) void screen_bounds_dot_int_kernel(const double* __restrict__ Xcs, const v4i* __restrict__ Xs,
+                                                                    const double* __restrict__ alpha,
+                                                                    const double* __restrict__ alpha_norm, CovParams cp, int n,
+                                                                    long long m, double mean_c, double y_mean, double y_std,
+                                                                    int acq_kind, double par, double eta, double* __restrict__ up,
+                                                                    double* __restrict__ lo, unsigned long long* __restrict__ bkey) {
+    __shared__ double sMx[4];
+    constexpr int TILES = SD_STAGE / 16, STAGE_VECS = TILES * 64, PER = STAGE_VECS / 256;
+    __shared__ v4i sA[STAGE_VECS];
+    __shared__ __attribute__((aligned(32))) double sAN[2 * SD_STAGE];
+    const double *sAl = sAN, *sNj = sAN + SD_STAGE;
+    const int tid = threadIdx.x, lane = tid & 63, wave = tid >> 6, g = lane >> 4, D = cp.dim;
+    const long long i = (long long)blockIdx.x * SD_CAND + wave * 16 + (lane & 15);
+    const bool live = i < m;
+    const long long ii = live ? i : 0;
+    const double inv_h = alpha_norm[SD_INT + 1];
+    v4i B0 = {0, 0, 0, 0}, B1 = {0, 0, 0, 0}, B2 = {0, 0, 0, 0};
+    double nb = SD_INT_OFF;
+    bool far = false, lost = false;
+#pragma unroll
+    for (int d = 0; d < SD_INT_MAX_D; ++d) {
+        if (d < D) {
+            const double q = rint((Xcs[ii * D + d] - alpha_norm[SD_CTR + d]) * inv_h);
+            const bool fin = fabs(q) < __builtin_huge_val();
+            const double qc = fin ? fmax(fmin(q, SD_INT_AMAX), -SD_INT_AMAX) : 0.0;
+            lost = lost || !fin;
+            far = far || qc != q;
+            int d0, d1, d2;
+            screen_int_digits((int)qc, d0, d1, d2);
+            screen_int_put(B0, d, d0);
+            screen_int_put(B1, d, d1);
+            screen_int_put(B2, d, d2);
+            nb = fma(qc, qc, nb);
+        }
+    }
+    const v4i zero = {0, 0, 0, 0};
+    const v4i bop0 = g == 0 ? B0 : zero;
+    const v4i bop1 = g == 0 ? B1 : g == 1 ? B0 : zero;
+    const v4i bop2 = g == 0 ? B2 : g == 1 ? B1 : g == 2 ? B0 : zero;
+    const v4i bop3 = g == 1 ? B2 : g == 2 ? B1 : zero;
+    const double hs = alpha_norm[SD_INT];
+    const double scale = KIND == ROBO_KERNEL_MATERN52_ARD ? 5.0 * hs * hs : -0.5 * hs * hs;
+    const int nst = (n + SD_STAGE - 1) / SD_STAGE;
+    v4i pa[PER];
+#pragma unroll
+    for (int e = 0; e < PER; ++e) pa[e] = Xs[e * 256 + tid];
+    double pan = alpha[tid];
+    double dot[4] = {0.0, 0.0, 0.0, 0.0};
+    for (int s = 0; s < nst; ++s) {
+        __syncthreads();
+#pragma unroll
+        for (int e = 0; e < PER; ++e) sA[e * 256 + tid] = pa[e];
+        sAN[tid] = pan;
+        __syncthreads();
+        if (s + 1 < nst) {
+            const v4i* nx = Xs + (size_t)(s + 1) * STAGE_VECS;
+#pragma unroll
+            for (int e = 0; e < PER; ++e) pa[e] = nx[e * 256 + tid];
+            pan = alpha[(s + 1) * 2 * SD_STAGE + tid];
+        }
+        v4i a = sA[lane];
+        v4i s0 = mfma_i8(a, bop0, zero), s1 = mfma_i8(a, bop1, zero), s2 = mfma_i8(a, bop2, zero), s3 = mfma_i8(a, bop3, zero);
+#pragma unroll
+        for (int t = 0; t < TILES; ++t) {
+            v4i n0 = s0, n1 = s1, n2 = s2, n3 = s3;
+            if (t + 1 < TILES) {
+                a = sA[(t + 1) * 64 + lane];
+                n0 = mfma_i8(a, bop0, zero);
+                n1 = mfma_i8(a, bop1, zero);
+                n2 = mfma_i8(a, bop2, zero);
+                n3 = mfma_i8(a, bop3, zero);
+            }
+            const double* nj = sNj + t * 16 + g * 4;
+            const double* al = sAl + t * 16 + g * 4;
+#pragma unroll
+            for (int r = 0; r < 4; ++r) {
+                const int t0 = s0[r] * 256 + s1[r], t1 = s2[r] * 256 + s3[r];
+                const double p = fma((double)t0, 65536.0, (double)t1);
+                const double u = fma(p, -512.0, nj[r] + nb);
+                dot[r] = fma((double)screen_single_cov<KIND>((float)(u * scale)), al[r], dot[r]);
+            }
+            s0 = n0;
+            s1 = n1;
+            s2 = n2;
+            s3 = n3;
+        }
+    }
+    double mu = (dot[0] + dot[1]) + (dot[2] + dot[3]);
+    mu += __shfl_xor(mu, 16);
+    mu += __shfl_xor(mu, 32);
+    double lmax = -__builtin_huge_val();
+    if (g == 0 && live) {
+        const double kself = cp.amp;
+        double mt = mu + mean_c;
+        mt = mt * y_std + y_mean;
+        const double v_prior = kself * (y_std * y_std);
+        const double eps_c = lost ? __builtin_nan("") : far ? 1.0 : alpha_norm[SD_INT + 2];
+        const double delta = SCREEN_DELTA_REL * (fabs(y_mean) + fabs(y_std) * (fabs(mean_c) + sqrt(fabs(kself)) * alpha_norm[0])) +
+                             (SCREEN_LEAN_SAFETY * SD_LEAN_EPS + SCREEN_SINGLE_SAFETY * (SD_SINGLE_EPS + eps_c)) * fabs(y_std) *
+                                 fabs(cp.amp) * alpha_norm[1];
         double u, l;
         screen_bounds(acq_kind, par, eta, mt, delta, v_prior, u, l);
         up[i] = u;
@@ -586,7 +745,8 @@
 static int alpha_ensure(robo_gp* g) {
     const size_t np = (size_t)g->n_pad_max;
     const int ks = screen_dot_ks(g);
-    const size_t dot_doubles = ks ? SD_CTR + SCREEN_DOT_MAX_D + 2 * np + np * 4 * (size_t)ks : 0;
+    const bool ints = ks && g->dim <= SD_INT_MAX_D;
+    const size_t dot_doubles = ks ? SD_STATS + 2 * np + np * 4 * (size_t)ks + (ints ? 2 * np + 8 * np : 0) : 0;
     if (!g->d_alpha) ROBO_TRY(dev_alloc(&g->d_alpha, 2 * np + 8 + dot_doubles));
     if (g->alpha_gen == g->fit_gen) return ROBO_OK;
     robo_ctx* c = g->ctx;
@@ -598,20 +758,31 @@
     double* stats = g->d_alpha + 2 * np;
     hipLaunchKernelGGL(screen_alpha_norm_kernel, dim3(1), dim3(256), 0, st, (const double*)a, (const double*)g->d_Xs, g->cov,
                        g->n, stats);
-    g->dot_extent = g->dot_alpha_sum = 0.0;
+    g->dot_extent = g->dot_alpha_sum = g->int_step = g->int_eps = 0.0;
     if (ks) {
-        double* apack = stats + SD_CTR + SCREEN_DOT_MAX_D;
+        double* apack = stats + SD_STATS;
         const int nst = (g->n + SD_STAGE - 1) / SD_STAGE;
         hipLaunchKernelGGL(screen_dot_prep_kernel, dim3(1), dim3(256), 0, st, (const double*)a, (const double*)g->d_Xs, g->dim,
-                           g->n, stats);
+                           g->n, g->kind == ROBO_KERNEL_MATERN52_ARD ? 1 : 0, stats);
         hipLaunchKernelGGL(screen_dot_pack_kernel, dim3((unsigned)(nst * SD_STAGE / 64)), dim3(256), 0, st, (const double*)a,
                            (const double*)g->d_Xs, (const double*)stats, g->cov.amp, g->dim, ks, g->n, apack + 2 * np, apack);
+        if (ints) {
+            double* ipack = apack + 2 * np + np * 4 * (size_t)ks;
+            hipLaunchKernelGGL(screen_int_pack_kernel, dim3((unsigned)(nst * SD_STAGE / 64)), dim3(256), 0, st, (const double*)a,
+                               (const double*)g->d_Xs, (const double*)stats, g->cov.amp, g->dim, g->n,
+                               reinterpret_cast<v4i*>(ipack + 2 * np), ipack);
+        }
         ROBO_LAUNCH_CHECK();
+        static_assert(SD_STATS - 1 <= 48, "the pinned block's tail");
         double* hp = c->h_pinned + MAX_DIM + 16;
-        ROBO_HIP_CHECK(hipMemcpyAsync(hp, stats + 1, 3 * sizeof(double), hipMemcpyDeviceToHost, st));
+        ROBO_HIP_CHECK(hipMemcpyAsync(hp, stats + 1, (SD_STATS - 1) * sizeof(double), hipMemcpyDeviceToHost, st));
         ROBO_HIP_CHECK(hipStreamSynchronize(st));
         g->dot_alpha_sum = hp[0];
         g->dot_extent = hp[2];
+        if (ints) {
+            g->int_step = hp[SD_INT - 1];
+            g->int_eps = hp[SD_INT + 3 - 1] > 0.0 ? hp[SD_INT + 2 - 1] : 0.0;
+        }
     }
     ROBO_LAUNCH_CHECK();
     g->alpha_gen = g->fit_gen;
@@ -639,6 +810,16 @@
     if (t == 0 || !screen_dot_wanted(g) || !screen_lean_wanted(g)) return false;
     if (t > 0) return true;
     const double term = SCREEN_SINGLE_SAFETY * SD_SINGLE_EPS * std::sqrt(std::fabs(g->cov.amp)) * g->dot_alpha_sum;
+    return term <= SCREEN_SINGLE_MAX;
+}
+
+static bool screen_int_wanted(const robo_gp* g) {
+    const int t = g->ctx->tune.acq_screen_int;
+    if (t == 0 || g->dim > SD_INT_MAX_D || !(g->int_step > 0.0)) return false;
+    if (t > 0) return true;
+    if (screen_dot_ks(g) != 4) return false;
+    if (!(g->int_eps > 0.0)) return false;
+    const double term = SCREEN_SINGLE_SAFETY * (SD_SINGLE_EPS + g->int_eps) * std::sqrt(std::fabs(g->cov.amp)) * g->dot_alpha_sum;
     return term <= SCREEN_SINGLE_MAX;
 }
 
@@ -662,10 +843,29 @@
     const dim3 grid((unsigned)((k->m + SC_CAND - 1) / SC_CAND));
     const double* alpha = g->d_alpha + (size_t)g->n_pad_max;
     const double* anorm = g->d_alpha + 2 * (size_t)g->n_pad_max;
+    k->scr_int = 0;
+    k->scr_int_step = 0.0;
     if (screen_dot_wanted(g)) {
-        const double* apack = anorm + SD_CTR + SCREEN_DOT_MAX_D;
+        const double* apack = anorm + SD_STATS;
         const double* rows = apack + 2 * (size_t)g->n_pad_max;
         const dim3 dgrid((unsigned)((k->m + SD_CAND - 1) / SD_CAND));
+        if (single && screen_int_wanted(g)) {
+            const double* ipack = rows + (size_t)g->n_pad_max * 4 * screen_dot_ks(g);
+            const v4i* irows = reinterpret_cast<const v4i*>(ipack + 2 * (size_t)g->n_pad_max);
+#define ROBO_SCREEN_INT_CALL(KIND)                                                                                              \
+    hipLaunchKernelGGL((screen_bounds_dot_int_kernel<KIND>), dgrid, dim3(256), 0, c->stream, (const double*)k->d_Xcs, irows, ipack, \
+                       anorm, g->cov, g->n, (long long)k->m, g->mean_c, g->y_mean, g->y_std, kind, par, eta, k->d_scr_up,      \
+                       k->d_scr_lo, bkey)
+            if (g->kind == ROBO_KERNEL_MATERN52_ARD) ROBO_SCREEN_INT_CALL(ROBO_KERNEL_MATERN52_ARD);
+            else ROBO_SCREEN_INT_CALL(ROBO_KERNEL_RBF_ARD);
+#undef ROBO_SCREEN_INT_CALL
+            ROBO_LAUNCH_CHECK();
+            k->scr_bounds_kernel = "screen_bounds_dot_kernel";
+            k->scr_finish = screen_lean_wanted(g) ? ROBO_SCREEN_FINISH_LEAN : ROBO_SCREEN_FINISH_FULL;
+            k->scr_int = 1;
+            k->scr_int_step = g->int_step;
+            return ROBO_OK;
+        }
 #define ROBO_SCREEN_DOT_CALL(KIND, KS, LEAN)                                                                                  \
     hipLaunchKernelGGL((screen_bounds_dot_kernel<KIND, KS, LEAN>), dgrid, dim3(256), 0, c->stream, (const double*)k->d_Xcs, rows,  \
                        apack, anorm, g->cov, g->n, (long long)k->m, g->mean_c, g->y_mean, g->y_std, kind, par, eta,          \
@@ -747,6 +947,8 @@
         k->scr_tail_fused = false;
         k->scr_first_stage = 0;
         k->scr_first_kept = 0;
+        k->scr_int = 0;
+        k->scr_int_step = 0.0;
     }
     if (want_values || !screen_eligible(g, k, kind, par, eta)) return acq_sweep(&g, 1, false, kind, par, &eta, k, allow_chain);
     if (g->screen_gen != g->fit_gen) {
@@ -796,8 +998,12 @@
             k->scr_first_stage = 2;
             g->single_skip = g->single_backoff;
             if (g->single_backoff < (1 << 20)) g->single_backoff *= 2;
+            const int first_int = k->scr_int;
+            const double first_step = k->scr_int_step;
             ROBO_TRY(launch_screen_bounds(g, k, kind, par, eta));
             ROBO_TRY(count_survivors());
+            k->scr_int = first_int;
+            k->scr_int_step = first_step;
         }
     }
     k->scr_n = k->m;
@@ -900,6 +1106,13 @@
     return ROBO_OK;
 }
 
+int32_t robo_cand_last_screen_form(robo_cand* k, int32_t* out_form, double* out_step) {
+    if (!k) return ROBO_BAD_ARGUMENT;
+    if (out_form) *out_form = k->scr_int ? ROBO_SCREEN_FORM_INT8 : ROBO_SCREEN_FORM_FP64;
+    if (out_step) *out_step = k->scr_int_step;
+    return ROBO_OK;
+}
+
 int32_t robo_acq_screen_bounds(robo_gp* g, int32_t acq_kind, double par, double eta, robo_cand* k, double* out_upper,
                                double* out_lower) {
     if (!g || !k) return ROBO_BAD_ARGUMENT;
```
